# meirbon/rfw-rs

Measured on AMD Instinct MI355X. Metric: Mrays/s (primary+shadow, 1spp), higher is better.
Workload: dtype f32

## Files before the change

### include/rfw_hip.h

```cpp
#ifndef RFW_HIP_H
#define RFW_HIP_H

#include "rfw_pod.h"

#ifdef __cplusplus
extern "C" {
#endif

#define RFW_HIP_API __attribute__((visibility("default")))
#define RFW_HIP_ABI_VERSION 2

enum {
    RFW_HIP_OK = 0,
    RFW_HIP_E_INVALID = -1,
    RFW_HIP_E_DEVICE = -2,
    RFW_HIP_E_STATE = -3,
    RFW_HIP_E_NOMEM = -4
};

enum { RFW_HIP_BUILDER_AUTO = 0, RFW_HIP_BUILDER_HOST_SAH = 1, RFW_HIP_BUILDER_DEVICE_LBVH = 2, RFW_HIP_BUILDER_DEVICE_SAH = 3 };

typedef struct {
    uint32_t struct_size;
    int32_t device;
// ... 55 lines not shown
    uint64_t split_references;
    uint64_t accel_bytes;
    uint32_t packet_copies;
    uint32_t pad;
} rfw_hip_scene_stats;

typedef struct {
    int32_t inst;
    int32_t tri;
    float t;
    float u, v;
} rfw_hip_hit;

RFW_HIP_API void* rfw_hip_create(uint32_t width, uint32_t height, double scale, const rfw_hip_options* options);
RFW_HIP_API void rfw_hip_destroy(void* instance);
RFW_HIP_API const char* rfw_hip_last_error(void* instance);
RFW_HIP_API uint32_t rfw_hip_abi_version(void);
RFW_HIP_API int64_t rfw_hip_selftest_splits(const rfw_rt_triangle* tris, uint32_t n, float split_tau, uint32_t threads, float* pieces7, uint32_t pieces_cap,
                                            uint32_t* duplicate_of, uint32_t duplicates_cap, uint32_t* n_pieces);
RFW_HIP_API uint32_t rfw_hip_selftest_index_magic(uint32_t d, uint64_t n_max);
RFW_HIP_API int64_t rfw_hip_selftest_bvh(const float* boxes6, uint32_t n, uint32_t max_leaf, uint32_t threads, uint32_t* out_nodes);

RFW_HIP_API int rfw_hip_set_2d_mesh(void* instance, uint32_t id, const void* vertices, uint32_t num_vertices, int32_t tex_id);
RFW_HIP_API int rfw_hip_set_2d_instances(void* instance, uint32_t mesh, const rfw_mat4* matrices, uint32_t num_matrices);
RFW_HIP_API int rfw_hip_set_3d_mesh(void* instance, uint32_t id, const rfw_mesh_data_3d* data);
RFW_HIP_API int rfw_hip_unload_3d_meshes(void* instance, const uint32_t* ids, uint32_t num_ids);
RFW_HIP_API int rfw_hip_set_3d_instances(void* instance, uint32_t mesh, const rfw_instances_data_3d* data);
RFW_HIP_API int rfw_hip_set_materials(void* instance, const rfw_device_material* materials, uint32_t num, const uint32_t* changed);
RFW_HIP_API int rfw_hip_set_textures(void* instance, const rfw_texture_data* textures, uint32_t num, const uint32_t* changed);
RFW_HIP_API int rfw_hip_synchronize(void* instance);
enum {
    RFW_HIP_RENDER_DEFAULT = 0,
    RFW_HIP_RENDER_NORMAL = 1,
    RFW_HIP_RENDER_ALBEDO = 2,
    RFW_HIP_RENDER_GBUFFER = 3,
    RFW_HIP_RENDER_SCREEN_SPACE = 4,
    RFW_HIP_RENDER_SSAO = 5,
    RFW_HIP_RENDER_FILTERED_SSAO = 6
};
RFW_HIP_API int rfw_hip_render(void* instance, const rfw_mat4* view_2d, const rfw_camera_view_3d* view_3d, uint32_t mode);
RFW_HIP_API int rfw_hip_resize(void* instance, uint32_t width, uint32_t height, double scale);
RFW_HIP_API int rfw_hip_set_point_lights(void* instance, const rfw_point_light* lights, uint32_t num, const uint32_t* changed);
RFW_HIP_API int rfw_hip_set_spot_lights(void* instance, const rfw_spot_light* lights, uint32_t num, const uint32_t* changed);
RFW_HIP_API int rfw_hip_set_area_lights(void* instance, const rfw_area_light* lights, uint32_t num, const uint32_t* changed);
RFW_HIP_API int rfw_hip_set_directional_lights(void* instance, const rfw_directional_light* lights, uint32_t num, const uint32_t* changed);
RFW_HIP_API int rfw_hip_set_skybox(void* instance, const rfw_texture_data* skybox);
RFW_HIP_API int rfw_hip_set_skins(void* instance, const rfw_skin_data* skins, uint32_t num, const uint32_t* changed);

RFW_HIP_API int rfw_hip_reset_accumulation(void* instance);
RFW_HIP_API int rfw_hip_set_option(void* instance, const char* key, double value);
RFW_HIP_API int rfw_hip_read_framebuffer(void* instance, float* rgba, uint64_t n_floats);
RFW_HIP_API int rfw_hip_read_accumulator(void* instance, float* rgba, uint64_t n_floats);
RFW_HIP_API int rfw_hip_get_frame_stats(void* instance, rfw_hip_frame_stats* out);
RFW_HIP_API int rfw_hip_drain_timing(void* instance, rfw_hip_frame_stats* sum, uint32_t* frames);
RFW_HIP_API int rfw_hip_get_scene_stats(void* instance, rfw_hip_scene_stats* out);
RFW_HIP_API int rfw_hip_set_stream(void* instance, void* hip_stream);
RFW_HIP_API void* rfw_hip_get_stream(void* instance);
RFW_HIP_API int rfw_hip_device_synchronize(void* instance);

RFW_HIP_API int rfw_hip_shard_info(void* instance, uint64_t* slab_floats, uint32_t* num_tiles_local, uint32_t* num_tiles_total);
RFW_HIP_API int rfw_hip_set_slab_output(void* instance, void* device_ptr);
RFW_HIP_API int rfw_hip_assemble_frame(void* instance, const void* gathered_device_ptr);

RFW_HIP_API int rfw_hip_comm_unique_id(void* out128);
RFW_HIP_API int rfw_hip_comm_init(void* instance, const void* id128, uint32_t rank, uint32_t world);
RFW_HIP_API int rfw_hip_comm_destroy(void* instance);
RFW_HIP_API int rfw_hip_comm_init_loopback(void* instance, uint64_t hub_key, uint32_t rank, uint32_t world);

#define RFW_HIP_P2P_HANDLE_BYTES 256
RFW_HIP_API int rfw_hip_p2p_export(void* instance, void* handle_out);
RFW_HIP_API int rfw_hip_p2p_connect(void* instance, const void* handles);
RFW_HIP_API int rfw_hip_p2p_disconnect(void* instance);

RFW_HIP_API int rfw_hip_intersect(void* instance, const float* origins, const float* directions,
                                  float t_min, float t_max, uint64_t n, rfw_hip_hit* hits);
RFW_HIP_API int rfw_hip_occludes(void* instance, const float* origins, const float* directions,
                                 float t_min, const float* t_max, uint64_t n, uint8_t* occluded);
RFW_HIP_API int rfw_hip_depth_test(void* instance, const float* origins, const float* directions,
                                   float t_min, float t_max, uint64_t n, rfw_hip_hit* hits, uint32_t* depth);

RFW_HIP_API int rfw_hip_intersect4(void* instance, const float* origin_xyz4, const float* direction_xyz4, const float* t_min4, float* t4,
                                   int32_t* instance_ids4, int32_t* prim_ids4);
RFW_HIP_API int rfw_hip_occludes4(void* instance, const float* origin_xyz4, const float* direction_xyz4, const float* t_min4, const float* t_max4,
                                  uint8_t* occluded4);

RFW_HIP_API int rfw_hip_debug_read(void* instance, const char* what, void* dst, uint64_t bytes, uint64_t* written);

RFW_HIP_API int rfw_hip_debug_occludes_depth(void* instance, const float* origins, const float* directions, float t_min, const float* t_max,
                                             uint64_t num_rays, uint8_t* occluded, uint32_t* depth);
RFW_HIP_API int rfw_hip_debug_lbvh_stress(void* instance, uint32_t num_boxes, uint32_t iterations, uint32_t seed, uint64_t* errors, uint64_t* checked);

RFW_HIP_API int rfw_hip_debug_eval_shading(void* instance, int op, uint64_t n, const float* in48, float* out12);

RFW_HIP_API int rfw_hip_render_batch(void* instance, const rfw_camera_view_3d* views, uint32_t count);
RFW_HIP_API int rfw_hip_assemble_batch(void* instance, const void* gathered_device_ptr, uint32_t count);
RFW_HIP_API int rfw_hip_render_samples(void* instance, const rfw_camera_view_3d* view, uint32_t count);
RFW_HIP_API int rfw_hip_set_blue_noise(void* instance, const uint32_t* table, uint32_t n_words);
RFW_HIP_API int rfw_hip_read_framebuffer_at(void* instance, uint32_t frame, float* rgba, uint64_t n_floats);
RFW_HIP_API int rfw_hip_read_accumulator_at(void* instance, uint32_t frame, float* rgba, uint64_t n_floats);

RFW_HIP_API void rfw_hip_srgb_steps(float* out255);
RFW_HIP_API void* rfw_hip_host_alloc(uint64_t bytes);
RFW_HIP_API void rfw_hip_host_free(void* ptr);
RFW_HIP_API int rfw_hip_download_frame(void* instance, uint32_t what, uint32_t frame, float* host_rgba, uint64_t n_floats);
RFW_HIP_API int rfw_hip_wait_downloads(void* instance);
RFW_HIP_API int rfw_hip_wait_download(void* instance, const void* host_ptr);
// ... 10 lines not shown
```

### rfw-rs_amd/backend.py

```python
import ctypes as C
import enum
import os

import numpy as np

from . import pod
from .scene import BackendTable

_HERE = os.path.dirname(os.path.abspath(__file__))
HIP_LIB = os.environ.get("RFW_HIP_LIB") or os.path.join(_HERE, "csrc", "librfw_hip.so")

EXPORTS = [
    "rfw_hip_create", "rfw_hip_destroy", "rfw_hip_last_error", "rfw_hip_abi_version", "rfw_hip_selftest_bvh", "rfw_hip_selftest_splits", "rfw_hip_selftest_index_magic",
    "rfw_hip_set_2d_mesh", "rfw_hip_set_2d_instances", "rfw_hip_set_3d_mesh", "rfw_hip_unload_3d_meshes",
    "rfw_hip_set_3d_instances", "rfw_hip_set_materials", "rfw_hip_set_textures", "rfw_hip_synchronize",
    "rfw_hip_render", "rfw_hip_resize", "rfw_hip_set_point_lights", "rfw_hip_set_spot_lights",
    "rfw_hip_set_area_lights", "rfw_hip_set_directional_lights", "rfw_hip_set_skybox", "rfw_hip_set_skins",
    "rfw_hip_reset_accumulation", "rfw_hip_set_option", "rfw_hip_read_framebuffer", "rfw_hip_read_accumulator",
    "rfw_hip_get_frame_stats", "rfw_hip_drain_timing", "rfw_hip_get_scene_stats", "rfw_hip_set_stream", "rfw_hip_get_stream", "rfw_hip_device_synchronize",
    "rfw_hip_shard_info", "rfw_hip_set_slab_output", "rfw_hip_assemble_frame", "rfw_hip_intersect", "rfw_hip_occludes", "rfw_hip_debug_occludes_depth",
    "rfw_hip_debug_read", "rfw_hip_bandwidth_probe", "rfw_hip_depth_test", "rfw_hip_render_batch", "rfw_hip_assemble_batch",
    "rfw_hip_read_framebuffer_at", "rfw_hip_read_accumulator_at", "rfw_hip_host_alloc", "rfw_hip_host_free", "rfw_hip_download_frame",
    "rfw_hip_wait_downloads", "rfw_hip_wait_download", "rfw_hip_srgb_steps", "rfw_hip_render_samples", "rfw_hip_set_blue_noise", "rfw_hip_debug_eval_shading", "rfw_hip_comm_unique_id", "rfw_hip_comm_init", "rfw_hip_comm_init_loopback", "rfw_hip_comm_destroy", "rfw_hip_p2p_export", "rfw_hip_p2p_connect", "rfw_hip_p2p_disconnect", "rfw_hip_intersect4", "rfw_hip_occludes4", "rfw_hip_debug_lbvh_stress", "rfw_hip_issue_probe",
]

_lib = None


ABI_VERSION = 2


def hip_lib():
    global _lib
    if _lib is None:
        if not os.path.exists(HIP_LIB):
            raise RuntimeError(f"HIP extension {HIP_LIB} is missing — build it with __graft_entry__.build(); there is no CPU fallback")
        try:
            import torch
        except ImportError:
            pass
        l = C.CDLL(HIP_LIB)
        vp, u32, u64, f32, cp = C.c_void_p, C.c_uint32, C.c_uint64, C.c_float, C.c_char_p
        l.rfw_hip_create.restype = vp
        l.rfw_hip_create.argtypes = [u32, u32, C.c_double, C.POINTER(pod.HipOptions)]
        l.rfw_hip_destroy.argtypes = [vp]
        l.rfw_hip_destroy.restype = None
        l.rfw_hip_last_error.argtypes = [vp]
        l.rfw_hip_last_error.restype = cp
        l.rfw_hip_abi_version.restype = u32
        if l.rfw_hip_abi_version() != ABI_VERSION:
            raise RuntimeError(f"{HIP_LIB} speaks ABI version {l.rfw_hip_abi_version()}, this binding version {ABI_VERSION}: rebuild the library")
        l.rfw_hip_selftest_bvh.argtypes = [vp, u32, u32, u32, C.POINTER(u32)]
        l.rfw_hip_selftest_bvh.restype = C.c_int64
        l.rfw_hip_selftest_splits.argtypes = [vp, u32, C.c_float, u32, vp, u32, vp, u32, C.POINTER(u32)]
        l.rfw_hip_selftest_splits.restype = C.c_int64
        l.rfw_hip_selftest_index_magic.argtypes = [u32, C.c_uint64]
        l.rfw_hip_selftest_index_magic.restype = u32
        l.rfw_hip_set_2d_mesh.argtypes = [vp, u32, vp, u32, C.c_int32]
        l.rfw_hip_set_2d_instances.argtypes = [vp, u32, vp, u32]
        l.rfw_hip_set_3d_mesh.argtypes = [vp, u32, C.POINTER(pod.MeshData3D)]
        l.rfw_hip_unload_3d_meshes.argtypes = [vp, C.POINTER(u32), u32]
        l.rfw_hip_set_3d_instances.argtypes = [vp, u32, C.POINTER(pod.InstancesData3D)]
        l.rfw_hip_set_materials.argtypes = [vp, vp, u32, vp]
        l.rfw_hip_set_textures.argtypes = [vp, vp, u32, vp]
        l.rfw_hip_synchronize.argtypes = [vp]
        l.rfw_hip_render.argtypes = [vp, C.POINTER(pod.Mat4), C.POINTER(pod.CameraView3D), u32]
        l.rfw_hip_resize.argtypes = [vp, u32, u32, C.c_double]
        for n in ("point", "spot", "area", "directional"):
            getattr(l, f"rfw_hip_set_{n}_lights").argtypes = [vp, vp, u32, vp]
        l.rfw_hip_set_skybox.argtypes = [vp, C.POINTER(pod.TextureData)]
        l.rfw_hip_set_skins.argtypes = [vp, vp, u32, vp]
        l.rfw_hip_reset_accumulation.argtypes = [vp]
        l.rfw_hip_set_option.argtypes = [vp, cp, C.c_double]
        l.rfw_hip_read_framebuffer.argtypes = [vp, vp, u64]
        l.rfw_hip_read_accumulator.argtypes = [vp, vp, u64]
        l.rfw_hip_get_frame_stats.argtypes = [vp, C.POINTER(pod.FrameStats)]
# ... 231 lines not shown

    def accumulator_at(self, frame):
        a = np.empty((self.height, self.width, 4), dtype=np.float32)
        self._check(self._l.rfw_hip_read_accumulator_at(self._h, frame, a.ctypes.data, a.size))
        return a

    def framebuffer_at(self, frame):
        a = np.empty((self.height, self.width, 4), dtype=np.float32)
        self._check(self._l.rfw_hip_read_framebuffer_at(self._h, frame, a.ctypes.data, a.size))
        return a

    def host_frame(self, presented=False):
        n = self.height * self.width * (1 if presented else 4)
        p = self._l.rfw_hip_host_alloc(n * 4)
        if not p:
            raise BackendError("rfw_hip_host_alloc failed")
        if presented:
            a = np.ctypeslib.as_array(C.cast(p, C.POINTER(C.c_uint8)), shape=(self.height, self.width, 4))
        else:
            a = np.ctypeslib.as_array(C.cast(p, C.POINTER(C.c_float)), shape=(self.height, self.width, 4))
        self._pinned[a.ctypes.data] = p
        return a

    def free_host_frame(self, a):
        self._l.rfw_hip_host_free(self._pinned.pop(a.ctypes.data))

    def download_frame(self, dst, accumulator=False, frame=0):
        if dst.dtype == np.uint8:
            self._check(self._l.rfw_hip_download_frame(self._h, 2, frame, dst.ctypes.data, dst.size // 4))
        else:
            self._check(self._l.rfw_hip_download_frame(self._h, 1 if accumulator else 0, frame, dst.ctypes.data, dst.size))

    def srgb_steps(self):
        t = np.empty(255, np.float32)
        self._l.rfw_hip_srgb_steps(t.ctypes.data)
        return t

    def wait_downloads(self, dst=None):
        if dst is None:
            self._check(self._l.rfw_hip_wait_downloads(self._h))
        else:
            self._check(self._l.rfw_hip_wait_download(self._h, dst.ctypes.data))

    def framebuffer(self):
        a = np.empty((self.height, self.width, 4), dtype=np.float32)
        self._check(self._l.rfw_hip_read_framebuffer(self._h, a.ctypes.data, a.size))
        return a

    def accumulator(self):
        a = np.empty((self.height, self.width, 4), dtype=np.float32)
        self._check(self._l.rfw_hip_read_accumulator(self._h, a.ctypes.data, a.size))
        return a

    def frame_stats(self):
        s = pod.FrameStats()
        self._check(self._l.rfw_hip_get_frame_stats(self._h, C.byref(s)))
        return {n: (list(getattr(s, n)) if n in ("nodes_visited", "tris_tested", "instances_entered", "node_test_executions", "tri_test_executions", "wave_max_nodes", "uniform_node_test_executions") else getattr(s, n)) for n, _ in pod.FrameStats._fields_}

    def drain_timing(self):
        s, n = pod.FrameStats(), C.c_uint32(0)
        self._check(self._l.rfw_hip_drain_timing(self._h, C.byref(s), C.byref(n)))
        return {k: getattr(s, k) for k, _ in pod.FrameStats._fields_ if k.startswith("ms_")}, int(n.value)

    def scene_stats(self):
        s = pod.SceneStats()
        self._check(self._l.rfw_hip_get_scene_stats(self._h, C.byref(s)))
        return {n: getattr(s, n) for n, _ in pod.SceneStats._fields_}

    def set_stream(self, stream_handle):
        self._check(self._l.rfw_hip_set_stream(self._h, C.c_void_p(stream_handle)))

    def stream_handle(self):
        return int(self._l.rfw_hip_get_stream(self._h) or 0)

    def device_synchronize(self):
        self._check(self._l.rfw_hip_device_synchronize(self._h))

    def shard_info(self):
        f, a, b = C.c_uint64(0), C.c_uint32(0), C.c_uint32(0)
        self._check(self._l.rfw_hip_shard_info(self._h, C.byref(f), C.byref(a), C.byref(b)))
        return {"slab_floats": int(f.value), "tiles_local": int(a.value), "tiles_total": int(b.value)}

    def set_slab_output(self, device_ptr):
        self._check(self._l.rfw_hip_set_slab_output(self._h, C.c_void_p(device_ptr)))

    def assemble_frame(self, gathered_device_ptr):
        self._check(self._l.rfw_hip_assemble_frame(self._h, C.c_void_p(gathered_device_ptr)))

    def intersect(self, origins, directions, t_min=1e-4, t_max=1e26):
        o = np.ascontiguousarray(origins, dtype=np.float32)
        d = np.ascontiguousarray(directions, dtype=np.float32)
        hits = np.empty(len(o), dtype=HIT_DTYPE)
        self._check(self._l.rfw_hip_intersect(self._h, o.ctypes.data, d.ctypes.data, t_min, t_max, len(o), hits.ctypes.data))
        return hits

    def depth_test(self, origins, directions, t_min=1e-4, t_max=1e26):
        o = np.ascontiguousarray(origins, dtype=np.float32)
        d = np.ascontiguousarray(directions, dtype=np.float32)
        hits = np.empty(len(o), dtype=HIT_DTYPE)
        depth = np.empty(len(o), dtype=np.uint32)
        self._check(self._l.rfw_hip_depth_test(self._h, o.ctypes.data, d.ctypes.data, t_min, t_max, len(o), hits.ctypes.data, depth.ctypes.data))
        return hits, depth

    def occludes_depth(self, origins, directions, t_max, t_min=1e-3):
        o = np.ascontiguousarray(origins, dtype=np.float32)
        d = np.ascontiguousarray(directions, dtype=np.float32)
# ... 56 lines not shown
```

### rfw-rs_amd/csrc/api_frame.cpp

```cpp
#include "api_internal.h"

using namespace rfwapi;

namespace rfwapi {
thread_local std::string g_create_error;
}
namespace rfwhip {
static EnvSwitches g_env;
const EnvSwitches& env_switches() { return g_env; }
void read_env_switches()
{
    EnvSwitches e;
    auto set = [](const char* name) { const char* v = getenv(name); return v != nullptr && std::strcmp(v, "0") != 0; };
    e.build_trace = set("RFW_BUILD_TRACE");
    e.no_forest = set("RFW_NO_FOREST");
    e.lbvh_fenced = set("RFW_LBVH_FENCED");
    e.p2p_data_cached = set("RFW_P2P_DATA_CACHED");
    e.p2p_flags_finegrained = set("RFW_P2P_FLAGS_FINEGRAINED");
    if (const char* v = getenv("RFW_PACKET_AUTO_MAX_TRIANGLES")) e.packet_auto_max_triangles = strtoull(v, nullptr, 10);
    if (const char* v = getenv("RFW_SPATIAL_SPLITS")) { e.has_spatial_splits = true; e.spatial_splits = (float)std::max(0.0, atof(v)); }
    if (const char* v = getenv("RFW_PACKET_TRACE")) e.packet_trace = std::max(0, atoi(v));
    if (const char* v = getenv("RFW_NODE_ORDER")) e.node_order = std::max(0, atoi(v));
    static std::mutex mu;
    std::lock_guard<std::mutex> g(mu);
    g_env = e;
}
}
namespace rfwapi {
uint32_t index_magic(const uint32_t d, const uint64_t n_max)
{
    if (d < 2u) return 0u;
    const uint64_t m = ((1ull << 32) + d - 1u) / d, e = m * d - (1ull << 32);
    if (m > 0xffffffffull || n_max >= (1ull << 32)) return 0u;
    return (e == 0 || n_max < (1ull << 32) / e) ? (uint32_t)m : 0u;
}

void compute_shard(Instance* I)
{
    const uint32_t S = I->substreams, wv = I->world * S;
    I->tiles_x = (I->width + I->tile_size - 1) / I->tile_size;
    I->tiles_y = (I->height + I->tile_size - 1) / I->tile_size;
    const uint32_t total = I->tiles_x * I->tiles_y;
    I->local_tiles_v = (total + wv - 1) / wv;
    I->cap_v = I->local_tiles_v * I->tile_size * I->tile_size;
    I->local_tiles = I->local_tiles_v * S;
    I->capacity = I->cap_v * S;
    uint64_t px = 0;
    for (uint32_t t = 0; t < total; t++) {
        if ((t % wv) / S != I->rank) continue;
        const uint32_t tx = t % I->tiles_x, ty = t / I->tiles_x;
        const uint32_t w = std::min(I->tile_size, I->width - tx * I->tile_size), h = std::min(I->tile_size, I->height - ty * I->tile_size);
        px += (uint64_t)w * h;
    }
    I->local_pixels = px;
}

int alloc_paths(Instance* I)
{
    compute_shard(I);
    const size_t n = (size_t)I->capacity * I->max_batch;
    for (int h = 0; h < 2; h++) {
        HIP_TRY(I, I->d_ray_o[h].ensure(n));
        HIP_TRY(I, I->d_ray_d[h].ensure(n));
        HIP_TRY(I, I->d_thr[h].ensure(n));
        HIP_TRY(I, I->d_hit[h].ensure(n));
    }
    HIP_TRY(I, I->d_sh_o.ensure(n * kShadowBuckets));
    HIP_TRY(I, I->d_sh_d.ensure(n * kShadowBuckets));
    HIP_TRY(I, I->d_sh_e.ensure(n * kShadowBuckets));
    HIP_TRY(I, I->d_acc_slab.ensure(n));
    HIP_TRY(I, hipMemsetAsync(I->d_acc_slab.ptr, 0, n * sizeof(float4), I->stream));
    const size_t px = (size_t)I->width * I->height * I->max_batch;
    HIP_TRY(I, I->d_frame_out.ensure(px));
    I->acc_source = nullptr;
// ... 87 lines not shown
    PathDev p;
    const size_t off = (size_t)sub * I->cap_v;
    for (int h = 0; h < 2; h++) {
        p.ray_o[h] = I->d_ray_o[h].ptr + off;
        p.ray_d[h] = I->d_ray_d[h].ptr + off;
        p.thr[h] = I->d_thr[h].ptr + off;
        p.hit[h] = I->d_hit[h].ptr + off;
    }
    p.sh_o = I->d_sh_o.ptr + off * kShadowBuckets;
    p.sh_d = I->d_sh_d.ptr + off * kShadowBuckets;
    p.sh_e = I->d_sh_e.ptr + off * kShadowBuckets;
    p.acc = I->d_acc_slab.ptr + off;
    p.capacity = I->cap_v;
    return p;
}

inline int ev_index(uint32_t bounce, int kernel, int end) { return EV_KERNEL_BASE + 2 * ((int)bounce * kKernelsPerBounce + kernel) + end; }
constexpr int kEvBlit = EV_KERNEL_BASE + 2 * (kMaxBounces * kKernelsPerBounce);

hipEvent_t* ring_events(Instance* I, int slot, uint32_t sub) { return I->ring.data() + ((size_t)slot * I->substreams + sub) * kNumEvents; }

static float ao_radius_of(Instance* I)
{
    if (I->ao_radius > 0.0f) return I->ao_radius;
    Instance* O = scene_of(I);
    if (O->ao_auto_version != O->scene_version) {
        float lo[3] = {INFINITY, INFINITY, INFINITY}, hi[3] = {-INFINITY, -INFINITY, -INFINITY};
        for (const auto& kv : O->inst_lists) {
            const rfw_aabb& b = kv.second.local_aabb;
            for (const rfw_mat4& m : kv.second.matrices) {
                bool zero = true;
                for (int c = 0; c < 16; c++) zero = zero && m.m[c] == 0.0f;
                if (zero) continue;
                for (int c = 0; c < 8; c++) {
                    const float x = (c & 1) ? b.max[0] : b.min[0], y = (c & 2) ? b.max[1] : b.min[1], z = (c & 4) ? b.max[2] : b.min[2];
                    const float w[3] = {m.m[0] * x + m.m[4] * y + m.m[8] * z + m.m[12], m.m[1] * x + m.m[5] * y + m.m[9] * z + m.m[13],
                                        m.m[2] * x + m.m[6] * y + m.m[10] * z + m.m[14]};
                    for (int a = 0; a < 3; a++) { lo[a] = std::min(lo[a], w[a]); hi[a] = std::max(hi[a], w[a]); }
                }
            }
        }
        double d2 = 0.0;
        for (int a = 0; a < 3; a++) d2 += hi[a] >= lo[a] ? ((double)hi[a] - lo[a]) * ((double)hi[a] - lo[a]) : 0.0;
        O->ao_auto_radius = d2 > 0.0 ? (float)(0.05 * std::sqrt(d2)) : 1.0f;
        O->ao_auto_version = O->scene_version;
    }
    return O->ao_auto_radius;
}

int do_render(Instance* I, const rfw_camera_view_3d* views, uint32_t k, bool samples, uint32_t mode)
{
    const rfw_camera_view_3d& view = views[0];
    HIP_TRY(I, hipSetDevice(I->device));
    if (!scene_of(I)->synchronized || tlas_of(I)->d_tlas_nodes.ptr == nullptr) return RFW_HIP_OK;
    if (I->scene && I->scene->scene_ready && I->waited_version != I->scene->scene_version) {
        HIP_TRY(I, hipStreamWaitEvent(I->stream, I->scene->scene_ready, 0));
        I->waited_version = I->scene->scene_version;
    }
    {
        Instance* S = scene_of(I);
        if (S->tables_ready && I->tables_waited != S->tables_version) {
            HIP_TRY(I, hipStreamWaitEvent(I->stream, S->tables_ready, 0));
            I->tables_waited = S->tables_version;
        }
        I->tables_used = S->tables_version;
        if (I->tables_oldest_pending == ~0ull) I->tables_oldest_pending = S->tables_version;
    }
    if ((I->have_last_view && (std::memcmp(&I->last_view, &view, sizeof(view)) != 0 || mode != I->render_mode)) || I->after_batch) I->sample_count = 0;
    I->render_mode = mode;
    I->after_batch = k > 1 && !samples;
    I->last_view = view;
    I->have_last_view = true;
    if (k > 1) {
        if (k > I->max_batch || k > (uint32_t)kMaxBatch) return fail(I, RFW_HIP_E_INVALID, "render_batch: more frames than options.max_batch");
        if (I->substreams > 1) return fail(I, RFW_HIP_E_STATE, "render_batch: not available with sub-streams");
        if ((uint64_t)I->width * I->height >= (1ull << 24)) return fail(I, RFW_HIP_E_INVALID, "render_batch: frames of 2^24 pixels or more cannot be batched");
        for (uint32_t f = 1; f < k; f++)
            if (views[f].spread_angle != view.spread_angle) return fail(I, RFW_HIP_E_INVALID, "render_batch: the views of a batch must share one spread angle (field of view and height)");
        if (!samples) I->sample_count = 0;
    }

    const uint32_t S = I->substreams;
    const bool count = (I->flags & RFW_HIP_FLAG_COUNT_TRAVERSAL) != 0;
    const bool nee = !(I->flags & RFW_HIP_FLAG_NO_NEE);
    hipStream_t main = I->stream;
    const bool tm = I->timing;
    const int slot = (int)(I->frame_index % kTimingRing);
    I->events = ring_events(I, slot, 0);
    const uint32_t bounces = std::min<uint32_t>(I->max_path_length, kMaxBounces);
    const bool ao = mode >= RFW_HIP_RENDER_SSAO;
    const uint32_t ao_rounds = ao ? I->ao_samples : 0u;
    if (ao) HIP_TRY(I, I->d_ao_guide.ensure((size_t)I->width * I->height));
    const bool dn = I->denoise > 0 && mode == RFW_HIP_RENDER_DEFAULT && (k == 1 || samples) && I->world <= 1 && !scene_of(I)->comm && !scene_of(I)->loop &&
                    !scene_of(I)->p2p.connected;
    if (dn) {
        const size_t px = (size_t)I->width * I->height;
        HIP_TRY(I, I->d_dn_guide.ensure(3 * px));
        for (int q = 0; q < 2 && I->denoise > 1; q++) HIP_TRY(I, I->d_dn_plane[q].ensure(px));
    }

    if (tm) (void)hipEventRecord(I->events[EV_FRAME0], main);
    I->counter_phase ^= 1u;
    if (S > 1) HIP_TRY(I, hipEventRecord(I->ev_fork, main));
    SceneDev sc[kMaxSub];
    PathDev p[kMaxSub];
    CameraParams cam[kMaxSub];
    hipStream_t st[kMaxSub];
    for (uint32_t s = 0; s < S; s++) {
        st[s] = S > 1 ? I->sub[s] : main;
        if (S > 1) HIP_TRY(I, hipStreamWaitEvent(st[s], I->ev_fork, 0));
        sc[s] = scene_dev(I);
        sc[s].counters = I->d_counters.ptr + (size_t)I->counter_phase * kMaxSub + s;
        sc[s].counters_next = I->d_counters.ptr + (size_t)(I->counter_phase ^ 1u) * kMaxSub + s;
        sc[s].spill = I->d_spill.ptr + (size_t)s * (I->cap_v + kSpillMargin);
        p[s] = path_dev(I, s);
        cam[s] = camera_params(I, view, s);
        {
            const Instance* O = scene_of(I);
            const int g = O->shade_group;
            if (g == 256 || (g == 0 && k == 1 && !O->slots.empty())) cam[s].flags |= kFlagShadeSmallGroups;
        }
    }
    BatchViews bv;
    if (k > 1) {
        cam[0].batch = k;
        if (scene_of(I)->stream_auto) cam[0].stream_run = scene_of(I)->stream_run;
        p[0].capacity = I->cap_v * k;
        for (uint32_t f = 0; f < k; f++) {
            cam[0].batch_sample[f] = samples ? I->sample_count + f : 0u;
            FrameView& v = bv.v[f];
            v.pos[0] = views[f].pos.x; v.pos[1] = views[f].pos.y; v.pos[2] = views[f].pos.z; v.lens_size = views[f].lens_size;
            v.right[0] = views[f].right.x; v.right[1] = views[f].right.y; v.right[2] = views[f].right.z; v.pad0 = 0.0f;
            v.up[0] = views[f].up.x; v.up[1] = views[f].up.y; v.up[2] = views[f].up.z; v.pad1 = 0.0f;
            v.p1[0] = views[f].p1.x; v.p1[1] = views[f].p1.y; v.p1[2] = views[f].p1.z; v.pad2 = 0.0f;
        }
    }
    if (mode != RFW_HIP_RENDER_DEFAULT) {
        const float radius = ao ? ao_radius_of(I) : 0.0f;
        const float dir[3] = {view.direction.x, view.direction.y, view.direction.z};
        for (uint32_t s = 0; s < S; s++) {
            hipEvent_t* ev = ring_events(I, slot, s);
            if (tm) (void)hipEventRecord(ev[ev_index(0, 0, 0)], st[s]);
            launch_primary(st[s], cam[s], sc[s], p[s], count);
            if (tm) (void)hipEventRecord(ev[ev_index(0, 0, 1)], st[s]);
            if (tm) (void)hipEventRecord(ev[ev_index(0, 1, 0)], st[s]);
            launch_aov(st[s], cam[s], sc[s], p[s], mode, ao_rounds, radius, I->d_ao_guide.ptr, dir);
            if (tm) (void)hipEventRecord(ev[ev_index(0, 1, 1)], st[s]);
            if (tm) (void)hipEventRecord(ev[ev_index(0, 2, 0)], st[s]);
        }
        for (uint32_t r = 0; r < ao_rounds; r++)
            for (uint32_t s = 0; s < S; s++) launch_shadow(st[s], cam[s], sc[s], p[s], r, count);
        for (uint32_t s = 0; s < S; s++)
            if (tm) (void)hipEventRecord(ring_events(I, slot, s)[ev_index(0, 2, 1)], st[s]);
    }
    for (uint32_t b = 0; b < bounces && mode == RFW_HIP_RENDER_DEFAULT; b++) {
        for (uint32_t s = 0; s < S; s++) {
            hipEvent_t* ev = ring_events(I, slot, s);
            if (tm) (void)hipEventRecord(ev[ev_index(b, 0, 0)], st[s]);
            if (b == 0 && k > 1) launch_primary_batch(st[s], cam[s], bv, sc[s], p[s], count);
            else if (b == 0) launch_primary(st[s], cam[s], sc[s], p[s], count);
            else {
                const uint32_t* order = nullptr;
                const int mode = scene_of(I)->sort_extension_rays;
                if ((mode == 1 || (mode == 2 && k > 1 && cam[s].stream_run == 0u)) && S == 1) {
                    const size_t n = p[s].capacity;
                    for (int q = 0; q < 2; q++) { HIP_TRY(I, I->d_sort_keys[q].ensure(n)); HIP_TRY(I, I->d_sort_vals[q].ensure(n)); }
                    HIP_TRY(I, I->d_sort_ws.ensure(sort_pairs_workspace_bytes((uint32_t)n)));
                    launch_extension_keys(st[s], sc[s], p[s], b, I->d_sort_keys[0].ptr, I->d_sort_vals[0].ptr);
                    HIP_TRY(I, sort_pairs_u32(st[s], I->d_sort_ws.ptr, I->d_sort_ws.cap, I->d_sort_keys[0].ptr, I->d_sort_keys[1].ptr, I->d_sort_vals[0].ptr,
                                              I->d_sort_vals[1].ptr, (uint32_t)n, 32));
                    order = I->d_sort_vals[1].ptr;
                }
                launch_extend(st[s], cam[s], sc[s], p[s], b, count, order);
            }
            if (tm) (void)hipEventRecord(ev[ev_index(b, 0, 1)], st[s]);
            if (b == 0 && dn) {
                PathDev g = p[s];
                if (k > 1) {
                    const size_t last = (size_t)(k - 1u) * I->cap_v;
                    g.hit[0] += last; g.ray_o[0] += last; g.ray_d[0] += last;
                    g.capacity = I->cap_v;
                }
                launch_dn_guide(st[s], cam[s], sc[s], g, I->d_dn_guide.ptr, k > 1 ? 0x00ffffffu : 0xffffffffu);
            }
        }
        for (uint32_t s = 0; s < S; s++) {
            hipEvent_t* ev = ring_events(I, slot, s);
            if (tm) (void)hipEventRecord(ev[ev_index(b, 1, 0)], st[s]);
            launch_shade(st[s], cam[s], sc[s], p[s], b);
            if (tm) (void)hipEventRecord(ev[ev_index(b, 1, 1)], st[s]);
        }
        if (nee)
            for (uint32_t s = 0; s < S; s++) {
                hipEvent_t* ev = ring_events(I, slot, s);
                if (tm) (void)hipEventRecord(ev[ev_index(b, 2, 0)], st[s]);
                launch_shadow(st[s], cam[s], sc[s], p[s], b, count);
                if (tm) (void)hipEventRecord(ev[ev_index(b, 2, 1)], st[s]);
            }
    }
    if (S > 1)
        for (uint32_t s = 0; s < S; s++) {
            HIP_TRY(I, hipEventRecord(I->ev_join[s], st[s]));
            HIP_TRY(I, hipStreamWaitEvent(main, I->ev_join[s], 0));
        }
    if (samples && k > 1) {
        launch_sum_batch(main, I->d_acc_slab.ptr, I->cap_v, k);
        cam[0].batch = 1;
    }
    I->sample_count += samples ? k : 1;
    const uint32_t frames_out = samples ? 1u : k;
    if (tm) (void)hipEventRecord(I->events[kEvBlit], main);
    if (Instance* C = scene_of(I); C->comm || C->loop) {
        const uint64_t n_send = slab_words(I) * frames_out;
        pack_slabs(I, main, I->d_send.ptr, frames_out);
        if (C->comm_chain && C->comm_chain_pending) HIP_TRY(I, hipStreamWaitEvent(main, C->comm_chain, 0));
        if (C->loop) {
            const int lrc = loop_all_gather(I, main, n_send);
            if (lrc != RFW_HIP_OK) return lrc;
        } else {
            const ncclResult_t nr = g_rccl.all_gather(I->d_send.ptr, I->d_recv.ptr, n_send, ncclFloat, C->comm, main);
            if (nr != ncclSuccess) return fail(I, RFW_HIP_E_DEVICE, std::string("ncclAllGather: ") + g_rccl.error_string(nr));
        }
        if (C->comm_chain) { HIP_TRY(I, hipEventRecord(C->comm_chain, main)); C->comm_chain_pending = true; }
        const int arc = gathered_arrived(I, main, I->d_recv.ptr, frames_out);
        if (arc != RFW_HIP_OK) return arc;
    } else if (C->p2p.connected) {
        const int prc = p2p_exchange(I, main, frames_out);
        if (prc != RFW_HIP_OK) return prc;
    } else if (I->world <= 1)
    {
        if (dn) {
            float4* const planes[2] = {I->d_dn_plane[0].ptr, I->d_dn_plane[1].ptr};
            launch_atrous(main, cam[0], I->d_acc_slab.ptr, I->cap_v, I->d_dn_guide.ptr, planes, I->d_frame_out.ptr, I->sample_count, I->denoise, I->denoise_colour,
                          I->denoise_form);
        }
        else if (mode == RFW_HIP_RENDER_FILTERED_SSAO) launch_ao_filter(main, cam[0], I->d_acc_slab.ptr, I->cap_v, I->d_ao_guide.ptr, I->d_frame_out.ptr, I->sample_count);
        else launch_assemble(main, cam[0], I->d_acc_slab.ptr, false, false, I->cap_v, I->d_frame_out.ptr, I->sample_count, mode != RFW_HIP_RENDER_DEFAULT);
        I->acc_source = I->d_acc_slab.ptr; I->acc_source_rgb = false; I->acc_source_batch = frames_out;
    }
    if (I->external_slab)
        pack_slabs(I, main, I->external_slab, frames_out);
    if (tm) (void)hipEventRecord(I->events[kEvBlit + 1], main);
    if (tm) (void)hipEventRecord(I->events[EV_FRAME1], main);
    HIP_TRY(I, hipGetLastError());
    const uint32_t passes = mode == RFW_HIP_RENDER_DEFAULT ? bounces : 1u;
    I->last_bounces = passes;
    I->ring_bounces[slot] = tm ? passes : 0;
    I->ring_nee[slot] = mode == RFW_HIP_RENDER_DEFAULT ? nee : ao;
    I->ao_rounds = ao_rounds;
// ... 3 lines not shown
    I->last_count_flag = count;
    if (I->frame_done) HIP_TRY(I, hipEventRecord(I->frame_done, main));
    return RFW_HIP_OK;
}

}

extern "C" {

uint32_t rfw_hip_abi_version(void) { return RFW_HIP_ABI_VERSION; }
uint32_t rfw_hip_selftest_index_magic(uint32_t d, uint64_t n_max) { return index_magic(d, n_max); }


void* rfw_hip_create(uint32_t width, uint32_t height, double , const rfw_hip_options* o)
{
    read_env_switches();
    int ndev = 0;
    hipError_t e = hipGetDeviceCount(&ndev);
    if (e != hipSuccess || ndev == 0) {
        g_create_error = std::string("no HIP device available (") + (e == hipSuccess ? "0 devices" : hipGetErrorString(e)) +
                         "); this backend has no CPU fallback";
        return nullptr;
    }
    if (width == 0 || height == 0) {
        g_create_error = "width and height must be non-zero";
        return nullptr;
    }
    Instance* I = new Instance();
    I->width = width;
    I->height = height;
    int dev = -1;
    uint32_t n_slots = 1;
    if (o) {
        dev = o->device;
        if (o->max_path_length) I->max_path_length = std::min<uint32_t>(o->max_path_length, kMaxBounces);
        if (o->clamp_value > 0.0f) I->clamp_value = o->clamp_value;
        I->world = std::max<uint32_t>(o->world, 1);
        I->rank = o->rank;
        if (o->tile_size) I->tile_size = o->tile_size;
        if (o->builder) I->builder = o->builder;
        I->flags = o->flags & 15u;
        if (o->streams) I->substreams = std::min<uint32_t>(o->streams, kMaxSub);
        if (o->struct_size >= offsetof(rfw_hip_options, frames_in_flight) + sizeof(uint32_t)) n_slots = std::min<uint32_t>(std::max<uint32_t>(o->frames_in_flight, 1u), 24u);
        if (o->struct_size >= offsetof(rfw_hip_options, max_batch) + sizeof(uint32_t)) I->max_batch = std::min<uint32_t>(std::max<uint32_t>(o->max_batch, 1u), (uint32_t)kMaxBatch);
    }
    {
        const EnvSwitches& env = env_switches();
        if (env.has_spatial_splits) I->split_tau = env.spatial_splits;
        const int pt = env.packet_trace >= 0 ? env.packet_trace : kDefaultPacketTrace;
        I->packet_auto = env.packet_trace < 0;
        if (pt & 1) I->flags |= kFlagPacketPrimary;
        if (pt & 2) I->flags |= kFlagPacketShadow;
        if (pt & 4) I->flags |= kFlagPacketShadowFar;
    }
    if (I->max_batch > 1 && I->substreams > 1) {
        g_create_error = "max_batch > 1 needs streams <= 1 (a batch already fills the device with one launch per stage)";
        delete I;
        return nullptr;
    }
    if (I->rank >= I->world || (I->tile_size % 8) != 0) {
        g_create_error = "invalid shard options (rank >= world, or tile_size not a multiple of 8)";
        delete I;
        return nullptr;
    }
    I->blas_on_device = I->builder != RFW_HIP_BUILDER_HOST_SAH;
    I->blas_sah_on_device = I->builder == RFW_HIP_BUILDER_DEVICE_SAH || I->builder == RFW_HIP_BUILDER_AUTO;
    I->tlas_on_device = I->builder != RFW_HIP_BUILDER_HOST_SAH;
    if (dev < 0) (void)hipGetDevice(&dev);
    I->device = dev;
    I->build_threads = (int)std::max(1u, std::min(16u, std::thread::hardware_concurrency()));
    auto bail = [&](const char* what, hipError_t err) -> void* {
        g_create_error = std::string(what) + ": " + hipGetErrorString(err);
        delete I;
        return nullptr;
    };
    if ((e = hipSetDevice(dev)) != hipSuccess) return bail("hipSetDevice", e);
    if ((e = hipStreamCreateWithFlags(&I->own_stream, hipStreamNonBlocking)) != hipSuccess) return bail("hipStreamCreate", e);
    I->stream = I->own_stream;
    I->ring.assign((size_t)kTimingRing * I->substreams * kNumEvents, nullptr);
    for (auto& ev : I->ring)
        if ((e = hipEventCreate(&ev)) != hipSuccess) return bail("hipEventCreate", e);
    I->events = I->ring.data();
    if ((e = hipEventCreateWithFlags(&I->ev_fork, hipEventDisableTiming)) != hipSuccess) return bail("hipEventCreate", e);
    for (uint32_t k = 0; k < I->substreams && I->substreams > 1; k++) {
        if ((e = hipStreamCreateWithFlags(&I->sub[k], hipStreamNonBlocking)) != hipSuccess) return bail("hipStreamCreate", e);
        if ((e = hipEventCreateWithFlags(&I->ev_join[k], hipEventDisableTiming)) != hipSuccess) return bail("hipEventCreate", e);
    }
    for (int k = 0; k < Instance::kStages; k++)
        if ((e = hipEventCreateWithFlags(&I->stage_event[k], hipEventDisableTiming)) != hipSuccess) return bail("hipEventCreate", e);
    if ((e = hipHostMalloc((void**)&I->overflow_host, 64, hipHostMallocMapped)) != hipSuccess) return bail("hipHostMalloc (overflow flag)", e);
    std::memset(I->overflow_host, 0, 64);
    if ((e = hipHostGetDevicePointer((void**)&I->overflow_dev, I->overflow_host, 0)) != hipSuccess) return bail("hipHostGetDevicePointer", e);
    if (alloc_paths(I) != RFW_HIP_OK) {
        g_create_error = I->err;
        delete I;
        return nullptr;
    }
    (void)hipStreamSynchronize(I->stream);
    if (n_slots > 1) {
        if ((e = hipEventCreateWithFlags(&I->frame_done, hipEventDisableTiming)) != hipSuccess) return bail("hipEventCreate", e);
        if ((e = hipEventCreateWithFlags(&I->scene_ready, hipEventDisableTiming)) != hipSuccess) return bail("hipEventCreate", e);
        rfw_hip_options so;
        std::memset(&so, 0, sizeof(so));
        if (o) std::memcpy(&so, o, std::min<size_t>(o->struct_size ? o->struct_size : sizeof(so), sizeof(so)));
        so.struct_size = sizeof(so);
        so.device = I->device;
        so.frames_in_flight = 1;
        so.max_batch = I->max_batch;
        for (uint32_t k = 1; k < n_slots; k++) {
            Instance* c = static_cast<Instance*>(rfw_hip_create(width, height, 1.0, &so));
            if (!c) {
                for (Instance* d : I->slots) rfw_hip_destroy(d);
                I->slots.clear();
                rfw_hip_destroy(I);
                return nullptr;
            }
            c->scene = I;
            c->slot_index = k;
            if (hipEventCreateWithFlags(&c->frame_done, hipEventDisableTiming) != hipSuccess) {
                g_create_error = "hipEventCreate (frame slot)";
                rfw_hip_destroy(c);
                for (Instance* d : I->slots) rfw_hip_destroy(d);
                I->slots.clear();
                rfw_hip_destroy(I);
                return nullptr;
            }
            I->slots.push_back(c);
        }
    }
    return I;
}

void rfw_hip_destroy(void* inst)
{
    if (!inst) return;
    Instance* I = static_cast<Instance*>(inst);
    for (Instance* c : I->slots) rfw_hip_destroy(c);
    I->slots.clear();
    {
        std::lock_guard<std::mutex> g(I->mu);
        (void)hipSetDevice(I->device);
        (void)hipDeviceSynchronize();
        if (I->scene_ready) (void)hipEventDestroy(I->scene_ready);
        if (I->frame_done) (void)hipEventDestroy(I->frame_done);
        if (I->download_done) (void)hipEventDestroy(I->download_done);
        I->d_blas_nodes.release(); I->d_tlas_nodes.release(); I->d_blas_wide.release(); I->d_tlas_wide.release(); I->d_blas_oct.release(); I->d_tlas_oct.release(); I->d_blas_raw.release(); I->d_tlas_raw.release(); I->d_packets.release(); I->d_triangles.release();
        I->d_mesh_records.release(); I->d_matrices.release(); I->d_mesh_of_instance.release(); I->d_tlas_prims.release();
        I->d_xforms.release(); I->d_normals.release();
        for (auto& tb : I->tables) { tb.materials.release(); tb.area.release(); tb.point.release(); tb.spot.release(); tb.dir.release(); }
        if (I->tables_ready) (void)hipEventDestroy(I->tables_ready);
        if (I->upload_stream) (void)hipStreamDestroy(I->upload_stream);
        I->d_spill.release(); I->d_counters.release(); I->d_tex_data.release(); I->d_tex_desc.release(); I->d_blue_noise.release();
        I->d_valid_gids.release(); I->d_stage_dev.release(); I->d_tlas_order.release(); I->d_node_count.release(); I->d_inst_boxes.release(); I->d_mesh_local.release();
        I->d_tri_boxes.release(); I->d_lbvh_ws.release(); I->d_blas_order.release();
        I->d_q_o.release(); I->d_q_d.release(); I->d_q_t.release(); I->d_q_h.release(); I->d_q_depth.release(); I->d_q_r.release();
        if (I->comm) { (void)g_rccl.comm_destroy(I->comm); I->comm = nullptr; }
        if (I->loop) loop_leave(I);
        if (I->loop_sent) { (void)hipEventDestroy(I->loop_sent); I->loop_sent = nullptr; }
        if (I->comm_chain) (void)hipEventDestroy(I->comm_chain);
        for (auto& ev : I->ev_build)
            if (ev) (void)hipEventDestroy(ev);
        if (I->records_stream) (void)hipStreamSynchronize(I->records_stream);
        if (I->ev_heads) (void)hipEventDestroy(I->ev_heads);
        if (I->ev_records) (void)hipEventDestroy(I->ev_records);
        if (I->records_stream) (void)hipStreamDestroy(I->records_stream);
        I->d_heads.release();
        I->meshes.clear();
        for (auto& L : I->lanes) {
            if (L.s) (void)hipStreamDestroy(L.s);
            if (L.done) (void)hipEventDestroy(L.done);
            L.ws.release(); L.boxes.release();
        }
        p2p_release(I);
        I->d_send.release(); I->d_recv.release();
        for (int q = 0; q < 2; q++) { I->d_sort_keys[q].release(); I->d_sort_vals[q].release(); }
        I->d_sort_ws.release();
        if (I->overflow_host) (void)hipHostFree(I->overflow_host);
        I->pins.release();
        I->d_skin_data.release(); I->d_joints.release(); I->d_bounds_scratch.release(); I->d_sah_ws.release(); I->d_mesh_node_counts.release(); I->d_forest.release(); I->d_refit_parent.release(); I->d_refit_nint.release(); I->d_refit_arrive.release();
        for (int k = 0; k < Instance::kStages; k++) {
            if (I->stage_buf[k]) (void)hipHostFree(I->stage_buf[k]);
            if (I->stage_event[k]) (void)hipEventDestroy(I->stage_event[k]);
        }
        for (int h = 0; h < 2; h++) { I->d_ray_o[h].release(); I->d_ray_d[h].release(); I->d_thr[h].release(); I->d_hit[h].release(); }
        I->d_sh_o.release(); I->d_sh_d.release(); I->d_sh_e.release(); I->d_acc_slab.release(); I->d_frame_acc.release(); I->d_frame_out.release(); I->d_present.release();
        I->d_dn_guide.release(); I->d_dn_plane[0].release(); I->d_dn_plane[1].release();
        for (auto& ev : I->ring)
            if (ev) (void)hipEventDestroy(ev);
        if (I->ev_fork) (void)hipEventDestroy(I->ev_fork);
        for (int k = 0; k < kMaxSub; k++) {
            if (I->ev_join[k]) (void)hipEventDestroy(I->ev_join[k]);
            if (I->sub[k]) (void)hipStreamDestroy(I->sub[k]);
        }
        if (I->own_stream) (void)hipStreamDestroy(I->own_stream);
    }
    delete I;
}

const char* rfw_hip_last_error(void* inst)
{
    if (!inst) return g_create_error.c_str();
    return static_cast<Instance*>(inst)->err.c_str();
}

// ... 23 lines not shown
    if (rc != RFW_HIP_OK && cur != I && !cur->err.empty()) I->err = cur->err;
    return rc;
}

int rfw_hip_render(void* inst, const rfw_mat4* , const rfw_camera_view_3d* view, uint32_t mode)
{
    LOCK(inst);
    if (!view) return fail(I, RFW_HIP_E_INVALID, "render: null view");
    CHECK_OVERFLOW(I);
    return render_impl(I, view, 1, false, mode <= (uint32_t)RFW_HIP_RENDER_FILTERED_SSAO ? mode : (uint32_t)RFW_HIP_RENDER_DEFAULT);
}

int rfw_hip_render_batch(void* inst, const rfw_camera_view_3d* views, uint32_t count)
{
    LOCK(inst);
    if (!views || count == 0) return fail(I, RFW_HIP_E_INVALID, "render_batch: no views");
    CHECK_OVERFLOW(I);
    if (count == 1) {
        I->sample_count = 0;
        I->restart = true;
    }
    const int rc = render_impl(I, views, count);
    if (rc == RFW_HIP_OK && count == 1) (I->slots.empty() ? I : slot_ptr(I, I->cur_slot))->after_batch = true;
    return rc;
}

int rfw_hip_render_samples(void* inst, const rfw_camera_view_3d* view, uint32_t count)
{
    LOCK(inst);
    if (!view || count == 0) return fail(I, RFW_HIP_E_INVALID, "render_samples: no view / no samples");
    CHECK_OVERFLOW(I);
    if (count > I->max_batch || count > (uint32_t)kMaxBatch) return fail(I, RFW_HIP_E_INVALID, "render_samples: more samples than options.max_batch");
    if (count == 1) return render_impl(I, view, 1);
    rfw_camera_view_3d views[kMaxBatch];
    for (uint32_t f = 0; f < count; f++) views[f] = *view;
    return render_impl(I, views, count, true);
}


int rfw_hip_resize(void* inst, uint32_t w, uint32_t h, double)
{
    LOCK(inst);
    if (w == 0 || h == 0) return fail(I, RFW_HIP_E_INVALID, "resize: zero size");
    if (scene_of(I)->p2p.data && (w != I->width || h != I->height)) return fail(I, RFW_HIP_E_STATE, "resize: disconnect the p2p exchange first (its buffers are sized for the frame)");
    HIP_TRY(I, hipSetDevice(I->device));
    HIP_TRY(I, hipStreamSynchronize(I->stream));
    for (Instance* c : I->slots) {
        const int rc = rfw_hip_resize(c, w, h, 1.0);
        if (rc != RFW_HIP_OK) return fail(I, rc, c->err);
    }
    I->restart = true;
    I->width = w;
    I->height = h;
    I->deferred = Instance::Deferred(); I->acc_source = nullptr; I->presented_valid = false;
    const int arc = alloc_paths(I);
    if (arc == RFW_HIP_OK && (scene_of(I)->comm || scene_of(I)->loop)) {
        const size_t n = (size_t)I->capacity * I->max_batch * 3u;
        HIP_TRY(I, I->d_send.ensure(n));
        HIP_TRY(I, I->d_recv.ensure(n * I->world));
    }
    return arc;
}


int rfw_hip_reset_accumulation(void* inst)
{
    LOCK(inst);
    I->sample_count = 0;
    I->restart = true;
    return RFW_HIP_OK;
}

int rfw_hip_set_option(void* inst, const char* key, double value)
{
    LOCK(inst);
    if (!key) return fail(I, RFW_HIP_E_INVALID, "set_option: null key");
    const std::string k(key);
    if (k == "max_path_length") I->max_path_length = std::max<uint32_t>(1, std::min<uint32_t>((uint32_t)value, kMaxBounces));
    else if (k == "clamp_value") I->clamp_value = (float)value;
    else if (k == "nee") I->flags = value != 0.0 ? (I->flags & ~RFW_HIP_FLAG_NO_NEE) : (I->flags | RFW_HIP_FLAG_NO_NEE);
    else if (k == "count_traversal") I->flags = value != 0.0 ? (I->flags | RFW_HIP_FLAG_COUNT_TRAVERSAL) : (I->flags & ~RFW_HIP_FLAG_COUNT_TRAVERSAL);
    else if (k == "shadow_order") {
        I->flags &= ~(kFlagNearFirstDirectional | kFlagFarFirstPositional);
        if ((int)value == 1) I->flags |= kFlagNearFirstDirectional;
        else if ((int)value == 2) I->flags |= kFlagFarFirstPositional;
    }
    else if (k == "packet_trace") {
        I->flags &= ~(kFlagPacketPrimary | kFlagPacketShadow | kFlagPacketShadowFar);
        I->packet_auto = false;
        if ((int)value & 1) I->flags |= kFlagPacketPrimary;
        if ((int)value & 2) I->flags |= kFlagPacketShadow;
        if ((int)value & 4) I->flags |= kFlagPacketShadowFar;
        if (blas_wide_wanted(I, I->n_tris) && !I->d_blas_wide.ptr && I->n_tris) {
            for (auto& kv : I->meshes) kv.second.dirty = true;
            I->meshes_dirty = true;
            I->layout_valid = false;
        }
    }
    else if (k == "shade_group") {
        if ((int)value != 0 && (int)value != 256 && (int)value != 512) return fail(I, RFW_HIP_E_INVALID, "set_option: shade_group is 0, 256 or 512");
        I->shade_group = (int)value;
    }
    else if (k == "tlas_fused") I->tlas_fused = std::max(0, std::min(2, (int)value));
    else if (k == "sample_count") I->sample_count = (uint32_t)value;
    else if (k == "ao_samples" || k == "ao_radius") {
        if (k == "ao_samples") {
            if (!(value >= 1.0 && value <= (double)kAoMaxSamples)) return fail(I, RFW_HIP_E_INVALID, "set_option: ao_samples is 1 ... 8");
            I->ao_samples = (uint32_t)value;
        } else {
            if (!(value >= 0.0) || !std::isfinite(value)) return fail(I, RFW_HIP_E_INVALID, "set_option: ao_radius is >= 0 (0 = automatic)");
            I->ao_radius = (float)value;
        }
        I->sample_count = 0;
        I->restart = true;
    }
    else if (k == "denoise" || k == "denoise_colour") {
        if (k == "denoise") {
            if (!(value >= 0.0 && value <= (double)kDenoiseMaxPasses) || value != std::floor(value)) return fail(I, RFW_HIP_E_INVALID, "set_option: denoise is 0 (off) or 1 ... 5 passes");
            if ((uint32_t)value == I->denoise) return RFW_HIP_OK;
            I->denoise = (uint32_t)value;
        } else {
            if (!(value > 0.0) || !std::isfinite(value) || !((float)value > 0.0f) || !std::isfinite((float)value)) return fail(I, RFW_HIP_E_INVALID, "set_option: denoise_colour is > 0");
            if ((float)value == I->denoise_colour) return RFW_HIP_OK;
            I->denoise_colour = (float)value;
        }
        I->sample_count = 0;
        I->restart = true;
    }
    else if (k == "denoise_form") {
        if (value != 0.0 && value != 1.0 && value != 2.0) return fail(I, RFW_HIP_E_INVALID, "set_option: denoise_form is 0, 1 or 2");
        I->denoise_form = (uint32_t)value;
    }
    else if (k == "gather_format") {
        if (value < 0 || value > 2) return fail(I, RFW_HIP_E_INVALID, "set_option: gather_format is 0, 1 or 2");
        I->gather_format = (uint32_t)value;
        for (uint32_t q = 0; q <= I->slots.size(); q++) {
            Instance* c = slot_ptr(I, q);
            c->deferred = Instance::Deferred(); c->acc_source = nullptr; c->presented_valid = false;
        }
    }
    else if (k == "present_rank") I->present_rank = (int)value;
    else if (k == "timing") I->timing = value != 0.0;
    else if (k == "sort_extension_rays") I->sort_extension_rays = std::max(0, std::min(2, (int)value));
    else if (k == "texture_array") { I->texture_array = value != 0.0; I->tex_offsets.clear(); }
    else if (k == "spill_rows") {
        I->spill_rows = std::min<uint32_t>((uint32_t)std::max(0.0, value), (uint32_t)kStackSpill);
        clear_overflow(I);
    }
    else if (k == "sky_r") I->sky[0] = (float)value;
    else if (k == "sky_g") I->sky[1] = (float)value;
// ... 131 lines not shown
        Instance* c = slot_ptr(I, (uint32_t)k);
        if (c->download_dst.empty()) continue;
        if (host_ptr && std::find(c->download_dst.begin(), c->download_dst.end(), host_ptr) == c->download_dst.end()) continue;
        HIP_TRY(I, hipEventSynchronize(c->download_done));
        c->download_dst.clear();
    }
    return RFW_HIP_OK;
}
int rfw_hip_wait_downloads(void* inst) { return rfw_hip_wait_download(inst, nullptr); }

int rfw_hip_read_framebuffer(void* inst, float* rgba, uint64_t n) { return read_frame_impl(inst, 0, false, rgba, n); }
int rfw_hip_read_accumulator(void* inst, float* rgba, uint64_t n) { return read_frame_impl(inst, 0, true, rgba, n); }

static void add_frame_timing(Instance* I, int slot, uint32_t nb, bool nee, rfw_hip_frame_stats* out)
{
    hipEvent_t* e0 = ring_events(I, slot, 0);
    auto el = [&](hipEvent_t a, hipEvent_t b) { float ms = 0.0f; (void)hipEventElapsedTime(&ms, a, b); return ms; };
    out->ms_total += el(e0[EV_FRAME0], e0[EV_FRAME1]);
    out->ms_other += el(e0[kEvBlit], e0[kEvBlit + 1]);
    for (uint32_t s = 0; s < I->substreams; s++) {
        hipEvent_t* ev = ring_events(I, slot, s);
        for (uint32_t b = 0; b < nb; b++) {
            const float tr = el(ev[ev_index(b, 0, 0)], ev[ev_index(b, 0, 1)]);
            if (b == 0) out->ms_trace_primary += tr; else out->ms_trace_extend += tr;
            out->ms_shade += el(ev[ev_index(b, 1, 0)], ev[ev_index(b, 1, 1)]);
            if (nee) out->ms_trace_shadow += el(ev[ev_index(b, 2, 0)], ev[ev_index(b, 2, 1)]);
        }
    }
}

int rfw_hip_get_frame_stats(void* inst, rfw_hip_frame_stats* out)
{
    LOCK(inst);
    if (!out) return fail(I, RFW_HIP_E_INVALID, "get_frame_stats: null out");
    if (!I->slots.empty() && I->cur_slot != 0) {
        Instance* c = slot_ptr(I, I->cur_slot);
        const int rc = rfw_hip_get_frame_stats(c, out);
        if (rc != RFW_HIP_OK) I->err = c->err;
        return rc;
    }
    HIP_TRY(I, hipSetDevice(I->device));
    std::memset(out, 0, sizeof(*out));
    HIP_TRY(I, hipStreamSynchronize(I->stream));
    QueueCounters qc[kMaxSub];
    HIP_TRY(I, hipMemcpy(qc, I->d_counters.ptr + (size_t)I->counter_phase * kMaxSub, I->substreams * sizeof(QueueCounters), hipMemcpyDeviceToHost));
    CHECK_OVERFLOW(I);
    const uint32_t nb = I->last_bounces;
    out->primary_rays = nb ? I->local_pixels : 0;
    for (uint32_t s = 0; s < I->substreams; s++) {
        for (uint32_t b = 0; b + 1 < nb; b++) out->extension_rays += qc[s].ext[b];
        if (!(I->flags & RFW_HIP_FLAG_NO_NEE))
            for (uint32_t b = 0; b < nb; b++)
                for (int k = 0; k < kShadowBuckets; k++) out->shadow_rays += qc[s].shadow[b][k];
        for (int k = 0; k < 3; k++) {
            out->nodes_visited[k] += qc[s].trav[k][0];
            out->tris_tested[k] += qc[s].trav[k][1];
            out->instances_entered[k] += qc[s].trav[k][2];
            out->node_test_executions[k] += qc[s].wave_exec[k][0];
            out->tri_test_executions[k] += qc[s].wave_exec[k][1];
            out->uniform_node_test_executions[k] += qc[s].wave_uniform[k];
            out->wave_max_nodes[k] += qc[s].wave_max_nodes[k];
        }
    }
    out->sample_count = I->sample_count;
    out->bounces = nb;
    out->substreams = I->substreams;
    if (I->frame_recorded && nb) add_frame_timing(I, (int)((I->frame_index - 1) % kTimingRing), nb, !(I->flags & RFW_HIP_FLAG_NO_NEE), out);
    return RFW_HIP_OK;
}

int rfw_hip_drain_timing(void* inst, rfw_hip_frame_stats* sum, uint32_t* frames)
{
    LOCK(inst);
    if (!sum || !frames) return fail(I, RFW_HIP_E_INVALID, "drain_timing: null out");
    HIP_TRY(I, hipSetDevice(I->device));
    HIP_TRY(I, hipStreamSynchronize(I->stream));
    std::memset(sum, 0, sizeof(*sum));
    uint32_t n = 0;
    for (uint64_t f = I->drained_index; f < I->frame_index; f++) {
        const int slot = (int)(f % kTimingRing);
        const uint32_t nb = I->ring_bounces[slot];
        if (!nb) continue;
        add_frame_timing(I, slot, nb, I->ring_nee[slot], sum);
        n++;
    }
    sum->substreams = I->substreams;
    I->drained_index = I->frame_index;
    for (Instance* c : I->slots) {
        rfw_hip_frame_stats cs;
        uint32_t cn = 0;
        const int rc = rfw_hip_drain_timing(c, &cs, &cn);
        if (rc != RFW_HIP_OK) return fail(I, rc, c->err);
        sum->ms_total += cs.ms_total; sum->ms_trace_primary += cs.ms_trace_primary; sum->ms_trace_extend += cs.ms_trace_extend;
        sum->ms_trace_shadow += cs.ms_trace_shadow; sum->ms_shade += cs.ms_shade; sum->ms_other += cs.ms_other;
        n += cn;
    }
    *frames = n;
    return RFW_HIP_OK;
}


int rfw_hip_set_stream(void* inst, void* stream)
{
    LOCK(inst);
    if (!I->slots.empty()) return fail(I, RFW_HIP_E_STATE, "set_stream: an instance with frames in flight launches on its slots' own streams");
    HIP_TRY(I, hipSetDevice(I->device));
    HIP_TRY(I, hipStreamSynchronize(I->stream));
    I->stream = stream ? (hipStream_t)stream : I->own_stream;
    return RFW_HIP_OK;
}

void* rfw_hip_get_stream(void* inst)
{
    if (!inst) return nullptr;
    Instance* I = static_cast<Instance*>(inst);
    std::lock_guard<std::mutex> g(I->mu);
    return (void*)I->stream;
}

int rfw_hip_device_synchronize(void* inst)
// ... 10 lines not shown
```

### rfw-rs_amd/csrc/api_internal.h

```cpp
#pragma once
#include <hip/hip_runtime.h>
#include <dlfcn.h>
#include <unistd.h>
#if __has_include(<rccl/rccl.h>)
#include <rccl/rccl.h>
#else
extern "C" {
typedef struct ncclComm* ncclComm_t;
typedef struct { char internal[128]; } ncclUniqueId;
typedef enum { ncclSuccess = 0 } ncclResult_t;
typedef enum { ncclFloat = 7 } ncclDataType_t;
ncclResult_t ncclGetUniqueId(ncclUniqueId* id);
ncclResult_t ncclCommInitRank(ncclComm_t* comm, int nranks, ncclUniqueId id, int rank);
ncclResult_t ncclCommDestroy(ncclComm_t comm);
ncclResult_t ncclAllGather(const void* send, void* recv, size_t count, ncclDataType_t type, ncclComm_t comm, hipStream_t stream);
const char* ncclGetErrorString(ncclResult_t r);
}
#endif

#include <algorithm>
#include <atomic>
#include <chrono>
#include <cmath>
#include <cstring>
// ... 281 lines not shown
    int stage_next = 0;
    void* stage = nullptr;
    bool tlas_on_device = true, blas_on_device = false, blas_sah_on_device = false;
    DevBuf<char> d_sah_ws;
    DevBuf<uint32_t> d_mesh_node_counts;
    DevBuf<ForestTree> d_forest;
    DevBuf<uint32_t> d_refit_parent, d_refit_nint, d_refit_arrive;
    DevBuf<QueueCounters> d_counters;
    uint32_t counter_phase = 0;
    uint32_t* overflow_host = nullptr;
    uint32_t* overflow_dev = nullptr;
    uint32_t spill_rows = kStackSpill;
    DevBuf<float> d_q_o, d_q_d, d_q_t;
    DevBuf<rfw_hip_hit> d_q_h;
    DevBuf<uint32_t> d_q_depth;
    DevBuf<uint8_t> d_q_r;
    std::vector<MeshRecord> mesh_records;
    std::map<uint32_t, uint32_t> mesh_index;
    std::vector<uint32_t> record_tri_cap;
    std::vector<uint32_t> record_tri_orig;
    DevBuf<SplitPiece> d_split_pieces;
    std::vector<uint32_t> record_piece_off, record_piece_n;
    float split_tau = 8e-5f;
    uint64_t n_split_refs = 0;
    uint32_t tri_end = 0, node_end = 0;
    uint64_t hole_tris = 0;
    bool layout_valid = false;
    bool node_counts_stale = false;
    uint32_t incremental_builds = 0, full_builds = 0, heads_first_builds = 0, tlas_fused_builds = 0;
    bool packet_auto = true;
    PinnedRing pins;
    uint64_t n_instances = 0, n_valid_instances = 0, n_tris = 0, n_blas_nodes = 0, n_tlas_nodes = 0;
    uint64_t n_tris_logical = 0;
    float ms_blas_build = 0, ms_tlas_build = 0, ms_stage_wait = 0;
    float ms_blas_upload = 0, ms_blas_kernels = 0;
    uint64_t blas_upload_bytes = 0, blas_kernel_bytes = 0;
    struct BuildLane { hipStream_t s = nullptr; hipEvent_t done = nullptr; DevBuf<char> ws; DevBuf<DevBox> boxes; };
    static constexpr int kBuildLanes = 8;
    BuildLane lanes[kBuildLanes];
    hipEvent_t ev_build[3] = {nullptr, nullptr, nullptr};
    DevBuf<TriHead> d_heads;
    hipStream_t records_stream = nullptr;
    hipEvent_t ev_heads = nullptr, ev_records = nullptr;
    bool build_from_heads = false;
    bool records_pending = false;
    bool records_timed = false;
    bool build_events_pending = false;

    DevBuf<float4> d_ray_o[2], d_ray_d[2], d_thr[2], d_sh_o, d_sh_d, d_sh_e, d_acc_slab, d_frame_acc, d_frame_out;
    DevBuf<uint32_t> d_present;
    DevBuf<uint4> d_hit[2];
    DevBuf<uint32_t> d_sort_keys[2], d_sort_vals[2];
    DevBuf<char> d_sort_ws;
    int shade_group = 0;
    int sort_extension_rays = 2;
    void* external_slab = nullptr;
    ncclComm_t comm = nullptr;
    DevBuf<float> d_send, d_recv;
    uint32_t gather_format = 0;
    int present_rank = -1;
    struct Deferred { const void* gathered = nullptr; uint32_t k = 0, samples = 1; } deferred;
    bool presented_valid = false;
    hipEvent_t comm_chain = nullptr;
    bool comm_chain_pending = false;
    struct LoopHub* loop = nullptr;
    uint32_t loop_seq = 0;
    hipEvent_t loop_sent = nullptr;
    struct P2P {
        bool connected = false;
        uint32_t* data = nullptr;
        uint32_t* flags = nullptr;
        size_t slot_words = 0;
        uint32_t n_slots = 0;
        std::vector<uint32_t*> peer_data, peer_flags;
        std::vector<uint8_t> opened;
        uint64_t timeout_ticks = 500000000ull;
    } p2p;
    uint32_t slot_index = 0;
    uint32_t stream_leaf_gate = 16;
    bool stream_auto = true;
    uint32_t stream_run = 8, stream_refill = 12;
    uint32_t p2p_seq = 0;
    bool frame_elsewhere = false;
    uint32_t tiles_x = 0, tiles_y = 0, local_tiles = 0, capacity = 0;
    uint64_t local_pixels = 0;
    uint32_t sample_count = 0;
    bool have_last_view = false;
    rfw_camera_view_3d last_view{};
    uint32_t render_mode = 0;
    uint32_t ao_samples = 4;
    float ao_radius = 0.0f;
    float ao_auto_radius = 0.0f;
    uint64_t ao_auto_version = 0;
    uint32_t ao_rounds = 0;
    DevBuf<float4> d_ao_guide;
    uint32_t denoise = 0;
    float denoise_colour = kDenoiseDefaultColour;
    uint32_t denoise_form = 0;
    DevBuf<float4> d_dn_guide, d_dn_plane[2];
    std::vector<hipEvent_t> ring;
    hipEvent_t* events = nullptr;
    uint32_t substreams = 1;
    hipStream_t sub[kMaxSub] = {};
    hipEvent_t ev_fork = nullptr, ev_join[kMaxSub] = {};
    uint32_t local_tiles_v = 0, cap_v = 0;
    uint64_t frame_index = 0, drained_index = 0;
// ... 103 lines not shown
```

### rfw-rs_amd/csrc/device_types.h

```cpp
#pragma once
#include <cmath>
#include <cstdint>
#include <cstring>

#include "../../include/rfw_pod.h"

namespace rfwhip {

struct alignas(16) Node4 {
    float lox[4], hix[4], loy[4], hiy[4], loz[4], hiz[4];
    uint32_t child[4];
    uint32_t pad[4];
};
static_assert(sizeof(Node4) == 128, "Node4 must be one 128-B line");
constexpr uint32_t kInvalidRef = 0xffffffffu;
constexpr uint32_t kLeafBit = 0x80000000u;
constexpr uint32_t kNoPath = 0xfffffffeu;
constexpr uint32_t kLeafFirstMask = 0x07ffffffu;
constexpr int kMaxLeafTris = 8;
inline __host__ __device__ uint32_t make_leaf(uint32_t first, uint32_t count) { return kLeafBit | ((count - 1u) << 27) | first; }

struct alignas(16) Node4Q {
    float ox, oy, oz;
    float sx;
// ... 136 lines not shown
    uint32_t flags;
    uint32_t mesh;
};
static_assert(sizeof(InstanceXform) == 64, "InstanceXform");
constexpr uint32_t kInstanceIdentity = 2u;

struct alignas(16) InstanceNormal {
    float n_r0[4], n_r1[4], n_r2[4];
};

struct TexDesc {
    uint32_t offset;
    uint32_t w, h, mips;
    uint32_t format;
    uint32_t pad[3];
};
static_assert(sizeof(TexDesc) == 32, "TexDesc");

struct MeshRecord {
    uint32_t node_base, node_count;
    uint32_t tri_base, tri_count;
    uint32_t tri_logical;
    uint32_t pad[3];
};
static_assert(sizeof(MeshRecord) == 32, "MeshRecord");

struct CameraParams {
    float pos[3]; float lens_size;
    float right[3]; float spread_angle;
    float up[3]; float clamp_value;
    float p1[3]; uint32_t tile_shift;
    uint32_t width, height, sample_count, width_magic;
    uint32_t point_light_count, area_light_count, spot_light_count, directional_light_count;
    uint32_t tile_size, tiles_x, tiles_y, rank;
    uint32_t world, local_tiles, flags, max_path_length;
    float sky[3]; uint32_t tiles_x_magic;
    uint32_t batch, frame_capacity, stream_run, stream_refill;
    uint32_t batch_sample[16];
};

constexpr int kMaxBatch = 16;
constexpr uint32_t kBlueNoiseWords = 5u * 65536u;
struct FrameView {
    float pos[3]; float lens_size;
    float right[3]; float pad0;
    float up[3]; float pad1;
    float p1[3]; float pad2;
};
struct BatchViews {
    FrameView v[kMaxBatch];
};

constexpr int kShadowBuckets = 8;
struct QueueCounters {
    uint32_t ext[8];
    uint32_t shadow[8][kShadowBuckets];
    unsigned long long trav[3][3];
    unsigned long long overflow, pad;
    unsigned long long wave_max_nodes[3];
    unsigned long long wave_exec[3][2];
    unsigned long long max_nodes[3];
    unsigned long long pad2;
    unsigned long long wave_uniform[3];
    unsigned long long pad3;
};

enum : uint32_t { kFlagNoNee = 1u, kFlagCount = 2u, kFlagNearFirstDirectional = 4u, kFlagFarFirstPositional = 8u,
                  kFlagPacketPrimary = 16u, kFlagPacketShadow = 32u,
                  kFlagPacketShadowFar = 64u, kFlagShadeSmallGroups = 128u };


}
```

### rfw-rs_amd/csrc/env_switches.h

```cpp
#pragma once
#include <cstdint>

namespace rfwhip {
struct EnvSwitches {
    bool build_trace = false;
    bool no_forest = false;
    bool lbvh_fenced = false;
    bool p2p_data_cached = false;
    bool p2p_flags_finegrained = false;
    uint64_t packet_auto_max_triangles = 0;
    bool has_spatial_splits = false;
    float spatial_splits = 0.0f;
    int node_order = 0;
    int packet_trace = -1;
};
const EnvSwitches& env_switches();
void read_env_switches();
}
```

### rfw-rs_amd/csrc/kernels.h

```cpp
#pragma once
#include <hip/hip_runtime.h>

#include "../../include/rfw_hip.h"
#include "device_types.h"

namespace rfwhip {

struct SceneDev {
    const Node4Q* tlas_nodes;
    const uint32_t* tlas_prims;
    const InstanceXform* instances;
    const InstanceNormal* instance_normals;
    const MeshRecord* meshes;
    const Node4Q* blas_nodes;
    const PacketNode* tlas_wide;
    const PacketNode* blas_wide;
    uint32_t tlas_wide_stride, blas_wide_stride;
    const Node4Q* tlas_oct;
    const Node4Q* blas_oct;
    const TriPacket* tri_packets;
    const rfw_rt_triangle* triangles;
    const rfw_device_material* materials;
    const rfw_area_light* area_lights;
    const rfw_point_light* point_lights;
    const rfw_spot_light* spot_lights;
    const rfw_directional_light* directional_lights;
    const uint32_t* tex_data;
    const TexDesc* tex_desc;
    uint32_t n_textures;
    TexDesc skybox;
    const uint8_t* blue_noise;
    uint32_t* spill;
    uint32_t spill_stride;
    uint32_t spill_rows;
    uint32_t* overflow_flag;
    QueueCounters* counters;
    QueueCounters* counters_next;
};

struct PathDev {
    float4* ray_o[2];
    float4* ray_d[2];
    float4* thr[2];
    uint4* hit[2];
    float4* sh_o;
    float4* sh_d;
    float4* sh_e;
    float4* acc;
    uint32_t capacity;
};

void launch_prepare_instances(hipStream_t s, const rfw_mat4* matrices, const uint32_t* mesh_of_instance, const MeshRecord* meshes, uint32_t n,
                              InstanceXform* xf, InstanceNormal* nm);
void launch_primary(hipStream_t s, const CameraParams& cam, const SceneDev& sc, const PathDev& p, bool count);
void launch_primary_batch(hipStream_t s, const CameraParams& cam, const BatchViews& views, const SceneDev& sc, const PathDev& p, bool count);
void launch_extend(hipStream_t s, const CameraParams& cam, const SceneDev& sc, const PathDev& p, uint32_t bounce, bool count, const uint32_t* order = nullptr);
void launch_extension_keys(hipStream_t s, const SceneDev& sc, const PathDev& p, uint32_t bounce, uint32_t* keys, uint32_t* vals);
void launch_shade(hipStream_t s, const CameraParams& cam, const SceneDev& sc, const PathDev& p, uint32_t bounce);
void launch_shadow(hipStream_t s, const CameraParams& cam, const SceneDev& sc, const PathDev& p, uint32_t bounce, bool count);
void launch_copy_f4(hipStream_t s, const float4* src, float4* dst, uint64_t n);
void launch_issue_probe(hipStream_t s, int mix, uint32_t cus, uint32_t trips, float* out);
uint32_t issue_probe_vector_per_trip(int mix);
struct OctantCopies {
    PacketNode* wide = nullptr;
    Node4Q* quant = nullptr;
    uint32_t stride = 0;
};
void launch_quantize_nodes(hipStream_t s, const Node4* in, Node4Q* out, const OctantCopies& oc, uint32_t first, uint32_t n, const uint32_t* live = nullptr);
void launch_tlas_finish(hipStream_t s, const Node4* raw, Node4Q* out, const OctantCopies& oc, uint32_t n_nodes_max, const uint32_t* live, const rfw_mat4* matrices,
                        const uint32_t* mesh_of_instance, const MeshRecord* meshes, uint32_t n_instances, InstanceXform* xf, InstanceNormal* nm);
void launch_expand_nodes(hipStream_t s, const Node4Q* in, const OctantCopies& oc, uint32_t first, uint32_t n, const uint32_t* live = nullptr);
void launch_quantize_regions(hipStream_t s, const Node4* in, Node4Q* out, const OctantCopies& oc, uint32_t n, const MeshRecord* recs, const uint32_t* counts, uint32_t n_recs);
void launch_assemble(hipStream_t s, const CameraParams& cam, const void* gathered, bool rgb, bool accumulator, uint64_t slab_elems, float4* frame,
                     uint32_t samples, bool linear = false);
void launch_sum_batch(hipStream_t s, float4* acc_slabs, uint64_t slab_elems, uint32_t count);
void launch_pack_rgb(hipStream_t s, const float4* acc_slab, float* out, uint64_t n);
void launch_pack_finished(hipStream_t s, const float4* acc_slab, void* out, uint64_t n, uint32_t samples, uint32_t format, const float* steps255, bool linear = false);
struct P2PTargets { uint32_t* p[16]; };
void launch_p2p_wait(hipStream_t s, const uint32_t* flags, uint32_t first, uint32_t count, uint32_t want, uint64_t limit_ticks, uint32_t* timeout_flag);
void launch_p2p_signal(hipStream_t s, const P2PTargets& targets, uint32_t count, uint32_t value);
void launch_assemble_finished(hipStream_t s, const CameraParams& cam, const void* gathered, uint64_t slab_elems, uint32_t format, float4* frame, uint32_t* presented);
void launch_present(hipStream_t s, const float4* frame, uint32_t* bgra, uint64_t n, const float* steps255, bool narrow);
constexpr uint32_t kAoMaxSamples = kShadowBuckets;
void launch_aov(hipStream_t s, const CameraParams& cam, const SceneDev& sc, const PathDev& p, uint32_t mode, uint32_t ao_samples, float ao_radius, float4* guide,
                const float direction[3]);
void launch_ao_filter(hipStream_t s, const CameraParams& cam, const float4* acc, uint64_t slab_elems, const float4* guide, float4* frame, uint32_t samples);
void launch_dn_guide(hipStream_t s, const CameraParams& cam, const SceneDev& sc, const PathDev& p, float4* guide, uint32_t pixel_mask);
constexpr uint32_t kDenoiseMaxPasses = 5;
constexpr float kDenoiseDefaultColour = 32.0f;
void launch_atrous(hipStream_t s, const CameraParams& cam, const float4* acc, uint64_t slab_elems, const float4* guide, float4* const planes[2], float4* frame,
                   uint32_t samples, uint32_t passes, float sigma_colour, uint32_t form);
void launch_eval_shading(hipStream_t s, const SceneDev& sc, const CameraParams& cam, int op, uint32_t n, const float* in, float* out);
void launch_query_closest(hipStream_t s, const SceneDev& sc, const float* origins, const float* directions, float t_min, float t_max, uint64_t n,
                          rfw_hip_hit* hits, uint32_t* depth = nullptr );
void launch_query_any(hipStream_t s, const SceneDev& sc, const float* origins, const float* directions, float t_min, const float* t_max, uint64_t n,
                      uint8_t* occluded, uint32_t* depth = nullptr );

}
```

### rfw-rs_amd/csrc/kernels.hip

```cpp
#include "kernels.h"
#include "shade_device.h"
#include "traverse.h"
#include "traverse_packet.h"

constexpr int kTraceWaves = 6, kTraceWavesAny = 8, kStreamWaves = 6, kStreamWavesAny = 8, kPacketWaves = 8;

namespace rfwhip {

RFW_DI bool morton_tile(uint32_t ts) { const uint32_t bpr = ts >> 3; return bpr <= 16u && (bpr & (bpr - 1u)) == 0u; }
RFW_DI uint32_t morton_even_bits(uint32_t v) { return (v & 1u) | ((v >> 1) & 2u) | ((v >> 2) & 4u) | ((v >> 3) & 8u); }
RFW_DI uint32_t morton_spread_bits(uint32_t v) { return (v & 1u) | ((v & 2u) << 1) | ((v & 4u) << 2) | ((v & 8u) << 3); }
RFW_DI uint32_t div_magic(const uint32_t n, const uint32_t d, const uint32_t magic) { return magic ? __umulhi(n, magic) : n / d; }
RFW_DI bool slab_to_pixel(const CameraParams& c, uint32_t idx, uint32_t& px, uint32_t& py)
{
    const uint32_t ts = c.tile_size, per_tile = ts * ts;
    const uint32_t lt = c.tile_shift != 0xffffffffu ? idx >> (2u * c.tile_shift) : idx / per_tile, within = idx - lt * per_tile;
    const uint32_t tile = lt * c.world + c.rank;
    if (tile >= c.tiles_x * c.tiles_y) return false;
    const uint32_t ty = div_magic(tile, c.tiles_x, c.tiles_x_magic), tx = tile - ty * c.tiles_x;
    const uint32_t block = within >> 6, lane = within & 63u, bpr = ts >> 3;
    uint32_t by, bx;
    if (morton_tile(ts)) {
        bx = morton_even_bits(block);
        by = morton_even_bits(block >> 1);
// ... 384 lines not shown
        float t = 1e26f, hu = 0.0f, hv = 0.0f;
        int32_t hi = -1, ht = -1;
        const SceneView sv = scene_view(sc);
        traverse<false, COUNT>(sv, O, D, 1e-4f, t, hu, hv, hi, ht, s_stack, threadIdx.x, block * kTraceBlock, tc);
        const uint32_t bary = f2u(65535.0f * hu) + (f2u(65535.0f * hv) << 16);
        p.hit[half][j] = make_uint4((uint32_t)hi, (uint32_t)ht, fbits(t), bary);
    }
    flush_counters<COUNT>(sc.counters, tc, 1);
}

struct ExtendStream {
    const PathDev& p;
    const uint32_t* order;
    uint32_t half;
    uint32_t next, end;
    uint32_t j;
    RFW_DI bool more() const { return next < end; }
    static constexpr float kTMin = 1e-4f;
    RFW_DI bool fetch(const uint64_t idle, f3& O, f3& D, float& t)
    {
        const uint32_t i = next + __builtin_amdgcn_mbcnt_hi((uint32_t)(idle >> 32), __builtin_amdgcn_mbcnt_lo((uint32_t)idle, 0u));
        if (i >= end) return false;
        j = order ? order[i] : i;
        const float4 o4 = p.ray_o[half][j], d4 = p.ray_d[half][j];
        O = mk3(o4.x, o4.y, o4.z);
        D = mk3(d4.x, d4.y, d4.z);
        t = 1e26f;
        return true;
    }
    RFW_DI void advance(const uint64_t idle) { next += (uint32_t)__popcll(idle); }
    RFW_DI void commit(bool, const float t, const float hu, const float hv, const int32_t hi, const int32_t ht)
    {
        const uint32_t bary = f2u(65535.0f * hu) + (f2u(65535.0f * hv) << 16);
        p.hit[half][j] = make_uint4((uint32_t)hi, (uint32_t)ht, fbits(t), bary);
    }
};
template <bool COUNT>
__global__ __launch_bounds__(kTraceBlock, kStreamWaves) void k_extend_stream(const CameraParams cam, const SceneDev sc, const PathDev p, const uint32_t bounce,
                                                                                const uint32_t* __restrict__ order)
{
    __shared__ uint32_t s_stack[kTraceLdsRows * kTraceBlock];
    const uint32_t run = cam.stream_run * kTraceBlock;
    const uint32_t block = xcd_run(blockIdx.x, 64u / cam.stream_run);
    const uint32_t count = sc.counters->ext[bounce - 1];
    if (block * run >= count) return;
    TravCounters tc{0, 0, 0};
    ExtendStream st{p, order, bounce & 1u, block * run, min(count, (block + 1u) * run), 0u};
    const SceneView sv = scene_view(sc);
    traverse_stream<false, COUNT, false>(sv, st, cam.stream_refill & 0xffu, cam.stream_refill >> 8, s_stack, threadIdx.x, blockIdx.x * kTraceBlock, tc);
    flush_counters<COUNT>(sc.counters, tc, 1);
}

RFW_DI bool bucket_far_first(const CameraParams& cam, const uint32_t bucket);
template <bool COUNT, bool BATCH = false>
__global__ __launch_bounds__(kTraceBlock, kTraceWavesAny) void k_shadow(const CameraParams cam, const SceneDev sc, const PathDev p, const uint32_t bounce)
{
    __shared__ uint32_t s_stack[kTraceLdsRowsAny * kTraceBlock];
    uint32_t block = xcd_block(blockIdx.x);
    const uint32_t spill_base = block * kTraceBlock;
    uint32_t bucket = 0, count = 0;
    {
        bool found = false;
        for (int kk = 0; kk < kShadowBuckets; kk++) {
            const int k = kShadowBuckets - 1 - kk;
            if ((cam.flags & kFlagPacketShadowFar) && bucket_far_first(cam, (uint32_t)k)) continue;
            const uint32_t c = sc.counters->shadow[bounce][k];
            const uint32_t nb = (c + kTraceBlock - 1) / kTraceBlock;
            if (!found) {
                if (block < nb) { found = true; bucket = (uint32_t)k; count = c; }
                else block -= nb;
            }
        }
        if (!found) return;
    }
    const uint32_t local = block * kTraceBlock + threadIdx.x;
    const uint32_t idx = bucket * p.capacity + local;
    TravCounters tc{0, 0, 0};
    if (local < count) {
        const float4 o4 = p.sh_o[idx], d4 = p.sh_d[idx];
        const f3 O = mk3(o4.x, o4.y, o4.z), D = mk3(d4.x, d4.y, d4.z);
        float t = d4.w - 0.0001f, hu, hv;
        if (t > 3.0e38f) t = 3.0e38f;
        int32_t hi = -1, ht = -1;
        const SceneView sv = scene_view(sc);
        const bool far_first = bucket == (uint32_t)kShadowBuckets - 1u ? !(cam.flags & kFlagNearFirstDirectional) : (cam.flags & kFlagFarFirstPositional) != 0u;
        const bool occluded = far_first ? traverse<true, COUNT, true>(sv, O, D, 0.001f, t, hu, hv, hi, ht, s_stack, threadIdx.x, spill_base, tc)
                                        : traverse<true, COUNT, false>(sv, O, D, 0.001f, t, hu, hv, hi, ht, s_stack, threadIdx.x, spill_base, tc);
        if (!occluded) {
            uint32_t lane = threadIdx.x;
            asm volatile("" : "+v"(lane));
            const float4 e = p.sh_e[bucket * p.capacity + block * kTraceBlock + lane];
            const uint32_t slot = fbits(e.w);
            float4 a = p.acc[slot];
            a.x += e.x; a.y += e.y; a.z += e.z; a.w += 0.0f;
            p.acc[slot] = a;
        }
    }
    flush_counters<COUNT>(sc.counters, tc, 2);
}

RFW_DI bool bucket_far_first(const CameraParams& cam, const uint32_t bucket);
template <bool COUNT, bool FAR>
__global__ __launch_bounds__(kTraceBlock, kPacketWaves) void k_shadow_packet(const CameraParams cam, const SceneDev sc, const PathDev p, const uint32_t bounce)
{
    uint32_t block = xcd_block(blockIdx.x);
    uint32_t bucket = 0, count = 0;
    {
        bool found = false;
        for (int kk = 0; kk < kShadowBuckets; kk++) {
            const int k = kShadowBuckets - 1 - kk;
            if (bucket_far_first(cam, (uint32_t)k) != FAR) continue;
            const uint32_t c = sc.counters->shadow[bounce][k];
            const uint32_t nb = (c + kTraceBlock - 1) / kTraceBlock;
            if (!found) {
                if (block < nb) { found = true; bucket = (uint32_t)k; count = c; }
                else block -= nb;
            }
        }
        if (!found) return;
    }
    const uint32_t local = block * kTraceBlock + threadIdx.x;
    const uint32_t idx = bucket * p.capacity + local;
    TravCounters tc{0, 0, 0};
    const bool valid = local < count;
    f3 O = mk3(0.0f), D = mk3(0.0f);
    float t = 1.0f, hu, hv;
    if (valid) {
        const float4 o4 = p.sh_o[idx], d4 = p.sh_d[idx];
        O = mk3(o4.x, o4.y, o4.z);
        D = mk3(d4.x, d4.y, d4.z);
        t = d4.w - 0.0001f;
        if (t > 3.0e38f) t = 3.0e38f;
    }
    int32_t hi = -1, ht = -1;
    bool occluded;
    const SceneView sv = scene_view(sc);
    traverse_packet<true, COUNT, FAR>(sv, sc.tlas_wide, sc.tlas_wide_stride, sc.blas_wide, sc.blas_wide_stride, valid, O, D, 0.001f, t, hu, hv, hi, ht, occluded, tc);
    if (valid && !occluded) {
        const float4 e = p.sh_e[idx];
        const uint32_t slot = fbits(e.w);
        float4 a = p.acc[slot];
        a.x += e.x; a.y += e.y; a.z += e.z; a.w += 0.0f;
        p.acc[slot] = a;
    }
    flush_counters<COUNT>(sc.counters, tc, 2);
}

struct ShadowStream {
    const PathDev& p;
    uint32_t base;
    uint32_t next, end;
// ... 5 lines not shown
        const uint32_t i = next + __builtin_amdgcn_mbcnt_hi((uint32_t)(idle >> 32), __builtin_amdgcn_mbcnt_lo((uint32_t)idle, 0u));
        if (i >= end) return false;
        idx = base + i;
        const float4 o4 = p.sh_o[idx], d4 = p.sh_d[idx];
        O = mk3(o4.x, o4.y, o4.z);
        D = mk3(d4.x, d4.y, d4.z);
        t = d4.w - 0.0001f;
        if (t > 3.0e38f) t = 3.0e38f;
        return true;
    }
    RFW_DI void advance(const uint64_t idle) { next += (uint32_t)__popcll(idle); }
    RFW_DI void commit(const bool occluded, float, float, float, int32_t, int32_t)
    {
        if (occluded) return;
        const float4 e = p.sh_e[idx];
        const uint32_t slot = fbits(e.w);
        float4 a = p.acc[slot];
        a.x += e.x; a.y += e.y; a.z += e.z; a.w += 0.0f;
        p.acc[slot] = a;
    }
};
RFW_DI bool bucket_far_first(const CameraParams& cam, const uint32_t bucket)
{
    return bucket == (uint32_t)kShadowBuckets - 1u ? !(cam.flags & kFlagNearFirstDirectional) : (cam.flags & kFlagFarFirstPositional) != 0u;
}
template <bool COUNT, bool FAR>
__global__ __launch_bounds__(kTraceBlock, kStreamWavesAny) void k_shadow_stream(const CameraParams cam, const SceneDev sc, const PathDev p, const uint32_t bounce)
{
    __shared__ uint32_t s_stack[kTraceLdsRowsAny * kTraceBlock];
    const uint32_t run = cam.stream_run * kTraceBlock;
    uint32_t block = xcd_run(blockIdx.x, 64u / cam.stream_run);
    uint32_t bucket = 0, count = 0;
    {
        bool found = false;
        for (int kk = 0; kk < kShadowBuckets; kk++) {
            const int k = kShadowBuckets - 1 - kk;
            if (bucket_far_first(cam, (uint32_t)k) != FAR) continue;
            const uint32_t c = sc.counters->shadow[bounce][k];
            const uint32_t nb = (c + run - 1u) / run;
            if (!found) {
                if (block < nb) { found = true; bucket = (uint32_t)k; count = c; }
                else block -= nb;
            }
        }
        if (!found) return;
    }
    TravCounters tc{0, 0, 0};
    ShadowStream st{p, bucket * p.capacity, block * run, min(count, (block + 1u) * run), 0u};
    const SceneView sv = scene_view(sc);
    traverse_stream<true, COUNT, FAR>(sv, st, cam.stream_refill & 0xffu, cam.stream_refill >> 8, s_stack, threadIdx.x, blockIdx.x * kTraceBlock, tc);
    flush_counters<COUNT>(sc.counters, tc, 2);
}

template <bool BATCH, int kShadeBlock>
__global__ __launch_bounds__(kShadeBlock) void k_shade(const CameraParams cam, const SceneDev sc, const PathDev p, const uint32_t bounce)
{
    static_assert(kShadeBlock >= 128 && 8 * (kShadeBlock / 64) <= 64, "k_shade: the extension-ray filing needs a second wavefront and at most 64 (octant, wavefront) counts");
    const uint32_t idx = blockIdx.x * kShadeBlock + threadIdx.x;
    const uint32_t count = bounce == 0 ? p.capacity : sc.counters->ext[bounce - 1];
    if (blockIdx.x * kShadeBlock >= count) return;
    const uint32_t half = bounce & 1u, next_half = half ^ 1u;
    const uint32_t path_length = bounce;

    bool live = idx < count;

    bool push_ext = false, push_shadow = false;
    int light_bucket = 0;
    f3 ext_o = mk3(0.0f), ext_d = mk3(0.0f), ext_thr = mk3(0.0f);
    float ext_pdf = 0.0f;
    uint32_t ext_normal = 0;
    f3 sh_o = mk3(0.0f), sh_d = mk3(0.0f), sh_e = mk3(0.0f);
    float sh_dist = 0.0f;
    uint32_t PATH_ID = 0, PATH_WORD = 0, sh_slot = 0;

    uint4 S = make_uint4(kNoPath, 0u, 0u, 0u);
    if (live) {
        S = p.hit[half][idx];
        live = S.x != kNoPath;
    }
    if (live) {
        const float4 O4 = p.ray_o[half][idx], D4 = p.ray_d[half][idx];
        const f3 O = mk3(O4.x, O4.y, O4.z), D = mk3(D4.x, D4.y, D4.z);
        f3 throughput = mk3(1.0f);
        float bsdfPdf = 1.0f;
        if (path_length != 0) {
            const float4 T4 = p.thr[half][idx];
            throughput = mk3(T4.x, T4.y, T4.z);
            bsdfPdf = T4.w;
        }
        const uint32_t path_word = fbits(O4.w);
        PATH_ID = BATCH ? (path_word & 0xffffffu) : path_word;
        PATH_WORD = path_word;
        uint32_t owner, slot = idx;
        if (bounce != 0) {
            const uint32_t py_ = div_magic(PATH_ID, cam.width, cam.width_magic);
            slot = pixel_to_slab(cam, PATH_ID - py_ * cam.width, py_, owner) + (BATCH ? (path_word >> 24) * cam.frame_capacity : 0u);
        }
        const int32_t INST_ID = (int32_t)S.x;
        const uint32_t TRI_ID = S.y;
        const float T_VAL = bitsf(S.z);

        if (INST_ID < 0) {
            f3 sky = mk3(cam.sky[0], cam.sky[1], cam.sky[2]);
            if (sc.skybox.mips) {
                const float su = 0.5f * (1.0f + rfw_atan2f(D.x, -D.z) * (1.0f / 3.14159265359f));
                const float sv = 1.0f - rfw_acosf(D.y) * (1.0f / 3.14159265359f);
                const f4 c = texture_sample(sc.tex_data, sc.skybox, su, sv, (float)(int)path_length);
                sky = mk3(c.x, c.y, c.z);
            }
            f3 contribution = throughput * sky * (1.0f / bsdfPdf);
            CLAMPINTENSITY(contribution, cam.clamp_value);
            float4 a = p.acc[slot];
            a.x += contribution.x; a.y += contribution.y; a.z += contribution.z; a.w += 0.0f;
            p.acc[slot] = a;
        } else {
            const float4* tp = reinterpret_cast<const float4*>(sc.triangles + TRI_ID);
            const float4 q3 = tp[3], q4 = tp[4], q5 = tp[5], q6 = tp[6], T0 = tp[7], T1 = tp[8], T2 = tp[9];
            const uint4 q10 = *reinterpret_cast<const uint4*>(tp + 10);
            const int32_t mat_id = (int32_t)q10.y;
            const float tri_area = bitsf(q10.w);
            ShadingData sd = extractParameters(sc.materials + mat_id);

            const uint32_t sampleId = BATCH ? cam.batch_sample[path_word >> 24] : cam.sample_count;
            uint32_t seed = wang_hash(PATH_ID * 16789u + sampleId * 1791u + path_length * 720898027u);

            const float u = (float)(S.w & 65535u) * (1.0f / 65535.0f);
            const float v = (float)(S.w >> 16) * (1.0f / 65535.0f);
            const float w = 1.0f - u - v;

            f3 gN = mk3(q3.x, q3.y, q3.z);
            f3 N = w * mk3(q4.x, q4.y, q4.z) + u * mk3(q5.x, q5.y, q5.z) + v * mk3(q6.x, q6.y, q6.z);
            f3 T = w * mk3(T0.x, T0.y, T0.z) + u * mk3(T1.x, T1.y, T1.z) + v * mk3(T2.x, T2.y, T2.z);
            const float Tw = w * T0.w + u * T1.w + v * T2.w;

            const float4* np = reinterpret_cast<const float4*>(sc.instance_normals + INST_ID);
            const float4 n0 = np[0], n1 = np[1], n2 = np[2];
            gN = normalize(xform_rows(n0, n1, n2, gN, 0.0f));
            N = normalize(xform_rows(n0, n1, n2, N, 0.0f));
            T = normalize(xform_rows(n0, n1, n2, T, 0.0f));
            const f3 B = cross(N, T) * Tw;
            const f3 P = O + T_VAL * D;

            const bool any_map = (sd.flags & 63u) != 0u;
            if ((sd.color.x > 1.0f || sd.color.y > 1.0f || sd.color.z > 1.0f) && !(sd.flags & RFW_MAT_HAS_EMISSIVE_MAP)) {
                f3 contribution = mk3(0.0f);
                const float DdotNL = -dot(D, N);
                bool add = true;
                if (DdotNL > 0.0f) {
                    if (path_length == 0) {
                        contribution = throughput * sd.color * (1.0f / bsdfPdf);
                    } else {
                        const float lightPdf = CalculateLightPDF(D, T_VAL, tri_area, N);
                        const int lc = (int)(cam.area_light_count + cam.point_light_count + cam.spot_light_count + cam.directional_light_count);
                        const float pickProb = 1.0f / (float)lc;
                        if ((bsdfPdf + lightPdf * pickProb) <= 0.0f) add = false;
                        else contribution = throughput * sd.color * (1.0f / (bsdfPdf + lightPdf * pickProb));
                    }
                    CLAMPINTENSITY(contribution, cam.clamp_value);
                }
                if (add) {
                    float4 a = p.acc[slot];
                    a.x += contribution.x; a.y += contribution.y; a.z += contribution.z; a.w += 0.0f;
                    p.acc[slot] = a;
                }
            } else {
                if (any_map) {
                    const float lambda = __builtin_sqrtf(bitsf(q10.z)) + rfw_log2f(cam.spread_angle * (1.0f / gl_abs(dot(D, N))));
                    const float4 q0 = tp[0], q1 = tp[1], q2 = tp[2];
                    const float tu = w * q0.w + u * q1.w + v * q2.w;
                    const float tv = w * q3.w + u * q4.w + v * q5.w;
                    if ((sd.flags & RFW_MAT_HAS_DIFFUSE_MAP) && sd.diffuse_map >= 0 && (uint32_t)sd.diffuse_map < sc.n_textures) {
                        const f4 c = fetchTexelTrilinear(sc.tex_data, sc.tex_desc[sd.diffuse_map], lambda, tu, tv);
                        sd.color = sd.color * mk3(c.x, c.y, c.z);
                    }
                    if ((sd.flags & RFW_MAT_HAS_NORMAL_MAP) && sd.normal_map >= 0 && (uint32_t)sd.normal_map < sc.n_textures) {
                        const f4 c = texture_sample(sc.tex_data, sc.tex_desc[sd.normal_map], tu, tv, (float)f2i(lambda));
                        const f3 m = (mk3(c.x, c.y, c.z) - mk3(0.5f)) * 2.0f;
                        N = normalize((T * m.x + B * m.y) + N * m.z);
                    }
                }
                prepare_tint(sd);
                const bool backFacing = dot(D, gN) >= 0.0f;
                if (backFacing) {
                    N = N * -1.0f;
                    gN = gN * -1.0f;
                }
                throughput = throughput * (1.0f / bsdfPdf);
                float newBsdfPdf = 0.0f;
                f3 R = mk3(0.0f);
                float r1, r2;
                const bool blue = sc.blue_noise != nullptr && sampleId < 256u;
                const int by = (int)div_magic(PATH_ID, cam.width, cam.width_magic), bx = (int)(PATH_ID - (uint32_t)by * cam.width);
                if (blue) {
                    r1 = blueNoiseSampler(sc.blue_noise, sampleId, bx, by, (int)(4u + 4u * path_length));
                    r2 = blueNoiseSampler(sc.blue_noise, sampleId, bx, by, (int)(5u + 4u * path_length));
                } else {
                    r1 = randf(seed);
                    r2 = randf(seed);
                }
                const float F_gN = Fr_of(sd, dot(gN, D * -1.0f));
                const f3 bsdf = SampleBSDF(sd, N, gN, T, B, D * -1.0f, T_VAL, backFacing, r1, r2, R, newBsdfPdf, F_gN);
                throughput = throughput * bsdf * gl_abs(dot(N, R));
                throughput = gl_max(throughput, mk3(0.0f));
                if (!(newBsdfPdf <= 1e-4f || gl_isnan(newBsdfPdf))) {
                    const int lc = (int)(cam.area_light_count + cam.point_light_count + cam.spot_light_count + cam.directional_light_count);
                    if (!(cam.flags & kFlagNoNee) && lc > 0) {
                        float r3;
                        if (blue) r3 = blueNoiseSampler(sc.blue_noise, sampleId, bx, by, (int)(6u + 4u * path_length));
                        else r3 = randf(seed);
                        LightView lv;
                        lv.area = sc.area_lights; lv.point = sc.point_lights; lv.spot = sc.spot_lights; lv.directional = sc.directional_lights;
                        lv.n_area = (int)cam.area_light_count; lv.n_point = (int)cam.point_light_count;
                        lv.n_spot = (int)cam.spot_light_count; lv.n_directional = (int)cam.directional_light_count;
                        f3 lightColor = mk3(0.0f);
                        float pickProb = 0.0f, lightPdf = 0.0f;
                        int picked = 0;
                        f3 L = RandomPointOnLight(lv, r3, P, N, pickProb, lightPdf, lightColor, picked) - P;
                        const float dist = length(L);
                        L = L * (1.0f / dist);
                        const float NdotL = dot(L, N);
                        if (NdotL > 0.0f && lightPdf > 0.0f) {
                            float shadowPdf = 0.0f;
                            const f3 sampledBSDF = EvaluateBSDF(sd, gN, D * -1.0f, L, shadowPdf, F_gN);
                            if (shadowPdf > 0.0f) {
                                f3 contribution = throughput * sampledBSDF * lightColor * (NdotL / (lightPdf * pickProb));
                                if (!(gl_isnan(contribution.x) || gl_isnan(contribution.y) || gl_isnan(contribution.z))) {
                                    CLAMPINTENSITY(contribution, cam.clamp_value);
                                    sh_o = safe_origin(P, L, gN);
                                    sh_d = L;
                                    sh_dist = dist - 1e-4f;
                                    sh_e = contribution;
                                    sh_slot = slot;
                                    push_shadow = true;
                                    light_bucket = picked >= lc - (int)cam.directional_light_count ? kShadowBuckets - 1 : (int)((uint32_t)picked % (uint32_t)(kShadowBuckets - 1));
                                }
                            }
                        }
                    }
                    if (bounce + 1 < cam.max_path_length) {
                        ext_o = safe_origin(P, R, gN);
                        ext_d = R;
                        ext_normal = PackNormal(N);
                        ext_thr = throughput;
                        ext_pdf = newBsdfPdf;
                        push_ext = true;
                    }
                }
            }
        }
    }

    constexpr int kQ = kShadowBuckets + 1;
    __shared__ uint32_t s_cnt[kQ][kShadeBlock / 64];
    __shared__ uint32_t s_base[kQ];
    const uint32_t lane = threadIdx.x & 63u, wave = threadIdx.x >> 6;
    uint32_t my_rank = 0;
    for (int q = 0; q < kShadowBuckets; q++) {
        const bool mine = push_shadow && light_bucket == q;
        const unsigned long long m = __ballot(mine);
        if (lane == 0) s_cnt[q][wave] = (uint32_t)__popcll(m);
        if (mine) my_rank = __builtin_amdgcn_mbcnt_hi((uint32_t)(m >> 32), __builtin_amdgcn_mbcnt_lo((uint32_t)m, 0u));
    }
    __shared__ uint32_t s_ext[8][kShadeBlock / 64];
    const bool any_ext = bounce + 1 < cam.max_path_length;
    const uint32_t ext_oct = (fbits(ext_d.x) >> 31) | ((fbits(ext_d.y) >> 31) << 1) | ((fbits(ext_d.z) >> 31) << 2);
    uint32_t r_ex = 0;
    if (any_ext) {
        uint32_t total_wave = 0;
        for (uint32_t o8 = 0; o8 < 8u; o8++) {
            const bool mine = push_ext && ext_oct == o8;
            const unsigned long long m = __ballot(mine);
            if (lane == 0) s_ext[o8][wave] = (uint32_t)__popcll(m);
            if (mine) r_ex = __builtin_amdgcn_mbcnt_hi((uint32_t)(m >> 32), __builtin_amdgcn_mbcnt_lo((uint32_t)m, 0u));
            total_wave += (uint32_t)__popcll(m);
        }
        if (lane == 0) s_cnt[kShadowBuckets][wave] = total_wave;
    } else if (lane == 0) s_cnt[kShadowBuckets][wave] = 0u;
    __syncthreads();
    if (threadIdx.x < kQ) {
        uint32_t tot = 0;
        for (int k = 0; k < kShadeBlock / 64; k++) tot += s_cnt[threadIdx.x][k];
        uint32_t base = 0;
        if (tot) base = atomicAdd(threadIdx.x < kShadowBuckets ? &sc.counters->shadow[bounce][threadIdx.x] : &sc.counters->ext[bounce], tot);
        s_base[threadIdx.x] = base;
    }
    uint32_t ext_before = 0;
    constexpr uint32_t kExtCounts = 8u * (kShadeBlock / 64);
    if (any_ext && threadIdx.x >= 64u && threadIdx.x < 64u + kExtCounts) {
        const uint32_t t8 = threadIdx.x - 64u;
        const uint32_t* flat = &s_ext[0][0];
        for (uint32_t k = 0; k < t8; k++) ext_before += flat[k];
    }
    __syncthreads();
    if (any_ext && threadIdx.x >= 64u && threadIdx.x < 64u + kExtCounts) (&s_ext[0][0])[threadIdx.x - 64u] = ext_before;
    __syncthreads();
    if (push_shadow) {
        uint32_t off = s_base[light_bucket];
        for (uint32_t k = 0; k < wave; k++) off += s_cnt[light_bucket][k];
        const size_t j = (size_t)light_bucket * p.capacity + off + my_rank;
        p.sh_o[j] = make_float4(sh_o.x, sh_o.y, sh_o.z, bitsf(PATH_WORD));
        p.sh_d[j] = make_float4(sh_d.x, sh_d.y, sh_d.z, sh_dist);
        p.sh_e[j] = make_float4(sh_e.x, sh_e.y, sh_e.z, bitsf(sh_slot));
    }
    if (push_ext) {
        const uint32_t j = s_base[kShadowBuckets] + s_ext[ext_oct][wave] + r_ex;
        p.ray_o[next_half][j] = make_float4(ext_o.x, ext_o.y, ext_o.z, bitsf(PATH_WORD));
        p.ray_d[next_half][j] = make_float4(ext_d.x, ext_d.y, ext_d.z, bitsf(ext_normal));
        p.thr[next_half][j] = make_float4(ext_thr.x, ext_thr.y, ext_thr.z, ext_pdf);
    }
}

__global__ __launch_bounds__(256) void k_pack_rgb(const float4* __restrict__ acc_slab, float* __restrict__ out, const uint64_t n)
{
    const uint64_t i = (uint64_t)blockIdx.x * 256u + threadIdx.x;
    if (i >= n) return;
    const float4 a = acc_slab[i];
    out[3 * i] = a.x;
    out[3 * i + 1] = a.y;
    out[3 * i + 2] = a.z;
}
template <bool LINEAR> RFW_DI float finalise(const float a, const float s) { return LINEAR ? a * 1.0f / s : __builtin_sqrtf(a * 1.0f / s); }
template <bool LINEAR>
__global__ __launch_bounds__(256) void k_pack_f16(const float4* __restrict__ acc_slab, _Float16* __restrict__ out, const uint64_t n, const uint32_t samples)
{
    const uint64_t i = (uint64_t)blockIdx.x * 256u + threadIdx.x;
    if (i >= n) return;
    const float4 a = acc_slab[i];
    const float s = (float)(int)samples;
    out[3 * i] = (_Float16)finalise<LINEAR>(a.x, s);
    out[3 * i + 1] = (_Float16)finalise<LINEAR>(a.y, s);
    out[3 * i + 2] = (_Float16)finalise<LINEAR>(a.z, s);
}
struct SrgbSteps { float t[256]; };
__device__ inline uint32_t srgb_encode(const float* s_t, float x)
{
    uint32_t lo = 0;
    for (uint32_t bit = 128; bit != 0; bit >>= 1)
        if (x >= s_t[lo + bit - 1]) lo += bit;
    return lo;
}
template <bool LINEAR>
__global__ __launch_bounds__(256) void k_pack_bgra8(const float4* __restrict__ acc_slab, uint32_t* __restrict__ out, const uint64_t n, const uint32_t samples,
                                                   const SrgbSteps steps)
{
    __shared__ float s_t[256];
    s_t[threadIdx.x] = steps.t[threadIdx.x];
    __syncthreads();
    const float s = (float)(int)samples;
    for (uint64_t i = (uint64_t)blockIdx.x * 256u + threadIdx.x; i < n; i += (uint64_t)gridDim.x * 256u) {
        const float4 a = acc_slab[i];
        const float r = finalise<LINEAR>(a.x, s), g = finalise<LINEAR>(a.y, s), b = finalise<LINEAR>(a.z, s);
        out[i] = srgb_encode(s_t, b) | (srgb_encode(s_t, g) << 8) | (srgb_encode(s_t, r) << 16) | 0xff000000u;
    }
}
__global__ void k_assemble_f16(const CameraParams cam, const _Float16* __restrict__ gathered, const uint64_t slab_elems, float4* __restrict__ frame)
{
    const uint32_t px = blockIdx.x * blockDim.x + threadIdx.x, py = blockIdx.y * blockDim.y + threadIdx.y;
    if (px >= cam.width || py >= cam.height) return;
    uint32_t owner;
    const uint32_t slot = pixel_to_slab(cam, px, py, owner);
    const uint32_t f = blockIdx.z;
    const _Float16* g = gathered + 3 * (((uint64_t)owner * cam.batch + f) * slab_elems + slot);
// ... 172 lines not shown
    st.t[255] = __builtin_inff();
    return st;
}

void launch_prepare_instances(hipStream_t s, const rfw_mat4* matrices, const uint32_t* mesh_of_instance, const MeshRecord* meshes, uint32_t n,
                              InstanceXform* xf, InstanceNormal* nm)
{
    if (n == 0) return;
    hipLaunchKernelGGL(k_prepare_instances, dim3(ceil_div(n, 64)), dim3(64), 0, s, matrices, mesh_of_instance, meshes, n, xf, nm);
}
void launch_tlas_finish(hipStream_t s, const Node4* raw, Node4Q* out, const OctantCopies& oc, uint32_t n_nodes_max, const uint32_t* live, const rfw_mat4* matrices,
                        const uint32_t* mesh_of_instance, const MeshRecord* meshes, uint32_t n_instances, InstanceXform* xf, InstanceNormal* nm)
{
    const uint32_t expand_blocks = ceil_div((uint64_t)n_nodes_max * 8u, 256), prepare_blocks = ceil_div(n_instances, 256);
    if (expand_blocks + prepare_blocks == 0u) return;
    hipLaunchKernelGGL(k_tlas_finish, dim3(expand_blocks + prepare_blocks), dim3(256), 0, s, raw, out, oc.wide, oc.quant, oc.stride, n_nodes_max, live, expand_blocks, matrices,
                       mesh_of_instance, meshes, n_instances, xf, nm);
}
void launch_primary(hipStream_t s, const CameraParams& cam, const SceneDev& sc, const PathDev& p, bool count)
{
    const dim3 grid((ceil_div(p.capacity, kTraceBlock) + 511u) & ~511u), block(kTraceBlock);
    if ((cam.flags & kFlagPacketPrimary) && sc.tlas_wide && sc.blas_wide) {
        if (count) hipLaunchKernelGGL(k_primary_packet<true>, grid, block, 0, s, cam, sc, p);
        else hipLaunchKernelGGL(k_primary_packet<false>, grid, block, 0, s, cam, sc, p);
        return;
    }
    if (count) hipLaunchKernelGGL(k_primary<true>, grid, block, 0, s, cam, sc, p);
    else hipLaunchKernelGGL(k_primary<false>, grid, block, 0, s, cam, sc, p);
}
void launch_primary_batch(hipStream_t s, const CameraParams& cam, const BatchViews& views, const SceneDev& sc, const PathDev& p, bool count)
{
    const dim3 grid((ceil_div(p.capacity, kTraceBlock) + 511u) & ~511u), block(kTraceBlock);
    if ((cam.flags & kFlagPacketPrimary) && sc.tlas_wide && sc.blas_wide) {
        if (count) hipLaunchKernelGGL(k_primary_batch_packet<true>, grid, block, 0, s, cam, views, sc, p);
        else hipLaunchKernelGGL(k_primary_batch_packet<false>, grid, block, 0, s, cam, views, sc, p);
        return;
    }
    if (count) hipLaunchKernelGGL(k_primary_batch<true>, grid, block, 0, s, cam, views, sc, p);
    else hipLaunchKernelGGL(k_primary_batch<false>, grid, block, 0, s, cam, views, sc, p);
}
void launch_extend(hipStream_t s, const CameraParams& cam, const SceneDev& sc, const PathDev& p, uint32_t bounce, bool count, const uint32_t* order)
{
    const dim3 block(kTraceBlock);
    if (cam.stream_run) {
        const dim3 grid((ceil_div(p.capacity, kTraceBlock * cam.stream_run) + 511u) & ~511u);
        if (count) hipLaunchKernelGGL(k_extend_stream<true>, grid, block, 0, s, cam, sc, p, bounce, order);
        else hipLaunchKernelGGL(k_extend_stream<false>, grid, block, 0, s, cam, sc, p, bounce, order);
        return;
    }
    const dim3 grid((ceil_div(p.capacity, kTraceBlock) + 511u) & ~511u);
    if (count) hipLaunchKernelGGL(k_extend<true>, grid, block, 0, s, cam, sc, p, bounce, order);
    else hipLaunchKernelGGL(k_extend<false>, grid, block, 0, s, cam, sc, p, bounce, order);
}
void launch_shade(hipStream_t s, const CameraParams& cam, const SceneDev& sc, const PathDev& p, uint32_t bounce)
{
    const bool small = (cam.flags & kFlagShadeSmallGroups) != 0u;
    if (cam.batch > 1) {
        if (small) hipLaunchKernelGGL((k_shade<true, 256>), dim3(ceil_div(p.capacity, 256)), dim3(256), 0, s, cam, sc, p, bounce);
        else hipLaunchKernelGGL((k_shade<true, 512>), dim3(ceil_div(p.capacity, 512)), dim3(512), 0, s, cam, sc, p, bounce);
    } else {
        if (small) hipLaunchKernelGGL((k_shade<false, 256>), dim3(ceil_div(p.capacity, 256)), dim3(256), 0, s, cam, sc, p, bounce);
        else hipLaunchKernelGGL((k_shade<false, 512>), dim3(ceil_div(p.capacity, 512)), dim3(512), 0, s, cam, sc, p, bounce);
    }
}
void launch_shadow(hipStream_t s, const CameraParams& cam_in, const SceneDev& sc, const PathDev& p, uint32_t bounce, bool count)
{
    CameraParams cam = cam_in;
    if (!(bounce == 0 && sc.tlas_wide && sc.blas_wide && cam.batch <= 1) || (cam.flags & kFlagPacketShadow)) cam.flags &= ~kFlagPacketShadowFar;
    if (bounce == 0 && (cam.flags & kFlagPacketShadow) && sc.tlas_wide && sc.blas_wide && cam.batch <= 1) {
        const uint32_t blocks_ = (p.capacity + kTraceBlock - 1) / kTraceBlock + kShadowBuckets;
        const dim3 grid_(((blocks_ + 511u) / 512u) * 512u), block_(kTraceBlock);
        if (count) {
            hipLaunchKernelGGL((k_shadow_packet<true, true>), grid_, block_, 0, s, cam, sc, p, bounce);
            hipLaunchKernelGGL((k_shadow_packet<true, false>), grid_, block_, 0, s, cam, sc, p, bounce);
        } else {
            hipLaunchKernelGGL((k_shadow_packet<false, true>), grid_, block_, 0, s, cam, sc, p, bounce);
            hipLaunchKernelGGL((k_shadow_packet<false, false>), grid_, block_, 0, s, cam, sc, p, bounce);
        }
        return;
    }
    if (cam.flags & kFlagPacketShadowFar) {
        const uint32_t blocks_ = (p.capacity + kTraceBlock - 1) / kTraceBlock + kShadowBuckets;
        const dim3 grid_(((blocks_ + 511u) / 512u) * 512u), block_(kTraceBlock);
        if (count) hipLaunchKernelGGL((k_shadow_packet<true, true>), grid_, block_, 0, s, cam, sc, p, bounce);
        else hipLaunchKernelGGL((k_shadow_packet<false, true>), grid_, block_, 0, s, cam, sc, p, bounce);
    }
    const dim3 block(kTraceBlock);
    if (cam.stream_run && bounce >= 1u) {
        const dim3 grid((ceil_div(p.capacity, kTraceBlock * cam.stream_run) + kShadowBuckets + 511u) & ~511u);
        if (count) {
            hipLaunchKernelGGL((k_shadow_stream<true, true>), grid, block, 0, s, cam, sc, p, bounce);
            hipLaunchKernelGGL((k_shadow_stream<true, false>), grid, block, 0, s, cam, sc, p, bounce);
        } else {
            hipLaunchKernelGGL((k_shadow_stream<false, true>), grid, block, 0, s, cam, sc, p, bounce);
            hipLaunchKernelGGL((k_shadow_stream<false, false>), grid, block, 0, s, cam, sc, p, bounce);
        }
        return;
    }
    const dim3 grid((ceil_div(p.capacity, kTraceBlock) + kShadowBuckets + 511u) & ~511u);
    if (cam.batch > 1) {
        if (count) hipLaunchKernelGGL((k_shadow<true, true>), grid, block, 0, s, cam, sc, p, bounce);
        else hipLaunchKernelGGL((k_shadow<false, true>), grid, block, 0, s, cam, sc, p, bounce);
    } else if (count) hipLaunchKernelGGL((k_shadow<true, false>), grid, block, 0, s, cam, sc, p, bounce);
    else hipLaunchKernelGGL((k_shadow<false, false>), grid, block, 0, s, cam, sc, p, bounce);
}
typedef float copy_v4f __attribute__((ext_vector_type(4)));
__global__ __launch_bounds__(256) void k_copy_f4(const float4* __restrict__ src4, float4* __restrict__ dst4, const uint64_t n)
{
    const copy_v4f* __restrict__ src = reinterpret_cast<const copy_v4f*>(src4);
    copy_v4f* __restrict__ dst = reinterpret_cast<copy_v4f*>(dst4);
    constexpr uint64_t kChunk = 4u * 256u;
    for (uint64_t base = (uint64_t)blockIdx.x * kChunk; base < n; base += (uint64_t)gridDim.x * kChunk) {
        copy_v4f v[4];
#pragma unroll
        for (int u = 0; u < 4; u++) {
            const uint64_t i = base + (uint64_t)u * 256u + threadIdx.x;
            if (i < n) v[u] = __builtin_nontemporal_load(src + i);
        }
#pragma unroll
        for (int u = 0; u < 4; u++) {
            const uint64_t i = base + (uint64_t)u * 256u + threadIdx.x;
            if (i < n) __builtin_nontemporal_store(v[u], dst + i);
        }
    }
}
template <int MIX> __global__ __launch_bounds__(256) void k_issue_probe(float* out, const uint32_t trips, const float seed)
{
    typedef float v2 __attribute__((ext_vector_type(2)));
    float v[8];
    for (int i = 0; i < 8; i++) v[i] = seed + (float)(threadIdx.x + i);
    const float a = seed * 1.0001f, b = seed * 0.5f;
    const uint32_t u = fbits(seed) | 0x01020304u;
    v2 p[3] = {{v[0], v[1]}, {v[2], v[3]}, {v[4], v[5]}};
    const v2 pa = {a, a}, pb = {b, b};
    uint32_t sc0 = trips, sc1 = trips + 1u, sc2 = trips + 2u;
    for (uint32_t it = 0; it < trips; it++) {
        if (MIX == 0) {
#pragma unroll
            for (int r = 0; r < 4; r++)
#pragma unroll
                for (int k = 0; k < 8; k++) asm volatile("v_fma_f32 %0, %0, %1, %2" : "+v"(v[k]) : "v"(a), "v"(b));
        } else if (MIX == 1) {
#pragma unroll
            for (int r = 0; r < 2; r++) {
                asm volatile("v_cvt_f32_ubyte0 %0, %6\n\tv_cvt_f32_ubyte1 %1, %6\n\tv_cvt_f32_ubyte2 %2, %6\n\tv_cvt_f32_ubyte3 %3, %6\n\tv_cvt_f32_ubyte0 %4, %6\n\tv_cvt_f32_ubyte1 %5, %6"
                             : "=v"(p[0].x), "=v"(p[0].y), "=v"(p[1].x), "=v"(p[1].y), "=v"(p[2].x), "=v"(p[2].y) : "v"(u));
                asm volatile("v_pk_fma_f32 %0, %0, %3, %4\n\tv_pk_fma_f32 %1, %1, %3, %4\n\tv_pk_fma_f32 %2, %2, %3, %4" : "+v"(p[0]), "+v"(p[1]), "+v"(p[2]) : "v"(pa), "v"(pb));
                asm volatile("v_max3_f32 %0, %2, %3, %4\n\tv_min3_f32 %1, %5, %6, %7" : "=v"(v[6]), "=v"(v[7]) : "v"(p[0].x), "v"(p[1].x), "v"(p[2].x), "v"(p[0].y), "v"(p[1].y), "v"(p[2].y));
                asm volatile("v_min_f32 %0, %0, %1" : "+v"(v[7]) : "v"(a));
                asm volatile("v_cmp_ge_f32 vcc, %0, %1\n\tv_cmp_ge_f32 vcc, %0, %2" : : "v"(v[7]), "v"(v[6]), "v"(b) : "vcc");
            }
        } else {
            const float plane = __builtin_amdgcn_readfirstlane(seed);
#pragma unroll
            for (int c = 0; c < 4; c++) {
                uint64_t m;
// ... 178 lines not shown
```

### rfw-rs_amd/csrc/traverse.h

```cpp
#pragma once
#include "device_math.h"
#include "device_types.h"

namespace rfwhip {

constexpr int kTraceBlock = 64;
constexpr int kStackLds = 16;
constexpr int kStackLdsAny = 12;
constexpr int kStackSpill = 48;
constexpr uint32_t kAnyLeafPeriod = 2;
constexpr int kTraceLdsRows = kStackLds + 6, kTraceLdsRowsAny = kStackLdsAny + 6;

struct SceneView {
    const Node4Q* tlas_nodes;
    const uint32_t* tlas_prims;
    const InstanceXform* instances;
    const Node4Q* blas_nodes;
    const Node4Q* tlas_oct;
    const Node4Q* blas_oct;
    uint32_t tlas_oct_stride, blas_oct_stride;
    const TriPacket* tri_packets;
    uint32_t* spill;
    uint32_t spill_stride;
    uint32_t spill_rows;
    uint32_t* overflow_flag;
    QueueCounters* counters;
};

typedef float v2f __attribute__((ext_vector_type(2)));

RFW_DI f3 slab_inv(const f3 d)
{
    return mk3(__builtin_amdgcn_rcpf(d.x), __builtin_amdgcn_rcpf(d.y), __builtin_amdgcn_rcpf(d.z));
}

RFW_DI uint32_t octant_bits(const f3 inv) { return (inv.x < 0.0f ? 1u : 0u) | (inv.y < 0.0f ? 2u : 0u) | (inv.z < 0.0f ? 4u : 0u); }
RFW_DI const Node4Q* space_nodes(const SceneView& sc, const bool blas, const uint32_t node_base, const f3 inv)
{
    const uint32_t oct = octant_bits(inv);
    return blas ? sc.blas_oct + (size_t)oct * sc.blas_oct_stride + node_base : sc.tlas_oct + (size_t)oct * sc.tlas_oct_stride;
}

struct TravCounters {
    uint32_t nodes, tris, insts;
    uint32_t wave_nodes = 0, wave_tris = 0;
    uint32_t wave_uniform = 0;
};

template <bool ANY_HIT, bool COUNT, bool FAR_FIRST = false>
RFW_DI bool traverse(const SceneView& sc, const f3 O, const f3 D, const float t_min, float& t, float& hu, float& hv, int32_t& hit_inst,
                     int32_t& hit_tri, uint32_t* lds_stack, const uint32_t lane_slot, const uint32_t spill_base, TravCounters& tc)
{
    constexpr int kStack = ANY_HIT ? kStackLdsAny : kStackLds;
    f3 o = O, d = D;
    {
        uint32_t* park = lds_stack + kStack * kTraceBlock + lane_slot;
        park[0] = fbits(O.x); park[kTraceBlock] = fbits(O.y); park[2 * kTraceBlock] = fbits(O.z);
        park[3 * kTraceBlock] = fbits(D.x); park[4 * kTraceBlock] = fbits(D.y); park[5 * kTraceBlock] = fbits(D.z);
    }
    auto world_o = [&]() -> f3 {
        const uint32_t* park = lds_stack + kStack * kTraceBlock + lane_slot;
        return mk3(bitsf(park[0]), bitsf(park[kTraceBlock]), bitsf(park[2 * kTraceBlock]));
    };
    auto world_d = [&]() -> f3 {
        const uint32_t* park = lds_stack + kStack * kTraceBlock + lane_slot;
        return mk3(bitsf(park[3 * kTraceBlock]), bitsf(park[4 * kTraceBlock]), bitsf(park[5 * kTraceBlock]));
    };
    if (!((D.x == D.x) && (D.y == D.y) && (D.z == D.z) && (D.x != 0.0f || D.y != 0.0f || D.z != 0.0f))) return false;
    f3 inv = slab_inv(d);
    int sp = 0;
    int blas_sp = -1;
    int32_t cur_inst = -1;
    uint32_t tri_base = 0;
    uint32_t cur = 0;
    const Node4Q* nodes = space_nodes(sc, false, 0u, inv);

    constexpr bool kDsPop = ANY_HIT;
    auto spill_slot = [&]() -> uint32_t {
        uint32_t l = lane_slot;
        if (ANY_HIT) asm volatile("" : "+v"(l));
        return spill_base + l;
    };
    auto push = [&](uint32_t v) {
        if (sp < kStack) lds_stack[sp * kTraceBlock + lane_slot] = v;
        else if (sp < kStack + (int)sc.spill_rows) sc.spill[(size_t)(sp - kStack) * sc.spill_stride + spill_slot()] = v;
        else {
            *sc.overflow_flag = 1u;
            return;
        }
        sp++;
    };
    auto pop = [&]() -> uint32_t {
        sp--;
        if (kDsPop) {
            uint32_t v = lds_stack[(sp < kStack ? sp : kStack - 1) * kTraceBlock + lane_slot];
            if (__builtin_expect(sp >= kStack, 0)) {
                v = sc.spill[(size_t)(sp - kStack) * sc.spill_stride + spill_slot()];
                asm volatile("" : "+v"(v));
            }
            return v;
        }
        if (sp < kStack) return lds_stack[sp * kTraceBlock + lane_slot];
        return sc.spill[(size_t)(sp - kStack) * sc.spill_stride + spill_slot()];
    };

    if constexpr (ANY_HIT) {
#define RFW_TRAV_TOP
#define RFW_TRAV_OCCLUDED occ_ = 1u; next_ = kDoneRef; break;
#define RFW_TRAV_FLAT_WHILE __ballot(cur != kDoneRef) != 0ull
#define RFW_TRAV_LEAF_TRIP ((iteration % kAnyLeafPeriod) == 0u)
#define RFW_TRAV_TLAS_TRIP true
#include "traverse_flat.inc"
#undef RFW_TRAV_TOP
#undef RFW_TRAV_OCCLUDED
#undef RFW_TRAV_FLAT_WHILE
#undef RFW_TRAV_LEAF_TRIP
#undef RFW_TRAV_TLAS_TRIP
        return occ_ != 0u;
    } else {
#define RFW_TRAV_OCCLUDED
#define RFW_TRAV_EXHAUSTED break;
#include "traverse_nested.inc"
#undef RFW_TRAV_OCCLUDED
#undef RFW_TRAV_EXHAUSTED
        return false;
    }
}

template <bool ANY_HIT, bool COUNT, bool FAR_FIRST, class Stream>
RFW_DI void traverse_stream(const SceneView& sc, Stream& st, const uint32_t refill, const uint32_t leaf_gate, uint32_t* lds_stack, const uint32_t lane_slot, const uint32_t spill_base,
                            TravCounters& tc)
{
    constexpr int kStack = ANY_HIT ? kStackLdsAny : kStackLds;
    f3 o = mk3(0.0f), d = o;
    const float t_min = Stream::kTMin;
    float t = 0.0f, hu = 0.0f, hv = 0.0f;
    int32_t hit_inst = -1, hit_tri = -1;
    auto world_o = [&]() -> f3 {
        const uint32_t* park = lds_stack + kStack * kTraceBlock + lane_slot;
        return mk3(bitsf(park[0]), bitsf(park[kTraceBlock]), bitsf(park[2 * kTraceBlock]));
    };
    auto world_d = [&]() -> f3 {
        const uint32_t* park = lds_stack + kStack * kTraceBlock + lane_slot;
        return mk3(bitsf(park[3 * kTraceBlock]), bitsf(park[4 * kTraceBlock]), bitsf(park[5 * kTraceBlock]));
    };
    f3 inv = mk3(0.0f);
    int sp = 0;
    int blas_sp = -1;
    int32_t cur_inst = -1;
    uint32_t tri_base = 0;
    uint32_t cur = 0xfffffffdu;
    const Node4Q* nodes = sc.tlas_nodes;
    constexpr bool kDsPop = ANY_HIT;
    auto spill_slot = [&]() -> uint32_t {
        uint32_t l = lane_slot;
        if (ANY_HIT) asm volatile("" : "+v"(l));
        return spill_base + l;
    };
    auto push = [&](uint32_t v) {
        if (sp < kStack) lds_stack[sp * kTraceBlock + lane_slot] = v;
        else if (sp < kStack + (int)sc.spill_rows) sc.spill[(size_t)(sp - kStack) * sc.spill_stride + spill_slot()] = v;
// ... 81 lines not shown
```

### rfw-rs_amd/csrc/traverse_leaf.inc

```
            const uint32_t first = cur & kLeafFirstMask, count = ((cur >> 27) & 15u) + 1u;
            const float4* tp = reinterpret_cast<const float4*>(sc.tri_packets + tri_base + first);
            for (uint32_t k = 0; k < count; k++) {
                const float4 p0 = tp[3 * k], p1 = tp[3 * k + 1], p2 = tp[3 * k + 2];
                if (COUNT) {
                    tc.tris++;
                    if (__builtin_amdgcn_mbcnt_hi((uint32_t)(__ballot(1) >> 32), __builtin_amdgcn_mbcnt_lo((uint32_t)__ballot(1), 0u)) == 0u) tc.wave_tris++;
                }
                const f3 v0 = mk3(p0.x, p0.y, p0.z), edge1 = mk3(p1.x, p1.y, p1.z), edge2 = mk3(p2.x, p2.y, p2.z);
                const f3 h = cross(d, edge2);
                const float a = dot(edge1, h);
                const float f = 1.0f / a;
                const f3 s = o - v0;
                const float u = f * dot(s, h);
                const f3 q = cross(s, edge1);
                const float v = f * dot(d, q);
                const float tt = f * dot(edge2, q);
                const bool ok = !((a > -0.0001f) & (a < 0.0001f)) & !((u < 0.0f) | (u > 1.0f)) & !((v < 0.0f) | ((u + v) > 1.0f));
                if (ANY_HIT) {
                    if (ok & (tt > t_min) & (tt < t)) { RFW_TRAV_OCCLUDED }
                } else {
                    const int32_t prim = (int32_t)fbits(p0.w);
                    const bool lower = (cur_inst < hit_inst) | ((cur_inst == hit_inst) & (prim < hit_tri));
                    const bool take = ok & (tt > t_min) & ((tt < t) | ((tt == t) & (hit_inst >= 0) & lower));
                    t = take ? tt : t;
                    hu = take ? u * p1.w : hu;
                    hv = take ? v * p1.w : hv;
                    hit_inst = take ? cur_inst : hit_inst;
                    hit_tri = take ? prim : hit_tri;
                }
            }
```

Before: 7745.

## Add per-pixel shadow occluder cache probed in shade before tracing shadow rays

Adds a per-pixel cache that records the instance and triangle that last occluded each pixel's first-bounce shadow ray. The cache is written from the any-hit traversal when an occluder is found. The shade kernel re-tests the cached triangle against the new shadow ray, and if it still blocks, no shadow ray is queued for traversal. This is meant to skip full BVH traversal for shadow rays that stay occluded across frames. In exchange it adds an extra triangle fetch and test per shaded pixel, a cache buffer, and atomics. Resolved rays still count toward the shadow ray statistics.

```diff
diff --git a/include/rfw_hip.h b/include/rfw_hip.h
--- a/include/rfw_hip.h
+++ b/include/rfw_hip.h
@@ -131,6 +131,7 @@
 RFW_HIP_API int rfw_hip_read_framebuffer(void* instance, float* rgba, uint64_t n_floats);
 RFW_HIP_API int rfw_hip_read_accumulator(void* instance, float* rgba, uint64_t n_floats);
 RFW_HIP_API int rfw_hip_get_frame_stats(void* instance, rfw_hip_frame_stats* out);
+RFW_HIP_API int rfw_hip_shadow_cache_stats(void* instance, uint64_t* probed, uint64_t* resolved);
 RFW_HIP_API int rfw_hip_drain_timing(void* instance, rfw_hip_frame_stats* sum, uint32_t* frames);
 RFW_HIP_API int rfw_hip_get_scene_stats(void* instance, rfw_hip_scene_stats* out);
 RFW_HIP_API int rfw_hip_set_stream(void* instance, void* hip_stream);
diff --git a/rfw-rs_amd/backend.py b/rfw-rs_amd/backend.py
--- a/rfw-rs_amd/backend.py
+++ b/rfw-rs_amd/backend.py
@@ -22,6 +22,7 @@
     "rfw_hip_debug_read", "rfw_hip_bandwidth_probe", "rfw_hip_depth_test", "rfw_hip_render_batch", "rfw_hip_assemble_batch",
     "rfw_hip_read_framebuffer_at", "rfw_hip_read_accumulator_at", "rfw_hip_host_alloc", "rfw_hip_host_free", "rfw_hip_download_frame",
     "rfw_hip_wait_downloads", "rfw_hip_wait_download", "rfw_hip_srgb_steps", "rfw_hip_render_samples", "rfw_hip_set_blue_noise", "rfw_hip_debug_eval_shading", "rfw_hip_comm_unique_id", "rfw_hip_comm_init", "rfw_hip_comm_init_loopback", "rfw_hip_comm_destroy", "rfw_hip_p2p_export", "rfw_hip_p2p_connect", "rfw_hip_p2p_disconnect", "rfw_hip_intersect4", "rfw_hip_occludes4", "rfw_hip_debug_lbvh_stress", "rfw_hip_issue_probe",
+    "rfw_hip_shadow_cache_stats",
 ]
 
 _lib = None
@@ -359,6 +360,13 @@
         self._check(self._l.rfw_hip_read_accumulator(self._h, a.ctypes.data, a.size))
         return a
 
+    def shadow_cache_stats(self):
+        f = self._l.rfw_hip_shadow_cache_stats
+        f.argtypes = [C.c_void_p, C.POINTER(C.c_uint64), C.POINTER(C.c_uint64)]
+        probed, resolved = C.c_uint64(0), C.c_uint64(0)
+        self._check(f(self._h, C.byref(probed), C.byref(resolved)))
+        return int(probed.value), int(resolved.value)
+
     def frame_stats(self):
         s = pod.FrameStats()
         self._check(self._l.rfw_hip_get_frame_stats(self._h, C.byref(s)))
diff --git a/rfw-rs_amd/csrc/api_frame.cpp b/rfw-rs_amd/csrc/api_frame.cpp
--- a/rfw-rs_amd/csrc/api_frame.cpp
+++ b/rfw-rs_amd/csrc/api_frame.cpp
@@ -20,6 +20,7 @@
     if (const char* v = getenv("RFW_PACKET_AUTO_MAX_TRIANGLES")) e.packet_auto_max_triangles = strtoull(v, nullptr, 10);
     if (const char* v = getenv("RFW_SPATIAL_SPLITS")) { e.has_spatial_splits = true; e.spatial_splits = (float)std::max(0.0, atof(v)); }
     if (const char* v = getenv("RFW_PACKET_TRACE")) e.packet_trace = std::max(0, atoi(v));
+    if (const char* v = getenv("RFW_SHADOW_CACHE")) e.shadow_cache = std::max(0, std::min(3, atoi(v)));
     if (const char* v = getenv("RFW_NODE_ORDER")) e.node_order = std::max(0, atoi(v));
     static std::mutex mu;
     std::lock_guard<std::mutex> g(mu);
@@ -213,6 +214,7 @@
 {
     const rfw_camera_view_3d& view = views[0];
     HIP_TRY(I, hipSetDevice(I->device));
+    I->frame_shadow_cache = 0;
     if (!scene_of(I)->synchronized || tlas_of(I)->d_tlas_nodes.ptr == nullptr) return RFW_HIP_OK;
     if (I->scene && I->scene->scene_ready && I->waited_version != I->scene->scene_version) {
         HIP_TRY(I, hipStreamWaitEvent(I->stream, I->scene->scene_ready, 0));
@@ -260,6 +262,23 @@
         for (int q = 0; q < 2 && I->denoise > 1; q++) HIP_TRY(I, I->d_dn_plane[q].ensure(px));
     }
 
+    uint32_t occ_mode = 0;
+    if (mode == RFW_HIP_RENDER_DEFAULT && k == 1 && !count && nee && !(I->flags & (kFlagPacketShadow | kFlagPacketShadowFar))) occ_mode = (uint32_t)scene_of(I)->shadow_cache;
+    if (occ_mode == 3u) occ_mode = 1u;
+    else if (I->sample_count != 0u) occ_mode = 0u;
+    if (occ_mode) {
+        Instance* O = scene_of(I);
+        const size_t px = (size_t)I->width * I->height;
+        if (O->d_occ_cache.cap < px) {
+            HIP_TRY(I, O->d_occ_cache.ensure(px));
+            HIP_TRY(I, hipMemsetAsync(O->d_occ_cache.ptr, 0xff, O->d_occ_cache.cap * sizeof(unsigned long long), main));
+            HIP_TRY(I, hipStreamSynchronize(main));
+        }
+    }
+    I->frame_shadow_cache = occ_mode;
+    const OccDev occ_dev{occ_mode ? scene_of(I)->d_occ_cache.ptr : nullptr, (uint32_t)tlas_of(I)->n_instances, (uint32_t)scene_of(I)->mesh_records.size()};
+    const OccDev* occ = occ_mode ? &occ_dev : nullptr;
+
     if (tm) (void)hipEventRecord(I->events[EV_FRAME0], main);
     I->counter_phase ^= 1u;
     if (S > 1) HIP_TRY(I, hipEventRecord(I->ev_fork, main));
@@ -276,6 +295,9 @@
         sc[s].spill = I->d_spill.ptr + (size_t)s * (I->cap_v + kSpillMargin);
         p[s] = path_dev(I, s);
         cam[s] = camera_params(I, view, s);
+        if (occ_mode) {
+            cam[s].flags |= kFlagShadowCache | (occ_mode == 2u ? kFlagShadowCacheKeep : 0u);
+        }
         {
             const Instance* O = scene_of(I);
             const int g = O->shade_group;
@@ -348,14 +370,14 @@
         for (uint32_t s = 0; s < S; s++) {
             hipEvent_t* ev = ring_events(I, slot, s);
             if (tm) (void)hipEventRecord(ev[ev_index(b, 1, 0)], st[s]);
-            launch_shade(st[s], cam[s], sc[s], p[s], b);
+            launch_shade(st[s], cam[s], sc[s], p[s], b, occ);
             if (tm) (void)hipEventRecord(ev[ev_index(b, 1, 1)], st[s]);
         }
         if (nee)
             for (uint32_t s = 0; s < S; s++) {
                 hipEvent_t* ev = ring_events(I, slot, s);
                 if (tm) (void)hipEventRecord(ev[ev_index(b, 2, 0)], st[s]);
-                launch_shadow(st[s], cam[s], sc[s], p[s], b, count);
+                launch_shadow(st[s], cam[s], sc[s], p[s], b, count, occ);
                 if (tm) (void)hipEventRecord(ev[ev_index(b, 2, 1)], st[s]);
             }
     }
@@ -465,6 +487,7 @@
         if (pt & 1) I->flags |= kFlagPacketPrimary;
         if (pt & 2) I->flags |= kFlagPacketShadow;
         if (pt & 4) I->flags |= kFlagPacketShadowFar;
+        if (env.shadow_cache >= 0) I->shadow_cache = env.shadow_cache;
     }
     if (I->max_batch > 1 && I->substreams > 1) {
         g_create_error = "max_batch > 1 needs streams <= 1 (a batch already fills the device with one launch per stage)";
@@ -563,6 +586,7 @@
         for (auto& tb : I->tables) { tb.materials.release(); tb.area.release(); tb.point.release(); tb.spot.release(); tb.dir.release(); }
         if (I->tables_ready) (void)hipEventDestroy(I->tables_ready);
         if (I->upload_stream) (void)hipStreamDestroy(I->upload_stream);
+        I->d_occ_cache.release();
         I->d_spill.release(); I->d_counters.release(); I->d_tex_data.release(); I->d_tex_desc.release(); I->d_blue_noise.release();
         I->d_valid_gids.release(); I->d_stage_dev.release(); I->d_tlas_order.release(); I->d_node_count.release(); I->d_inst_boxes.release(); I->d_mesh_local.release();
         I->d_tri_boxes.release(); I->d_lbvh_ws.release(); I->d_blas_order.release();
@@ -692,6 +716,7 @@
     I->restart = true;
     I->width = w;
     I->height = h;
+    I->d_occ_cache.release();
     I->deferred = Instance::Deferred(); I->acc_source = nullptr; I->presented_valid = false;
     const int arc = alloc_paths(I);
     if (arc == RFW_HIP_OK && (scene_of(I)->comm || scene_of(I)->loop)) {
@@ -736,6 +761,10 @@
             I->meshes_dirty = true;
             I->layout_valid = false;
         }
+    }
+    else if (k == "shadow_cache") {
+        if (value != 0.0 && value != 1.0 && value != 2.0 && value != 3.0) return fail(I, RFW_HIP_E_INVALID, "set_option: shadow_cache is 0, 1, 2 or 3");
+        I->shadow_cache = (int)value;
     }
     else if (k == "shade_group") {
         if ((int)value != 0 && (int)value != 256 && (int)value != 512) return fail(I, RFW_HIP_E_INVALID, "set_option: shade_group is 0, 256 or 512");
@@ -973,6 +1002,7 @@
         if (!(I->flags & RFW_HIP_FLAG_NO_NEE))
             for (uint32_t b = 0; b < nb; b++)
                 for (int k = 0; k < kShadowBuckets; k++) out->shadow_rays += qc[s].shadow[b][k];
+        if (!(I->flags & RFW_HIP_FLAG_NO_NEE) && nb && I->frame_shadow_cache == 1u) out->shadow_rays += qc[s].occ_resolved;
         for (int k = 0; k < 3; k++) {
             out->nodes_visited[k] += qc[s].trav[k][0];
             out->tris_tested[k] += qc[s].trav[k][1];
@@ -987,6 +1017,26 @@
     out->bounces = nb;
     out->substreams = I->substreams;
     if (I->frame_recorded && nb) add_frame_timing(I, (int)((I->frame_index - 1) % kTimingRing), nb, !(I->flags & RFW_HIP_FLAG_NO_NEE), out);
+    return RFW_HIP_OK;
+}
+
+int rfw_hip_shadow_cache_stats(void* inst, uint64_t* probed, uint64_t* resolved)
+{
+    LOCK(inst);
+    if (!I->slots.empty() && I->cur_slot != 0) {
+        Instance* c = slot_ptr(I, I->cur_slot);
+        const int rc = rfw_hip_shadow_cache_stats(c, probed, resolved);
+        if (rc != RFW_HIP_OK) I->err = c->err;
+        return rc;
+    }
+    HIP_TRY(I, hipSetDevice(I->device));
+    HIP_TRY(I, hipStreamSynchronize(I->stream));
+    QueueCounters qc[kMaxSub];
+    HIP_TRY(I, hipMemcpy(qc, I->d_counters.ptr + (size_t)I->counter_phase * kMaxSub, I->substreams * sizeof(QueueCounters), hipMemcpyDeviceToHost));
+    uint64_t np = 0, nr = 0;
+    for (uint32_t s = 0; s < I->substreams && I->frame_shadow_cache; s++) { np += qc[s].occ_probed; nr += qc[s].occ_resolved; }
+    if (probed) *probed = np;
+    if (resolved) *resolved = nr;
     return RFW_HIP_OK;
 }
 
diff --git a/rfw-rs_amd/csrc/api_internal.h b/rfw-rs_amd/csrc/api_internal.h
--- a/rfw-rs_amd/csrc/api_internal.h
+++ b/rfw-rs_amd/csrc/api_internal.h
@@ -357,6 +357,9 @@
     DevBuf<uint4> d_hit[2];
     DevBuf<uint32_t> d_sort_keys[2], d_sort_vals[2];
     DevBuf<char> d_sort_ws;
+    int shadow_cache = 1;
+    DevBuf<unsigned long long> d_occ_cache;
+    uint32_t frame_shadow_cache = 0;
     int shade_group = 0;
     int sort_extension_rays = 2;
     void* external_slab = nullptr;
diff --git a/rfw-rs_amd/csrc/device_types.h b/rfw-rs_amd/csrc/device_types.h
--- a/rfw-rs_amd/csrc/device_types.h
+++ b/rfw-rs_amd/csrc/device_types.h
@@ -212,11 +212,13 @@
 };
 
 constexpr int kShadowBuckets = 8;
+constexpr unsigned long long kOccEmpty = ~0ull;
 struct QueueCounters {
     uint32_t ext[8];
     uint32_t shadow[8][kShadowBuckets];
     unsigned long long trav[3][3];
-    unsigned long long overflow, pad;
+    unsigned long long overflow;
+    uint32_t occ_probed, occ_resolved;
     unsigned long long wave_max_nodes[3];
     unsigned long long wave_exec[3][2];
     unsigned long long max_nodes[3];
@@ -227,7 +229,8 @@
 
 enum : uint32_t { kFlagNoNee = 1u, kFlagCount = 2u, kFlagNearFirstDirectional = 4u, kFlagFarFirstPositional = 8u,
                   kFlagPacketPrimary = 16u, kFlagPacketShadow = 32u,
-                  kFlagPacketShadowFar = 64u, kFlagShadeSmallGroups = 128u };
-
-
-}
+                  kFlagPacketShadowFar = 64u, kFlagShadeSmallGroups = 128u,
+                  kFlagShadowCache = 256u, kFlagShadowCacheKeep = 512u };
+
+
+}
diff --git a/rfw-rs_amd/csrc/env_switches.h b/rfw-rs_amd/csrc/env_switches.h
--- a/rfw-rs_amd/csrc/env_switches.h
+++ b/rfw-rs_amd/csrc/env_switches.h
@@ -12,6 +12,7 @@
     bool has_spatial_splits = false;
     float spatial_splits = 0.0f;
     int node_order = 0;
+    int shadow_cache = -1;
     int packet_trace = -1;
 };
 const EnvSwitches& env_switches();
diff --git a/rfw-rs_amd/csrc/kernels.h b/rfw-rs_amd/csrc/kernels.h
--- a/rfw-rs_amd/csrc/kernels.h
+++ b/rfw-rs_amd/csrc/kernels.h
@@ -38,6 +38,11 @@
     QueueCounters* counters_next;
 };
 
+struct OccDev {
+    unsigned long long* cache;
+    uint32_t n_instances, n_meshes;
+};
+
 struct PathDev {
     float4* ray_o[2];
     float4* ray_d[2];
@@ -56,8 +61,8 @@
 void launch_primary_batch(hipStream_t s, const CameraParams& cam, const BatchViews& views, const SceneDev& sc, const PathDev& p, bool count);
 void launch_extend(hipStream_t s, const CameraParams& cam, const SceneDev& sc, const PathDev& p, uint32_t bounce, bool count, const uint32_t* order = nullptr);
 void launch_extension_keys(hipStream_t s, const SceneDev& sc, const PathDev& p, uint32_t bounce, uint32_t* keys, uint32_t* vals);
-void launch_shade(hipStream_t s, const CameraParams& cam, const SceneDev& sc, const PathDev& p, uint32_t bounce);
-void launch_shadow(hipStream_t s, const CameraParams& cam, const SceneDev& sc, const PathDev& p, uint32_t bounce, bool count);
+void launch_shade(hipStream_t s, const CameraParams& cam, const SceneDev& sc, const PathDev& p, uint32_t bounce, const OccDev* occ = nullptr);
+void launch_shadow(hipStream_t s, const CameraParams& cam, const SceneDev& sc, const PathDev& p, uint32_t bounce, bool count, const OccDev* occ = nullptr);
 void launch_copy_f4(hipStream_t s, const float4* src, float4* dst, uint64_t n);
 void launch_issue_probe(hipStream_t s, int mix, uint32_t cus, uint32_t trips, float* out);
 uint32_t issue_probe_vector_per_trip(int mix);
diff --git a/rfw-rs_amd/csrc/kernels.hip b/rfw-rs_amd/csrc/kernels.hip
--- a/rfw-rs_amd/csrc/kernels.hip
+++ b/rfw-rs_amd/csrc/kernels.hip
@@ -460,8 +460,8 @@
 }
 
 RFW_DI bool bucket_far_first(const CameraParams& cam, const uint32_t bucket);
-template <bool COUNT, bool BATCH = false>
-__global__ __launch_bounds__(kTraceBlock, kTraceWavesAny) void k_shadow(const CameraParams cam, const SceneDev sc, const PathDev p, const uint32_t bounce)
+template <bool COUNT, bool BATCH, bool OCC>
+RFW_DI void shadow_body(const CameraParams& cam, const SceneDev& sc, const PathDev& p, const uint32_t bounce, const OccDev& oc)
 {
     __shared__ uint32_t s_stack[kTraceLdsRowsAny * kTraceBlock];
     uint32_t block = xcd_block(blockIdx.x);
@@ -492,8 +492,9 @@
         int32_t hi = -1, ht = -1;
         const SceneView sv = scene_view(sc);
         const bool far_first = bucket == (uint32_t)kShadowBuckets - 1u ? !(cam.flags & kFlagNearFirstDirectional) : (cam.flags & kFlagFarFirstPositional) != 0u;
-        const bool occluded = far_first ? traverse<true, COUNT, true>(sv, O, D, 0.001f, t, hu, hv, hi, ht, s_stack, threadIdx.x, spill_base, tc)
-                                        : traverse<true, COUNT, false>(sv, O, D, 0.001f, t, hu, hv, hi, ht, s_stack, threadIdx.x, spill_base, tc);
+        const OccSink occ{OCC && bounce == 0u && (cam.flags & kFlagShadowCache) ? oc.cache : nullptr, p.sh_o + (bucket * p.capacity + block * kTraceBlock)};
+        const bool occluded = far_first ? traverse<true, COUNT, true, OCC>(sv, O, D, 0.001f, t, hu, hv, hi, ht, s_stack, threadIdx.x, spill_base, tc, occ)
+                                        : traverse<true, COUNT, false, OCC>(sv, O, D, 0.001f, t, hu, hv, hi, ht, s_stack, threadIdx.x, spill_base, tc, occ);
         if (!occluded) {
             uint32_t lane = threadIdx.x;
             asm volatile("" : "+v"(lane));
@@ -505,6 +506,15 @@
         }
     }
     flush_counters<COUNT>(sc.counters, tc, 2);
+}
+template <bool COUNT, bool BATCH = false>
+__global__ __launch_bounds__(kTraceBlock, kTraceWavesAny) void k_shadow(const CameraParams cam, const SceneDev sc, const PathDev p, const uint32_t bounce)
+{
+    shadow_body<COUNT, BATCH, false>(cam, sc, p, bounce, OccDev{nullptr, 0u, 0u});
+}
+__global__ __launch_bounds__(kTraceBlock, kTraceWavesAny) void k_shadow_occ(const CameraParams cam, const SceneDev sc, const PathDev p, const uint32_t bounce, const OccDev oc)
+{
+    shadow_body<false, false, true>(cam, sc, p, bounce, oc);
 }
 
 RFW_DI bool bucket_far_first(const CameraParams& cam, const uint32_t bucket);
@@ -616,262 +626,48 @@
     flush_counters<COUNT>(sc.counters, tc, 2);
 }
 
+RFW_DI bool occ_probe(const SceneDev& sc, const OccDev& oc, const uint32_t pixel, const f3 O, const f3 D, const float t_min, const float t, bool& probed)
+{
+    const unsigned long long e = __atomic_load_n(oc.cache + pixel, __ATOMIC_RELAXED);
+    const uint32_t inst = (uint32_t)(e >> 32), rel = (uint32_t)e;
+    if (e == kOccEmpty || inst >= oc.n_instances) return false;
+    const float4* ip = reinterpret_cast<const float4*>(sc.instances + inst);
+    const uint4 meta = *reinterpret_cast<const uint4*>(ip + 3);
+    if (!(meta.z & 1u) || meta.w >= oc.n_meshes) return false;
+    const MeshRecord* rec = sc.meshes + meta.w;
+    const uint2 range = *reinterpret_cast<const uint2*>(&rec->tri_base);
+    if (range.x != meta.y || rel >= range.y) return false;
+    probed = true;
+    f3 o, d;
+    if (meta.z & kInstanceIdentity) {
+        o = mk3(O.x + 0.0f, O.y + 0.0f, O.z + 0.0f);
+        d = mk3(D.x + 0.0f, D.y + 0.0f, D.z + 0.0f);
+    } else {
+        const float4 r0 = ip[0], r1 = ip[1], r2 = ip[2];
+        o = xform_rows(r0, r1, r2, O, 1.0f);
+        d = xform_rows(r0, r1, r2, D, 0.0f);
+    }
+    const float4* tp = reinterpret_cast<const float4*>(sc.tri_packets + meta.y + rel);
+    const float4 p0 = tp[0], p1 = tp[1], p2 = tp[2];
+    const f3 v0 = mk3(p0.x, p0.y, p0.z), edge1 = mk3(p1.x, p1.y, p1.z), edge2 = mk3(p2.x, p2.y, p2.z);
+    RFW_TRI_TEST(o, d, v0, edge1, edge2)
+    return RFW_TRI_BLOCKS(t_min, t);
+}
+
 template <bool BATCH, int kShadeBlock>
 __global__ __launch_bounds__(kShadeBlock) void k_shade(const CameraParams cam, const SceneDev sc, const PathDev p, const uint32_t bounce)
 {
-    static_assert(kShadeBlock >= 128 && 8 * (kShadeBlock / 64) <= 64, "k_shade: the extension-ray filing needs a second wavefront and at most 64 (octant, wavefront) counts");
-    const uint32_t idx = blockIdx.x * kShadeBlock + threadIdx.x;
-    const uint32_t count = bounce == 0 ? p.capacity : sc.counters->ext[bounce - 1];
-    if (blockIdx.x * kShadeBlock >= count) return;
-    const uint32_t half = bounce & 1u, next_half = half ^ 1u;
-    const uint32_t path_length = bounce;
-
-    bool live = idx < count;
-
-    bool push_ext = false, push_shadow = false;
-    int light_bucket = 0;
-    f3 ext_o = mk3(0.0f), ext_d = mk3(0.0f), ext_thr = mk3(0.0f);
-    float ext_pdf = 0.0f;
-    uint32_t ext_normal = 0;
-    f3 sh_o = mk3(0.0f), sh_d = mk3(0.0f), sh_e = mk3(0.0f);
-    float sh_dist = 0.0f;
-    uint32_t PATH_ID = 0, PATH_WORD = 0, sh_slot = 0;
-
-    uint4 S = make_uint4(kNoPath, 0u, 0u, 0u);
-    if (live) {
-        S = p.hit[half][idx];
-        live = S.x != kNoPath;
-    }
-    if (live) {
-        const float4 O4 = p.ray_o[half][idx], D4 = p.ray_d[half][idx];
-        const f3 O = mk3(O4.x, O4.y, O4.z), D = mk3(D4.x, D4.y, D4.z);
-        f3 throughput = mk3(1.0f);
-        float bsdfPdf = 1.0f;
-        if (path_length != 0) {
-            const float4 T4 = p.thr[half][idx];
-            throughput = mk3(T4.x, T4.y, T4.z);
-            bsdfPdf = T4.w;
-        }
-        const uint32_t path_word = fbits(O4.w);
-        PATH_ID = BATCH ? (path_word & 0xffffffu) : path_word;
-        PATH_WORD = path_word;
-        uint32_t owner, slot = idx;
-        if (bounce != 0) {
-            const uint32_t py_ = div_magic(PATH_ID, cam.width, cam.width_magic);
-            slot = pixel_to_slab(cam, PATH_ID - py_ * cam.width, py_, owner) + (BATCH ? (path_word >> 24) * cam.frame_capacity : 0u);
-        }
-        const int32_t INST_ID = (int32_t)S.x;
-        const uint32_t TRI_ID = S.y;
-        const float T_VAL = bitsf(S.z);
-
-        if (INST_ID < 0) {
-            f3 sky = mk3(cam.sky[0], cam.sky[1], cam.sky[2]);
-            if (sc.skybox.mips) {
-                const float su = 0.5f * (1.0f + rfw_atan2f(D.x, -D.z) * (1.0f / 3.14159265359f));
-                const float sv = 1.0f - rfw_acosf(D.y) * (1.0f / 3.14159265359f);
-                const f4 c = texture_sample(sc.tex_data, sc.skybox, su, sv, (float)(int)path_length);
-                sky = mk3(c.x, c.y, c.z);
-            }
-            f3 contribution = throughput * sky * (1.0f / bsdfPdf);
-            CLAMPINTENSITY(contribution, cam.clamp_value);
-            float4 a = p.acc[slot];
-            a.x += contribution.x; a.y += contribution.y; a.z += contribution.z; a.w += 0.0f;
-            p.acc[slot] = a;
-        } else {
-            const float4* tp = reinterpret_cast<const float4*>(sc.triangles + TRI_ID);
-            const float4 q3 = tp[3], q4 = tp[4], q5 = tp[5], q6 = tp[6], T0 = tp[7], T1 = tp[8], T2 = tp[9];
-            const uint4 q10 = *reinterpret_cast<const uint4*>(tp + 10);
-            const int32_t mat_id = (int32_t)q10.y;
-            const float tri_area = bitsf(q10.w);
-            ShadingData sd = extractParameters(sc.materials + mat_id);
-
-            const uint32_t sampleId = BATCH ? cam.batch_sample[path_word >> 24] : cam.sample_count;
-            uint32_t seed = wang_hash(PATH_ID * 16789u + sampleId * 1791u + path_length * 720898027u);
-
-            const float u = (float)(S.w & 65535u) * (1.0f / 65535.0f);
-            const float v = (float)(S.w >> 16) * (1.0f / 65535.0f);
-            const float w = 1.0f - u - v;
-
-            f3 gN = mk3(q3.x, q3.y, q3.z);
-            f3 N = w * mk3(q4.x, q4.y, q4.z) + u * mk3(q5.x, q5.y, q5.z) + v * mk3(q6.x, q6.y, q6.z);
-            f3 T = w * mk3(T0.x, T0.y, T0.z) + u * mk3(T1.x, T1.y, T1.z) + v * mk3(T2.x, T2.y, T2.z);
-            const float Tw = w * T0.w + u * T1.w + v * T2.w;
-
-            const float4* np = reinterpret_cast<const float4*>(sc.instance_normals + INST_ID);
-            const float4 n0 = np[0], n1 = np[1], n2 = np[2];
-            gN = normalize(xform_rows(n0, n1, n2, gN, 0.0f));
-            N = normalize(xform_rows(n0, n1, n2, N, 0.0f));
-            T = normalize(xform_rows(n0, n1, n2, T, 0.0f));
-            const f3 B = cross(N, T) * Tw;
-            const f3 P = O + T_VAL * D;
-
-            const bool any_map = (sd.flags & 63u) != 0u;
-            if ((sd.color.x > 1.0f || sd.color.y > 1.0f || sd.color.z > 1.0f) && !(sd.flags & RFW_MAT_HAS_EMISSIVE_MAP)) {
-                f3 contribution = mk3(0.0f);
-                const float DdotNL = -dot(D, N);
-                bool add = true;
-                if (DdotNL > 0.0f) {
-                    if (path_length == 0) {
-                        contribution = throughput * sd.color * (1.0f / bsdfPdf);
-                    } else {
-                        const float lightPdf = CalculateLightPDF(D, T_VAL, tri_area, N);
-                        const int lc = (int)(cam.area_light_count + cam.point_light_count + cam.spot_light_count + cam.directional_light_count);
-                        const float pickProb = 1.0f / (float)lc;
-                        if ((bsdfPdf + lightPdf * pickProb) <= 0.0f) add = false;
-                        else contribution = throughput * sd.color * (1.0f / (bsdfPdf + lightPdf * pickProb));
-                    }
-                    CLAMPINTENSITY(contribution, cam.clamp_value);
-                }
-                if (add) {
-                    float4 a = p.acc[slot];
-                    a.x += contribution.x; a.y += contribution.y; a.z += contribution.z; a.w += 0.0f;
-                    p.acc[slot] = a;
-                }
-            } else {
-                if (any_map) {
-                    const float lambda = __builtin_sqrtf(bitsf(q10.z)) + rfw_log2f(cam.spread_angle * (1.0f / gl_abs(dot(D, N))));
-                    const float4 q0 = tp[0], q1 = tp[1], q2 = tp[2];
-                    const float tu = w * q0.w + u * q1.w + v * q2.w;
-                    const float tv = w * q3.w + u * q4.w + v * q5.w;
-                    if ((sd.flags & RFW_MAT_HAS_DIFFUSE_MAP) && sd.diffuse_map >= 0 && (uint32_t)sd.diffuse_map < sc.n_textures) {
-                        const f4 c = fetchTexelTrilinear(sc.tex_data, sc.tex_desc[sd.diffuse_map], lambda, tu, tv);
-                        sd.color = sd.color * mk3(c.x, c.y, c.z);
-                    }
-                    if ((sd.flags & RFW_MAT_HAS_NORMAL_MAP) && sd.normal_map >= 0 && (uint32_t)sd.normal_map < sc.n_textures) {
-                        const f4 c = texture_sample(sc.tex_data, sc.tex_desc[sd.normal_map], tu, tv, (float)f2i(lambda));
-                        const f3 m = (mk3(c.x, c.y, c.z) - mk3(0.5f)) * 2.0f;
-                        N = normalize((T * m.x + B * m.y) + N * m.z);
-                    }
-                }
-                prepare_tint(sd);
-                const bool backFacing = dot(D, gN) >= 0.0f;
-                if (backFacing) {
-                    N = N * -1.0f;
-                    gN = gN * -1.0f;
-                }
-                throughput = throughput * (1.0f / bsdfPdf);
-                float newBsdfPdf = 0.0f;
-                f3 R = mk3(0.0f);
-                float r1, r2;
-                const bool blue = sc.blue_noise != nullptr && sampleId < 256u;
-                const int by = (int)div_magic(PATH_ID, cam.width, cam.width_magic), bx = (int)(PATH_ID - (uint32_t)by * cam.width);
-                if (blue) {
-                    r1 = blueNoiseSampler(sc.blue_noise, sampleId, bx, by, (int)(4u + 4u * path_length));
-                    r2 = blueNoiseSampler(sc.blue_noise, sampleId, bx, by, (int)(5u + 4u * path_length));
-                } else {
-                    r1 = randf(seed);
-                    r2 = randf(seed);
-                }
-                const float F_gN = Fr_of(sd, dot(gN, D * -1.0f));
-                const f3 bsdf = SampleBSDF(sd, N, gN, T, B, D * -1.0f, T_VAL, backFacing, r1, r2, R, newBsdfPdf, F_gN);
-                throughput = throughput * bsdf * gl_abs(dot(N, R));
-                throughput = gl_max(throughput, mk3(0.0f));
-                if (!(newBsdfPdf <= 1e-4f || gl_isnan(newBsdfPdf))) {
-                    const int lc = (int)(cam.area_light_count + cam.point_light_count + cam.spot_light_count + cam.directional_light_count);
-                    if (!(cam.flags & kFlagNoNee) && lc > 0) {
-                        float r3;
-                        if (blue) r3 = blueNoiseSampler(sc.blue_noise, sampleId, bx, by, (int)(6u + 4u * path_length));
-                        else r3 = randf(seed);
-                        LightView lv;
-                        lv.area = sc.area_lights; lv.point = sc.point_lights; lv.spot = sc.spot_lights; lv.directional = sc.directional_lights;
-                        lv.n_area = (int)cam.area_light_count; lv.n_point = (int)cam.point_light_count;
-                        lv.n_spot = (int)cam.spot_light_count; lv.n_directional = (int)cam.directional_light_count;
-                        f3 lightColor = mk3(0.0f);
-                        float pickProb = 0.0f, lightPdf = 0.0f;
-                        int picked = 0;
-                        f3 L = RandomPointOnLight(lv, r3, P, N, pickProb, lightPdf, lightColor, picked) - P;
-                        const float dist = length(L);
-                        L = L * (1.0f / dist);
-                        const float NdotL = dot(L, N);
-                        if (NdotL > 0.0f && lightPdf > 0.0f) {
-                            float shadowPdf = 0.0f;
-                            const f3 sampledBSDF = EvaluateBSDF(sd, gN, D * -1.0f, L, shadowPdf, F_gN);
-                            if (shadowPdf > 0.0f) {
-                                f3 contribution = throughput * sampledBSDF * lightColor * (NdotL / (lightPdf * pickProb));
-                                if (!(gl_isnan(contribution.x) || gl_isnan(contribution.y) || gl_isnan(contribution.z))) {
-                                    CLAMPINTENSITY(contribution, cam.clamp_value);
-                                    sh_o = safe_origin(P, L, gN);
-                                    sh_d = L;
-                                    sh_dist = dist - 1e-4f;
-                                    sh_e = contribution;
-                                    sh_slot = slot;
-                                    push_shadow = true;
-                                    light_bucket = picked >= lc - (int)cam.directional_light_count ? kShadowBuckets - 1 : (int)((uint32_t)picked % (uint32_t)(kShadowBuckets - 1));
-                                }
-                            }
-                        }
-                    }
-                    if (bounce + 1 < cam.max_path_length) {
-                        ext_o = safe_origin(P, R, gN);
-                        ext_d = R;
-                        ext_normal = PackNormal(N);
-                        ext_thr = throughput;
-                        ext_pdf = newBsdfPdf;
-                        push_ext = true;
-                    }
-                }
-            }
-        }
-    }
-
-    constexpr int kQ = kShadowBuckets + 1;
-    __shared__ uint32_t s_cnt[kQ][kShadeBlock / 64];
-    __shared__ uint32_t s_base[kQ];
-    const uint32_t lane = threadIdx.x & 63u, wave = threadIdx.x >> 6;
-    uint32_t my_rank = 0;
-    for (int q = 0; q < kShadowBuckets; q++) {
-        const bool mine = push_shadow && light_bucket == q;
-        const unsigned long long m = __ballot(mine);
-        if (lane == 0) s_cnt[q][wave] = (uint32_t)__popcll(m);
-        if (mine) my_rank = __builtin_amdgcn_mbcnt_hi((uint32_t)(m >> 32), __builtin_amdgcn_mbcnt_lo((uint32_t)m, 0u));
-    }
-    __shared__ uint32_t s_ext[8][kShadeBlock / 64];
-    const bool any_ext = bounce + 1 < cam.max_path_length;
-    const uint32_t ext_oct = (fbits(ext_d.x) >> 31) | ((fbits(ext_d.y) >> 31) << 1) | ((fbits(ext_d.z) >> 31) << 2);
-    uint32_t r_ex = 0;
-    if (any_ext) {
-        uint32_t total_wave = 0;
-        for (uint32_t o8 = 0; o8 < 8u; o8++) {
-            const bool mine = push_ext && ext_oct == o8;
-            const unsigned long long m = __ballot(mine);
-            if (lane == 0) s_ext[o8][wave] = (uint32_t)__popcll(m);
-            if (mine) r_ex = __builtin_amdgcn_mbcnt_hi((uint32_t)(m >> 32), __builtin_amdgcn_mbcnt_lo((uint32_t)m, 0u));
-            total_wave += (uint32_t)__popcll(m);
-        }
-        if (lane == 0) s_cnt[kShadowBuckets][wave] = total_wave;
-    } else if (lane == 0) s_cnt[kShadowBuckets][wave] = 0u;
-    __syncthreads();
-    if (threadIdx.x < kQ) {
-        uint32_t tot = 0;
-        for (int k = 0; k < kShadeBlock / 64; k++) tot += s_cnt[threadIdx.x][k];
-        uint32_t base = 0;
-        if (tot) base = atomicAdd(threadIdx.x < kShadowBuckets ? &sc.counters->shadow[bounce][threadIdx.x] : &sc.counters->ext[bounce], tot);
-        s_base[threadIdx.x] = base;
-    }
-    uint32_t ext_before = 0;
-    constexpr uint32_t kExtCounts = 8u * (kShadeBlock / 64);
-    if (any_ext && threadIdx.x >= 64u && threadIdx.x < 64u + kExtCounts) {
-        const uint32_t t8 = threadIdx.x - 64u;
-        const uint32_t* flat = &s_ext[0][0];
-        for (uint32_t k = 0; k < t8; k++) ext_before += flat[k];
-    }
-    __syncthreads();
-    if (any_ext && threadIdx.x >= 64u && threadIdx.x < 64u + kExtCounts) (&s_ext[0][0])[threadIdx.x - 64u] = ext_before;
-    __syncthreads();
-    if (push_shadow) {
-        uint32_t off = s_base[light_bucket];
-        for (uint32_t k = 0; k < wave; k++) off += s_cnt[light_bucket][k];
-        const size_t j = (size_t)light_bucket * p.capacity + off + my_rank;
-        p.sh_o[j] = make_float4(sh_o.x, sh_o.y, sh_o.z, bitsf(PATH_WORD));
-        p.sh_d[j] = make_float4(sh_d.x, sh_d.y, sh_d.z, sh_dist);
-        p.sh_e[j] = make_float4(sh_e.x, sh_e.y, sh_e.z, bitsf(sh_slot));
-    }
-    if (push_ext) {
-        const uint32_t j = s_base[kShadowBuckets] + s_ext[ext_oct][wave] + r_ex;
-        p.ray_o[next_half][j] = make_float4(ext_o.x, ext_o.y, ext_o.z, bitsf(PATH_WORD));
-        p.ray_d[next_half][j] = make_float4(ext_d.x, ext_d.y, ext_d.z, bitsf(ext_normal));
-        p.thr[next_half][j] = make_float4(ext_thr.x, ext_thr.y, ext_thr.z, ext_pdf);
-    }
+#define RFW_SHADE_OCC 0
+#include "shade_body.inc"
+#undef RFW_SHADE_OCC
+}
+template <int kShadeBlock>
+__global__ __launch_bounds__(kShadeBlock) void k_shade_occ(const CameraParams cam, const SceneDev sc, const PathDev p, const uint32_t bounce, const OccDev oc)
+{
+    constexpr bool BATCH = false;
+#define RFW_SHADE_OCC 1
+#include "shade_body.inc"
+#undef RFW_SHADE_OCC
 }
 
 __global__ __launch_bounds__(256) void k_pack_rgb(const float4* __restrict__ acc_slab, float* __restrict__ out, const uint64_t n)
@@ -1150,18 +946,21 @@
     if (count) hipLaunchKernelGGL(k_extend<true>, grid, block, 0, s, cam, sc, p, bounce, order);
     else hipLaunchKernelGGL(k_extend<false>, grid, block, 0, s, cam, sc, p, bounce, order);
 }
-void launch_shade(hipStream_t s, const CameraParams& cam, const SceneDev& sc, const PathDev& p, uint32_t bounce)
+void launch_shade(hipStream_t s, const CameraParams& cam, const SceneDev& sc, const PathDev& p, uint32_t bounce, const OccDev* occ)
 {
     const bool small = (cam.flags & kFlagShadeSmallGroups) != 0u;
     if (cam.batch > 1) {
         if (small) hipLaunchKernelGGL((k_shade<true, 256>), dim3(ceil_div(p.capacity, 256)), dim3(256), 0, s, cam, sc, p, bounce);
         else hipLaunchKernelGGL((k_shade<true, 512>), dim3(ceil_div(p.capacity, 512)), dim3(512), 0, s, cam, sc, p, bounce);
+    } else if (bounce == 0 && (cam.flags & kFlagShadowCache) && occ && occ->cache) {
+        if (small) hipLaunchKernelGGL((k_shade_occ<256>), dim3(ceil_div(p.capacity, 256)), dim3(256), 0, s, cam, sc, p, bounce, *occ);
+        else hipLaunchKernelGGL((k_shade_occ<512>), dim3(ceil_div(p.capacity, 512)), dim3(512), 0, s, cam, sc, p, bounce, *occ);
     } else {
         if (small) hipLaunchKernelGGL((k_shade<false, 256>), dim3(ceil_div(p.capacity, 256)), dim3(256), 0, s, cam, sc, p, bounce);
         else hipLaunchKernelGGL((k_shade<false, 512>), dim3(ceil_div(p.capacity, 512)), dim3(512), 0, s, cam, sc, p, bounce);
     }
 }
-void launch_shadow(hipStream_t s, const CameraParams& cam_in, const SceneDev& sc, const PathDev& p, uint32_t bounce, bool count)
+void launch_shadow(hipStream_t s, const CameraParams& cam_in, const SceneDev& sc, const PathDev& p, uint32_t bounce, bool count, const OccDev* occ)
 {
     CameraParams cam = cam_in;
     if (!(bounce == 0 && sc.tlas_wide && sc.blas_wide && cam.batch <= 1) || (cam.flags & kFlagPacketShadow)) cam.flags &= ~kFlagPacketShadowFar;
@@ -1200,6 +999,7 @@
         if (count) hipLaunchKernelGGL((k_shadow<true, true>), grid, block, 0, s, cam, sc, p, bounce);
         else hipLaunchKernelGGL((k_shadow<false, true>), grid, block, 0, s, cam, sc, p, bounce);
     } else if (count) hipLaunchKernelGGL((k_shadow<true, false>), grid, block, 0, s, cam, sc, p, bounce);
+    else if (bounce == 0 && (cam.flags & kFlagShadowCache) && occ && occ->cache) hipLaunchKernelGGL(k_shadow_occ, grid, block, 0, s, cam, sc, p, bounce, *occ);
     else hipLaunchKernelGGL((k_shadow<false, false>), grid, block, 0, s, cam, sc, p, bounce);
 }
 typedef float copy_v4f __attribute__((ext_vector_type(4)));
diff --git a/rfw-rs_amd/csrc/shade_body.inc b/rfw-rs_amd/csrc/shade_body.inc
--- /dev/null
+++ b/rfw-rs_amd/csrc/shade_body.inc
@@ -0,0 +1,282 @@
+    static_assert(kShadeBlock >= 128 && 8 * (kShadeBlock / 64) <= 64, "k_shade: the extension-ray filing needs a second wavefront and at most 64 (octant, wavefront) counts");
+    const uint32_t idx = blockIdx.x * kShadeBlock + threadIdx.x;
+    const uint32_t count = bounce == 0 ? p.capacity : sc.counters->ext[bounce - 1];
+    if (blockIdx.x * kShadeBlock >= count) return;
+    const uint32_t half = bounce & 1u, next_half = half ^ 1u;
+    const uint32_t path_length = bounce;
+
+    bool live = idx < count;
+
+    bool push_ext = false, push_shadow = false;
+#if RFW_SHADE_OCC
+    bool occ_probed = false, occ_resolved = false;
+#endif
+    int light_bucket = 0;
+    f3 ext_o = mk3(0.0f), ext_d = mk3(0.0f), ext_thr = mk3(0.0f);
+    float ext_pdf = 0.0f;
+    uint32_t ext_normal = 0;
+    f3 sh_o = mk3(0.0f), sh_d = mk3(0.0f), sh_e = mk3(0.0f);
+    float sh_dist = 0.0f;
+    uint32_t PATH_ID = 0, PATH_WORD = 0, sh_slot = 0;
+
+    uint4 S = make_uint4(kNoPath, 0u, 0u, 0u);
+    if (live) {
+        S = p.hit[half][idx];
+        live = S.x != kNoPath;
+    }
+    if (live) {
+        const float4 O4 = p.ray_o[half][idx], D4 = p.ray_d[half][idx];
+        const f3 O = mk3(O4.x, O4.y, O4.z), D = mk3(D4.x, D4.y, D4.z);
+        f3 throughput = mk3(1.0f);
+        float bsdfPdf = 1.0f;
+        if (path_length != 0) {
+            const float4 T4 = p.thr[half][idx];
+            throughput = mk3(T4.x, T4.y, T4.z);
+            bsdfPdf = T4.w;
+        }
+        const uint32_t path_word = fbits(O4.w);
+        PATH_ID = BATCH ? (path_word & 0xffffffu) : path_word;
+        PATH_WORD = path_word;
+        uint32_t owner, slot = idx;
+        if (bounce != 0) {
+            const uint32_t py_ = div_magic(PATH_ID, cam.width, cam.width_magic);
+            slot = pixel_to_slab(cam, PATH_ID - py_ * cam.width, py_, owner) + (BATCH ? (path_word >> 24) * cam.frame_capacity : 0u);
+        }
+        const int32_t INST_ID = (int32_t)S.x;
+        const uint32_t TRI_ID = S.y;
+        const float T_VAL = bitsf(S.z);
+
+        if (INST_ID < 0) {
+            f3 sky = mk3(cam.sky[0], cam.sky[1], cam.sky[2]);
+            if (sc.skybox.mips) {
+                const float su = 0.5f * (1.0f + rfw_atan2f(D.x, -D.z) * (1.0f / 3.14159265359f));
+                const float sv = 1.0f - rfw_acosf(D.y) * (1.0f / 3.14159265359f);
+                const f4 c = texture_sample(sc.tex_data, sc.skybox, su, sv, (float)(int)path_length);
+                sky = mk3(c.x, c.y, c.z);
+            }
+            f3 contribution = throughput * sky * (1.0f / bsdfPdf);
+            CLAMPINTENSITY(contribution, cam.clamp_value);
+            float4 a = p.acc[slot];
+            a.x += contribution.x; a.y += contribution.y; a.z += contribution.z; a.w += 0.0f;
+            p.acc[slot] = a;
+        } else {
+            const float4* tp = reinterpret_cast<const float4*>(sc.triangles + TRI_ID);
+            const float4 q3 = tp[3], q4 = tp[4], q5 = tp[5], q6 = tp[6], T0 = tp[7], T1 = tp[8], T2 = tp[9];
+            const uint4 q10 = *reinterpret_cast<const uint4*>(tp + 10);
+            const int32_t mat_id = (int32_t)q10.y;
+            const float tri_area = bitsf(q10.w);
+            ShadingData sd = extractParameters(sc.materials + mat_id);
+
+            const uint32_t sampleId = BATCH ? cam.batch_sample[path_word >> 24] : cam.sample_count;
+            uint32_t seed = wang_hash(PATH_ID * 16789u + sampleId * 1791u + path_length * 720898027u);
+
+            const float u = (float)(S.w & 65535u) * (1.0f / 65535.0f);
+            const float v = (float)(S.w >> 16) * (1.0f / 65535.0f);
+            const float w = 1.0f - u - v;
+
+            f3 gN = mk3(q3.x, q3.y, q3.z);
+            f3 N = w * mk3(q4.x, q4.y, q4.z) + u * mk3(q5.x, q5.y, q5.z) + v * mk3(q6.x, q6.y, q6.z);
+            f3 T = w * mk3(T0.x, T0.y, T0.z) + u * mk3(T1.x, T1.y, T1.z) + v * mk3(T2.x, T2.y, T2.z);
+            const float Tw = w * T0.w + u * T1.w + v * T2.w;
+
+            const float4* np = reinterpret_cast<const float4*>(sc.instance_normals + INST_ID);
+            const float4 n0 = np[0], n1 = np[1], n2 = np[2];
+            gN = normalize(xform_rows(n0, n1, n2, gN, 0.0f));
+            N = normalize(xform_rows(n0, n1, n2, N, 0.0f));
+            T = normalize(xform_rows(n0, n1, n2, T, 0.0f));
+            const f3 B = cross(N, T) * Tw;
+            const f3 P = O + T_VAL * D;
+
+            const bool any_map = (sd.flags & 63u) != 0u;
+            if ((sd.color.x > 1.0f || sd.color.y > 1.0f || sd.color.z > 1.0f) && !(sd.flags & RFW_MAT_HAS_EMISSIVE_MAP)) {
+                f3 contribution = mk3(0.0f);
+                const float DdotNL = -dot(D, N);
+                bool add = true;
+                if (DdotNL > 0.0f) {
+                    if (path_length == 0) {
+                        contribution = throughput * sd.color * (1.0f / bsdfPdf);
+                    } else {
+                        const float lightPdf = CalculateLightPDF(D, T_VAL, tri_area, N);
+                        const int lc = (int)(cam.area_light_count + cam.point_light_count + cam.spot_light_count + cam.directional_light_count);
+                        const float pickProb = 1.0f / (float)lc;
+                        if ((bsdfPdf + lightPdf * pickProb) <= 0.0f) add = false;
+                        else contribution = throughput * sd.color * (1.0f / (bsdfPdf + lightPdf * pickProb));
+                    }
+                    CLAMPINTENSITY(contribution, cam.clamp_value);
+                }
+                if (add) {
+                    float4 a = p.acc[slot];
+                    a.x += contribution.x; a.y += contribution.y; a.z += contribution.z; a.w += 0.0f;
+                    p.acc[slot] = a;
+                }
+            } else {
+                if (any_map) {
+                    const float lambda = __builtin_sqrtf(bitsf(q10.z)) + rfw_log2f(cam.spread_angle * (1.0f / gl_abs(dot(D, N))));
+                    const float4 q0 = tp[0], q1 = tp[1], q2 = tp[2];
+                    const float tu = w * q0.w + u * q1.w + v * q2.w;
+                    const float tv = w * q3.w + u * q4.w + v * q5.w;
+                    if ((sd.flags & RFW_MAT_HAS_DIFFUSE_MAP) && sd.diffuse_map >= 0 && (uint32_t)sd.diffuse_map < sc.n_textures) {
+                        const f4 c = fetchTexelTrilinear(sc.tex_data, sc.tex_desc[sd.diffuse_map], lambda, tu, tv);
+                        sd.color = sd.color * mk3(c.x, c.y, c.z);
+                    }
+                    if ((sd.flags & RFW_MAT_HAS_NORMAL_MAP) && sd.normal_map >= 0 && (uint32_t)sd.normal_map < sc.n_textures) {
+                        const f4 c = texture_sample(sc.tex_data, sc.tex_desc[sd.normal_map], tu, tv, (float)f2i(lambda));
+                        const f3 m = (mk3(c.x, c.y, c.z) - mk3(0.5f)) * 2.0f;
+                        N = normalize((T * m.x + B * m.y) + N * m.z);
+                    }
+                }
+                prepare_tint(sd);
+                const bool backFacing = dot(D, gN) >= 0.0f;
+                if (backFacing) {
+                    N = N * -1.0f;
+                    gN = gN * -1.0f;
+                }
+                throughput = throughput * (1.0f / bsdfPdf);
+                float newBsdfPdf = 0.0f;
+                f3 R = mk3(0.0f);
+                float r1, r2;
+                const bool blue = sc.blue_noise != nullptr && sampleId < 256u;
+                const int by = (int)div_magic(PATH_ID, cam.width, cam.width_magic), bx = (int)(PATH_ID - (uint32_t)by * cam.width);
+                if (blue) {
+                    r1 = blueNoiseSampler(sc.blue_noise, sampleId, bx, by, (int)(4u + 4u * path_length));
+                    r2 = blueNoiseSampler(sc.blue_noise, sampleId, bx, by, (int)(5u + 4u * path_length));
+                } else {
+                    r1 = randf(seed);
+                    r2 = randf(seed);
+                }
+                const float F_gN = Fr_of(sd, dot(gN, D * -1.0f));
+                const f3 bsdf = SampleBSDF(sd, N, gN, T, B, D * -1.0f, T_VAL, backFacing, r1, r2, R, newBsdfPdf, F_gN);
+                throughput = throughput * bsdf * gl_abs(dot(N, R));
+                throughput = gl_max(throughput, mk3(0.0f));
+                if (!(newBsdfPdf <= 1e-4f || gl_isnan(newBsdfPdf))) {
+                    const int lc = (int)(cam.area_light_count + cam.point_light_count + cam.spot_light_count + cam.directional_light_count);
+                    if (!(cam.flags & kFlagNoNee) && lc > 0) {
+                        float r3;
+                        if (blue) r3 = blueNoiseSampler(sc.blue_noise, sampleId, bx, by, (int)(6u + 4u * path_length));
+                        else r3 = randf(seed);
+                        LightView lv;
+                        lv.area = sc.area_lights; lv.point = sc.point_lights; lv.spot = sc.spot_lights; lv.directional = sc.directional_lights;
+                        lv.n_area = (int)cam.area_light_count; lv.n_point = (int)cam.point_light_count;
+                        lv.n_spot = (int)cam.spot_light_count; lv.n_directional = (int)cam.directional_light_count;
+                        f3 lightColor = mk3(0.0f);
+                        float pickProb = 0.0f, lightPdf = 0.0f;
+                        int picked = 0;
+                        f3 L = RandomPointOnLight(lv, r3, P, N, pickProb, lightPdf, lightColor, picked) - P;
+                        const float dist = length(L);
+                        L = L * (1.0f / dist);
+                        const float NdotL = dot(L, N);
+                        if (NdotL > 0.0f && lightPdf > 0.0f) {
+                            float shadowPdf = 0.0f;
+                            const f3 sampledBSDF = EvaluateBSDF(sd, gN, D * -1.0f, L, shadowPdf, F_gN);
+                            if (shadowPdf > 0.0f) {
+                                f3 contribution = throughput * sampledBSDF * lightColor * (NdotL / (lightPdf * pickProb));
+                                if (!(gl_isnan(contribution.x) || gl_isnan(contribution.y) || gl_isnan(contribution.z))) {
+                                    CLAMPINTENSITY(contribution, cam.clamp_value);
+                                    sh_o = safe_origin(P, L, gN);
+                                    sh_d = L;
+                                    sh_dist = dist - 1e-4f;
+                                    sh_e = contribution;
+                                    sh_slot = slot;
+                                    push_shadow = true;
+#if RFW_SHADE_OCC
+                                    {
+                                        float t_ = sh_dist - 0.0001f;
+                                        if (t_ > 3.0e38f) t_ = 3.0e38f;
+                                        occ_resolved = occ_probe(sc, oc, PATH_ID, sh_o, sh_d, 0.001f, t_, occ_probed);
+                                        if (occ_resolved && !(cam.flags & kFlagShadowCacheKeep)) push_shadow = false;
+                                    }
+#endif
+                                    light_bucket = picked >= lc - (int)cam.directional_light_count ? kShadowBuckets - 1 : (int)((uint32_t)picked % (uint32_t)(kShadowBuckets - 1));
+                                }
+                            }
+                        }
+                    }
+                    if (bounce + 1 < cam.max_path_length) {
+                        ext_o = safe_origin(P, R, gN);
+                        ext_d = R;
+                        ext_normal = PackNormal(N);
+                        ext_thr = throughput;
+                        ext_pdf = newBsdfPdf;
+                        push_ext = true;
+                    }
+                }
+            }
+        }
+    }
+
+    constexpr int kQ = kShadowBuckets + 1;
+#if RFW_SHADE_OCC
+    constexpr int kQAll = kQ + 2;
+    __shared__ uint32_t s_cnt[kQAll][kShadeBlock / 64];
+#else
+    __shared__ uint32_t s_cnt[kQ][kShadeBlock / 64];
+#endif
+    __shared__ uint32_t s_base[kQ];
+    const uint32_t lane = threadIdx.x & 63u, wave = threadIdx.x >> 6;
+    uint32_t my_rank = 0;
+    for (int q = 0; q < kShadowBuckets; q++) {
+        const bool mine = push_shadow && light_bucket == q;
+        const unsigned long long m = __ballot(mine);
+        if (lane == 0) s_cnt[q][wave] = (uint32_t)__popcll(m);
+        if (mine) my_rank = __builtin_amdgcn_mbcnt_hi((uint32_t)(m >> 32), __builtin_amdgcn_mbcnt_lo((uint32_t)m, 0u));
+    }
+    __shared__ uint32_t s_ext[8][kShadeBlock / 64];
+    const bool any_ext = bounce + 1 < cam.max_path_length;
+    const uint32_t ext_oct = (fbits(ext_d.x) >> 31) | ((fbits(ext_d.y) >> 31) << 1) | ((fbits(ext_d.z) >> 31) << 2);
+    uint32_t r_ex = 0;
+    if (any_ext) {
+        uint32_t total_wave = 0;
+        for (uint32_t o8 = 0; o8 < 8u; o8++) {
+            const bool mine = push_ext && ext_oct == o8;
+            const unsigned long long m = __ballot(mine);
+            if (lane == 0) s_ext[o8][wave] = (uint32_t)__popcll(m);
+            if (mine) r_ex = __builtin_amdgcn_mbcnt_hi((uint32_t)(m >> 32), __builtin_amdgcn_mbcnt_lo((uint32_t)m, 0u));
+            total_wave += (uint32_t)__popcll(m);
+        }
+        if (lane == 0) s_cnt[kShadowBuckets][wave] = total_wave;
+    } else if (lane == 0) s_cnt[kShadowBuckets][wave] = 0u;
+#if RFW_SHADE_OCC
+    {
+        const unsigned long long mp = __ballot(occ_probed), mr = __ballot(occ_resolved);
+        if (lane == 0) { s_cnt[kQ][wave] = (uint32_t)__popcll(mp); s_cnt[kQ + 1][wave] = (uint32_t)__popcll(mr); }
+    }
+#endif
+    __syncthreads();
+    if (threadIdx.x < kQ) {
+        uint32_t tot = 0;
+        for (int k = 0; k < kShadeBlock / 64; k++) tot += s_cnt[threadIdx.x][k];
+        uint32_t base = 0;
+        if (tot) base = atomicAdd(threadIdx.x < kShadowBuckets ? &sc.counters->shadow[bounce][threadIdx.x] : &sc.counters->ext[bounce], tot);
+        s_base[threadIdx.x] = base;
+    }
+#if RFW_SHADE_OCC
+    if (threadIdx.x >= kQ && threadIdx.x < kQAll) {
+        uint32_t tot = 0;
+        for (int k = 0; k < kShadeBlock / 64; k++) tot += s_cnt[threadIdx.x][k];
+        if (tot) atomicAdd(threadIdx.x == kQ ? &sc.counters->occ_probed : &sc.counters->occ_resolved, tot);
+    }
+#endif
+    uint32_t ext_before = 0;
+    constexpr uint32_t kExtCounts = 8u * (kShadeBlock / 64);
+    if (any_ext && threadIdx.x >= 64u && threadIdx.x < 64u + kExtCounts) {
+        const uint32_t t8 = threadIdx.x - 64u;
+        const uint32_t* flat = &s_ext[0][0];
+        for (uint32_t k = 0; k < t8; k++) ext_before += flat[k];
+    }
+    __syncthreads();
+    if (any_ext && threadIdx.x >= 64u && threadIdx.x < 64u + kExtCounts) (&s_ext[0][0])[threadIdx.x - 64u] = ext_before;
+    __syncthreads();
+    if (push_shadow) {
+        uint32_t off = s_base[light_bucket];
+        for (uint32_t k = 0; k < wave; k++) off += s_cnt[light_bucket][k];
+        const size_t j = (size_t)light_bucket * p.capacity + off + my_rank;
+        p.sh_o[j] = make_float4(sh_o.x, sh_o.y, sh_o.z, bitsf(PATH_WORD));
+        p.sh_d[j] = make_float4(sh_d.x, sh_d.y, sh_d.z, sh_dist);
+        p.sh_e[j] = make_float4(sh_e.x, sh_e.y, sh_e.z, bitsf(sh_slot));
+    }
+    if (push_ext) {
+        const uint32_t j = s_base[kShadowBuckets] + s_ext[ext_oct][wave] + r_ex;
+        p.ray_o[next_half][j] = make_float4(ext_o.x, ext_o.y, ext_o.z, bitsf(PATH_WORD));
+        p.ray_d[next_half][j] = make_float4(ext_d.x, ext_d.y, ext_d.z, bitsf(ext_normal));
+        p.thr[next_half][j] = make_float4(ext_thr.x, ext_thr.y, ext_thr.z, ext_pdf);
+    }
diff --git a/rfw-rs_amd/csrc/traverse.h b/rfw-rs_amd/csrc/traverse.h
--- a/rfw-rs_amd/csrc/traverse.h
+++ b/rfw-rs_amd/csrc/traverse.h
@@ -41,15 +41,32 @@
     return blas ? sc.blas_oct + (size_t)oct * sc.blas_oct_stride + node_base : sc.tlas_oct + (size_t)oct * sc.tlas_oct_stride;
 }
 
+#define RFW_TRI_TEST(o_, d_, v0_, edge1_, edge2_)                                                                                    \
+    const f3 h = cross(d_, edge2_);                                                                                                   \
+    const float a = dot(edge1_, h);                                                                                                   \
+    const float f = 1.0f / a;                                                                                                         \
+    const f3 s = o_ - v0_;                                                                                                            \
+    const float u = f * dot(s, h);                                                                                                    \
+    const f3 q = cross(s, edge1_);                                                                                                    \
+    const float v = f * dot(d_, q);                                                                                                   \
+    const float tt = f * dot(edge2_, q);                                                                                              \
+    const bool ok = !((a > -0.0001f) & (a < 0.0001f)) & !((u < 0.0f) | (u > 1.0f)) & !((v < 0.0f) | ((u + v) > 1.0f));
+#define RFW_TRI_BLOCKS(t_min_, t_) (ok & (tt > (t_min_)) & (tt < (t_)))
+
+struct OccSink {
+    unsigned long long* cache = nullptr;
+    const float4* ids = nullptr;
+};
+
 struct TravCounters {
     uint32_t nodes, tris, insts;
     uint32_t wave_nodes = 0, wave_tris = 0;
     uint32_t wave_uniform = 0;
 };
 
-template <bool ANY_HIT, bool COUNT, bool FAR_FIRST = false>
+template <bool ANY_HIT, bool COUNT, bool FAR_FIRST = false, bool OCC = false>
 RFW_DI bool traverse(const SceneView& sc, const f3 O, const f3 D, const float t_min, float& t, float& hu, float& hv, int32_t& hit_inst,
-                     int32_t& hit_tri, uint32_t* lds_stack, const uint32_t lane_slot, const uint32_t spill_base, TravCounters& tc)
+                     int32_t& hit_tri, uint32_t* lds_stack, const uint32_t lane_slot, const uint32_t spill_base, TravCounters& tc, const OccSink occ = OccSink{})
 {
     constexpr int kStack = ANY_HIT ? kStackLdsAny : kStackLds;
     f3 o = O, d = D;
@@ -106,7 +123,16 @@
 
     if constexpr (ANY_HIT) {
 #define RFW_TRAV_TOP
-#define RFW_TRAV_OCCLUDED occ_ = 1u; next_ = kDoneRef; break;
+#define RFW_TRAV_OCCLUDED                                                                                                             \
+    if constexpr (OCC) {                                                                                                              \
+        if (occ.cache != nullptr) {                                                                                                   \
+            uint32_t l_ = lane_slot;                                                                                                  \
+            asm volatile("" : "+v"(l_));                                                                                              \
+            const uint32_t pixel_ = fbits(occ.ids[l_].w);                                                                             \
+            __atomic_store_n(occ.cache + pixel_, ((unsigned long long)(uint32_t)cur_inst << 32) | (unsigned long long)(first + k), __ATOMIC_RELAXED); \
+        }                                                                                                                             \
+    }                                                                                                                                 \
+    occ_ = 1u; next_ = kDoneRef; break;
 #define RFW_TRAV_FLAT_WHILE __ballot(cur != kDoneRef) != 0ull
 #define RFW_TRAV_LEAF_TRIP ((iteration % kAnyLeafPeriod) == 0u)
 #define RFW_TRAV_TLAS_TRIP true
diff --git a/rfw-rs_amd/csrc/traverse_leaf.inc b/rfw-rs_amd/csrc/traverse_leaf.inc
--- a/rfw-rs_amd/csrc/traverse_leaf.inc
+++ b/rfw-rs_amd/csrc/traverse_leaf.inc
@@ -7,17 +7,9 @@
                     if (__builtin_amdgcn_mbcnt_hi((uint32_t)(__ballot(1) >> 32), __builtin_amdgcn_mbcnt_lo((uint32_t)__ballot(1), 0u)) == 0u) tc.wave_tris++;
                 }
                 const f3 v0 = mk3(p0.x, p0.y, p0.z), edge1 = mk3(p1.x, p1.y, p1.z), edge2 = mk3(p2.x, p2.y, p2.z);
-                const f3 h = cross(d, edge2);
-                const float a = dot(edge1, h);
-                const float f = 1.0f / a;
-                const f3 s = o - v0;
-                const float u = f * dot(s, h);
-                const f3 q = cross(s, edge1);
-                const float v = f * dot(d, q);
-                const float tt = f * dot(edge2, q);
-                const bool ok = !((a > -0.0001f) & (a < 0.0001f)) & !((u < 0.0f) | (u > 1.0f)) & !((v < 0.0f) | ((u + v) > 1.0f));
+                RFW_TRI_TEST(o, d, v0, edge1, edge2)
                 if (ANY_HIT) {
-                    if (ok & (tt > t_min) & (tt < t)) { RFW_TRAV_OCCLUDED }
+                    if (RFW_TRI_BLOCKS(t_min, t)) { RFW_TRAV_OCCLUDED }
                 } else {
                     const int32_t prim = (int32_t)fbits(p0.w);
                     const bool lower = (cur_inst < hit_inst) | ((cur_inst == hit_inst) & (prim < hit_tri));
```

Result: faster. 9062 (median of 6 runs) (+17.0%).
